# ototoi/pbrt-r3

Measured on AMD Instinct MI355X. Metric: Mrays/s, higher is better.
Workload: dtype f32

## Files before the change

pbrt-r3_amd/csrc/pt_context.cpp:

```cpp
#include <hip/hip_runtime.h>

#include <dlfcn.h>

#include <chrono>
#include <cmath>
#include <cstdio>
#include <cstdlib>
#include <cstring>
#include <functional>
#include <string>
#include <array>
#include <memory>
#include <vector>
#include <algorithm>
#include <thread>

#include "../../include/pbrtgpu.h"
#include "pt_bvh.h"
#include "pt_device.h"
#include "pt_host_math.h"
#include "pt_kernels.h"
#include "pt_lobes.h"

namespace {
// ... 154 lines not shown
        ctx->sobol_n_inv = hdr[3];
        ctx->sobol_m32.resize((size_t)hdr[0] * hdr[1]);
        ctx->sobol_vdc.resize((size_t)hdr[2] * hdr[1]);
        ctx->sobol_inv.resize((size_t)hdr[3] * hdr[1]);
        ok = std::fread(ctx->sobol_m32.data(), 4, ctx->sobol_m32.size(), f) == ctx->sobol_m32.size() &&
             std::fread(ctx->sobol_vdc.data(), 8, ctx->sobol_vdc.size(), f) == ctx->sobol_vdc.size() &&
             std::fread(ctx->sobol_inv.data(), 8, ctx->sobol_inv.size(), f) == ctx->sobol_inv.size();
    }
    std::fclose(f);
    return ok;
}

template <class T>
pt_status upload(pt_context* ctx, DevBuf& b, const T* src, size_t n) {
    PT_HIP(b.alloc(n * sizeof(T)));
    if (n) PT_HIP(hipMemcpy(b.p, src, n * sizeof(T), hipMemcpyHostToDevice));
    return PT_OK;
}

pt_status ensure_pool(pt_context* ctx, size_t n_paths) {
    if (ctx->sc.n_instances && ctx->d_hit_inst.bytes < std::max(n_paths, ctx->pool_paths) * 4) {
        PT_HIP(ctx->d_hit_inst.alloc(std::max(n_paths, ctx->pool_paths) * 4));
        ctx->paths.hit_inst = ctx->d_hit_inst.as<uint32_t>();
    }
    const bool tex_split = ctx->sc.textured && !ctx->sc.n_instances;
    if (tex_split && ctx->d_tex_res.bytes < std::max(n_paths, ctx->pool_paths) * (size_t)(PT_TEX_RES_F4 * 16)) {
        PT_HIP(ctx->d_tex_res.alloc(std::max(n_paths, ctx->pool_paths) * (size_t)(PT_TEX_RES_F4 * 16)));
        ctx->paths.tex_res = ctx->d_tex_res.as<float4>();
    } else if (!tex_split && ctx->d_tex_res.p) {
        ctx->d_tex_res.release();
        ctx->paths.tex_res = nullptr;
    }
    if (ctx->pool_paths >= n_paths && ctx->d_pool.p) return PT_OK;
    const size_t per_path = 11 * 16 + 8 + 8 + 6 * 4 + 4;
    PT_HIP(ctx->d_pool.alloc(n_paths * per_path + 16384));
    char* base = ctx->d_pool.as<char>();
    size_t off = 0;
    auto carve = [&](size_t elem) { void* p = base + off; off += (n_paths * elem + 255) & ~(size_t)255; return p; };
    PtPaths& P = ctx->paths;
    P.ray_o = (float4*)carve(16); P.ray_d = (float4*)carve(16);
    P.sh_o = (float4*)carve(16); P.sh_d = (float4*)carve(16);
    P.pr_o = (float4*)carve(16); P.pr_d = (float4*)carve(16);
    P.beta = (float4*)carve(16); P.L = (float4*)carve(16);
    P.pendA = (float4*)carve(16); P.pendB = (float4*)carve(16); P.pbeta = (float4*)carve(16);
    P.p_film = (float2*)carve(8);
    P.sobol_index = (uint64_t*)carve(8);
    P.pixel = (uint32_t*)carve(4); P.state = (uint32_t*)carve(4);
    P.hit_t = (float*)carve(4); P.hit_rec = (int32_t*)carve(4);
    P.nee = (uint32_t*)carve(4);
    P.probe_rec = (int32_t*)carve(4);
    P.occluded = (uint8_t*)carve(1);
    if (off > ctx->d_pool.bytes) return ctx->fail(PT_ERR_DEVICE, "internal: path pool carve overflow");
    PT_HIP(ctx->d_qa.alloc(n_paths * 4));
    PT_HIP(ctx->d_qb.alloc(n_paths * 4));
    PT_HIP(ctx->d_qnee.alloc(n_paths * 4));
    PT_HIP(ctx->d_qsorted.alloc(n_paths * 4));
    PT_HIP(ctx->d_qshadow.alloc(n_paths * 4));
    PT_HIP(ctx->d_qprobe.alloc(n_paths * 4));
    ctx->pool_paths = n_paths;
    return PT_OK;
}

pt_status ensure_traversal_scratch(pt_context* ctx) {
    uint32_t need = ctx->max_stack + 1 > PT_FS_SLOTS - 1 ? ctx->max_stack + 1 - (PT_FS_SLOTS - 1) : 0;
    size_t threads = (size_t)std::max(ctx->grid_trace, 2048) * PT_BLOCK;
    if (!ctx->d_spill.p || ctx->spill_depth < need) {
        PT_HIP(ctx->d_spill.alloc((size_t)std::max(need, 1u) * threads * 4 + PT_DIAG_WORDS * 4));
        PT_HIP(hipMemsetAsync(ctx->d_spill.p, 0, PT_DIAG_WORDS * 4, ctx->stream));
        ctx->spill_depth = need;
    }
    return PT_OK;
}

hipEvent_t get_event(pt_context* ctx, size_t i) {
    while (ctx->ev.size() <= i) {
        hipEvent_t e;
        if (hipEventCreate(&e) != hipSuccess) return nullptr;
        ctx->ev.push_back(e);
    }
    return ctx->ev[i];
}

}

extern "C" {
// ... 1687 lines not shown
            for (int32_t x = sbnd[0]; x < sbnd[2]; x += 16) {
                pt_tile t = {x, y, std::min(x + 16, sbnd[2]), std::min(y + 16, sbnd[3])};
                all.push_back(t);
            }
        tiles = all.data();
        n_tiles = (uint32_t)all.size();
    }
    std::vector<uint32_t> tile_off(n_tiles);
    size_t n_pixels_total = 0;
    for (uint32_t i = 0; i < n_tiles; i++) {
        const pt_tile& t = tiles[i];
        if (t.x0 < sbnd[0] || t.y0 < sbnd[1] || t.x1 > sbnd[2] || t.y1 > sbnd[3] || t.x1 < t.x0 || t.y1 < t.y0)
            return ctx->fail(PT_ERR_INVALID_ARGUMENT, "tile outside the sample bounds");
        tile_off[i] = (uint32_t)n_pixels_total;
        n_pixels_total += (size_t)(t.x1 - t.x0) * (size_t)(t.y1 - t.y0);
        if (n_pixels_total > (size_t)(sbnd[2] - sbnd[0]) * (size_t)(sbnd[3] - sbnd[1])) return ctx->fail(PT_ERR_INVALID_ARGUMENT, "tiles overlap (more pixels than the sample bounds hold)");
    }
    if (n_pixels_total == 0) return PT_OK;
    const uint32_t spp = sc.sobol.spp;

    size_t pool_target = (size_t)288 << 20;
    if (const char* e = std::getenv("PBRTGPU_POOL_PATHS")) pool_target = std::max<size_t>(65536, std::strtoull(e, nullptr, 10));
    pool_target = std::min<size_t>(pool_target, (size_t)1 << 30);
    const bool ao = sc.integrator == PT_INTEGRATOR_AO;
    const bool aov = sc.integrator == PT_INTEGRATOR_AOV;
    const bool rec = sc.integrator == PT_INTEGRATOR_DIRECTLIGHTING || sc.integrator == PT_INTEGRATOR_WHITTED;
    const uint32_t rec_epp = !rec ? 0u : (sc.integrator == PT_INTEGRATOR_DIRECTLIGHTING && sc.direct_strategy == PT_DIRECT_ONE) ? 1u
                             : sc.integrator == PT_INTEGRATOR_WHITTED ? std::max(1u, sc.n_lights) : std::max(1u, ctx->light_samples_total);
    const uint32_t rec_depth = (uint32_t)std::max(1, sc.max_depth);
    const size_t rec_per_path = 64 + (size_t)rec_depth * PT_REC_FRAME_F4 * 16 + (size_t)rec_epp * (6 * 16 + 1 + 4 + 4 + 8);
    {
        size_t free_b = 0, total_b = 0;
        if (hipMemGetInfo(&free_b, &total_b) == hipSuccess) {
            size_t per_path = 11 * 16 + 8 + 8 + 6 * 4 + 4 + 6 * 4 + 4 * 4;
            if (sc.textured && !sc.n_instances) per_path += PT_TEX_RES_F4 * 16;
            if (ctx->sort_cont != 0) per_path += 4 * 4;
            if (rec) {
                const size_t have = ctx->pool_paths * per_path + ctx->rec_paths * rec_per_path;
                const size_t budget = (free_b + have) / 2;
                pool_target = std::min(pool_target, std::max<size_t>(65536, budget / (per_path + rec_per_path)));
            } else if (ctx->pool_paths < pool_target) {
                pool_target = std::min(pool_target, std::max<size_t>(ctx->pool_paths, std::max<size_t>(1u << 20, (free_b / 2) / per_path)));
            }
        }
    }
    if (rec) pool_target = std::min<size_t>(pool_target, ((size_t)1 << 31) / std::max(1u, rec_epp));
    if (rec) if (const char* e = std::getenv("PBRTGPU_REC_POOL_BYTES")) pool_target = std::max<size_t>(65536, std::min<size_t>(pool_target, std::strtoull(e, nullptr, 10) / rec_per_path));
    if (ao) pool_target = std::max<size_t>(65536, std::min<size_t>(pool_target, ((size_t)128 << 20) / (size_t)sc.ao_samples));
    size_t chunk_pix = std::min(n_pixels_total, pool_target);
    uint32_t S = (uint32_t)std::max<size_t>(1, std::min<size_t>(spp, pool_target / chunk_pix));
    {
        const uint32_t passes = (spp + S - 1) / S;
        S = (spp + passes - 1) / passes;
    }
    pt_status st;
    if ((st = ensure_pool(ctx, chunk_pix * S)) != PT_OK) return st;
    if (ctx->pixels_cap < n_pixels_total) {
        PT_HIP(ctx->d_pixels.alloc(n_pixels_total * 4));
        ctx->pixels_cap = n_pixels_total;
    }
    {
        const size_t sb_w = (size_t)(sbnd[2] - sbnd[0]), sb_h = (size_t)(sbnd[3] - sbnd[1]);
        const size_t bm_bytes = ((sb_w * sb_h + 31) / 32) * 4;
        if (ctx->d_tilebits.bytes < bm_bytes) PT_HIP(ctx->d_tilebits.alloc(bm_bytes));
        if (ctx->d_tiles.bytes < (size_t)n_tiles * 20) PT_HIP(ctx->d_tiles.alloc((size_t)n_tiles * 20));
        uint32_t* d_off = reinterpret_cast<uint32_t*>(ctx->d_tiles.as<char>() + (size_t)n_tiles * 16);
        PT_HIP(hipMemsetAsync(ctx->d_tilebits.p, 0, bm_bytes, ctx->stream));
// ... 50 lines not shown
            PT_HIP(ctx->d_csort_keys[1].alloc(ctx->pool_paths * 4));
            PT_HIP(ctx->d_csort_temp.alloc(tb));
            ctx->csort_cap = ctx->pool_paths;
        }
    }
    PtCounters* cnt = ctx->d_counters.as<PtCounters>();
    uint32_t* err = ctx->d_err.as<uint32_t>();
    size_t ev_i = 0;
    std::vector<std::pair<size_t, int>> spans;
    const bool bounce_log = std::getenv("PBRTGPU_BOUNCE_LOG") != nullptr;
    std::vector<std::array<uint32_t, 3>> bounce_counts;
    const bool no_events = std::getenv("PBRTGPU_NO_EVENTS") != nullptr;

    hipEvent_t ev_begin = get_event(ctx, ev_i++), ev_end = get_event(ctx, ev_i++);
    PT_HIP(hipEventRecord(ev_begin, ctx->stream));

    for (size_t c0 = 0; c0 < n_pixels_total; c0 += chunk_pix) {
        uint32_t n_pix = (uint32_t)std::min(chunk_pix, n_pixels_total - c0);
        const uint32_t* d_pix = ctx->d_pixels.as<uint32_t>() + c0;
        for (uint32_t s0 = 0; s0 < spp; s0 += S) {
            uint32_t ns = std::min(S, spp - s0);
            uint32_t* qa = ctx->d_qa.as<uint32_t>();
            uint32_t* qb = ctx->d_qb.as<uint32_t>();
            Q.cur = qa; Q.next = qb;
            PT_HIP(ptk_gen(ctx->stream, ctx->grid_wide, sc, ctx->paths, Q, d_pix, n_pix, s0, ns, cnt));
            if (ao) {
                const uint32_t n_paths = n_pix * ns;
                const size_t cap = (size_t)n_paths * (size_t)sc.ao_samples;
                if (ctx->ao_rays_cap < cap) {
                    PT_HIP(ctx->d_ao.alloc(cap * 41 + 256));
                    ctx->ao_rays_cap = cap;
                    PT_HIP(ptk_iota(ctx->stream, ctx->grid_wide, reinterpret_cast<uint32_t*>(ctx->d_ao.as<char>() + ctx->ao_rays_cap * 36), (uint32_t)cap));
                }
                float4* ao_o = ctx->d_ao.as<float4>();
                float4* ao_d = ao_o + ctx->ao_rays_cap;
                float* ao_w = reinterpret_cast<float*>(ao_d + ctx->ao_rays_cap);
                uint32_t* ao_ids = reinterpret_cast<uint32_t*>(ao_w + ctx->ao_rays_cap);
                uint8_t* ao_occ = reinterpret_cast<uint8_t*>(ao_ids + ctx->ao_rays_cap);
                uint32_t* ao_count = ctx->d_ticket.as<uint32_t>() + 2;
                hipEvent_t a = get_event(ctx, ev_i), b = get_event(ctx, ev_i + 1), c = get_event(ctx, ev_i + 2);
                if (!a || !b || !c) return ctx->fail(PT_ERR_DEVICE, "hipEventCreate failed");
                spans.push_back({ev_i, 0});
                ev_i += 3;
                PT_HIP(hipMemsetAsync(ctx->d_ticket.p, 0, 16, ctx->stream));
                PT_HIP(ptk_ao_tag(ctx->stream, ctx->grid_wide, ctx->paths, n_pix, n_paths, s0));
                PT_HIP(hipEventRecord(a, ctx->stream));
                PT_HIP(ptk_trace_any(ctx, ctx->stream, ctx->grid_trace, ctx->grid_trace_dist, sc, ctx->paths, Q, cnt, ctx->d_spill.as<uint32_t>(), ctx->spill_depth, err, 0, ctx->scene_alpha ? 1 : 0));
                ctx->trace_launches++;
                PT_HIP(ptk_ao_rays_any(ctx, ctx->stream, ctx->grid_wide, sc, ctx->paths, n_paths, ao_o, ao_d, ao_w, ao_count, cnt));
                {
                    PtPaths AP = ctx->paths;
                    AP.sh_o = ao_o; AP.sh_d = ao_d; AP.occluded = ao_occ;
                    PtQueues AQ = Q;
                    AQ.shadow = ao_ids;
                    PT_HIP(ptk_ao_queue(ctx->stream, AQ, ao_count, (uint32_t)sc.ao_samples));
                    PT_HIP(ptk_trace_any(ctx, ctx->stream, ctx->grid_trace, ctx->grid_trace_dist, sc, AP, AQ, cnt, ctx->d_spill.as<uint32_t>(), ctx->spill_depth, err, 0, ctx->scene_alpha ? 1 : 0));
                    ctx->trace_launches++;
                }
                PT_HIP(hipEventRecord(b, ctx->stream));
                PT_HIP(ptk_ao_resolve_any(ctx, ctx->stream, ctx->grid_wide, sc, ctx->paths, n_paths, ao_w, ao_occ));
                PT_HIP(hipEventRecord(c, ctx->stream));
            } else if (aov) {
                const uint32_t n_paths = n_pix * ns;
                hipEvent_t a = get_event(ctx, ev_i), b = get_event(ctx, ev_i + 1), c = get_event(ctx, ev_i + 2);
                if (!a || !b || !c) return ctx->fail(PT_ERR_DEVICE, "hipEventCreate failed");
                spans.push_back({ev_i, 0});
                ev_i += 3;
                PT_HIP(hipEventRecord(a, ctx->stream));
                PT_HIP(ptk_trace_any(ctx, ctx->stream, ctx->grid_trace, ctx->grid_trace_dist, sc, ctx->paths, Q, cnt, ctx->d_spill.as<uint32_t>(), ctx->spill_depth, err, 0, ctx->scene_alpha ? 1 : 0));
                ctx->trace_launches++;
                PT_HIP(hipEventRecord(b, ctx->stream));
                PT_HIP(ptk_aov_any(ctx, ctx->stream, ctx->grid_wide, sc, ctx->paths, n_paths, ctx->aov_target, ctx->aov_scale, cnt));
                PT_HIP(hipEventRecord(c, ctx->stream));
            } else if (rec) {
                const uint32_t n_paths = n_pix * ns;
                const size_t np = chunk_pix * (size_t)S, ne = np * rec_epp;
                if (ctx->rec_paths < np || ctx->rec_epp != rec_epp || ctx->rec_depth != rec_depth || !ctx->d_rec.p) {
                    PT_HIP(ctx->d_rec.alloc(np * rec_per_path + 65536));
                    ctx->rec_paths = np; ctx->rec_epp = rec_epp; ctx->rec_depth = rec_depth;
                    if (!ctx->d_counts2.p) PT_HIP(ctx->d_counts2.alloc(PT_COUNTS_WORDS * 4));
                }
                PT_HIP(hipMemsetAsync(ctx->d_counts2.p, 0, PT_COUNTS_WORDS * 4, ctx->stream));
                PtRec R;
                char* rb = ctx->d_rec.as<char>();
                auto take = [&](size_t bytes) { char* q = rb; rb += (bytes + 255) & ~(size_t)255; return q; };
                R.diff = (float4*)take(np * 64);
                R.frames = (float4*)take(np * (size_t)rec_depth * PT_REC_FRAME_F4 * 16);
                R.sh_o = (float4*)take(ne * 16); R.sh_d = (float4*)take(ne * 16); R.pr_o = (float4*)take(ne * 16); R.pr_d = (float4*)take(ne * 16);
                R.A = (float4*)take(ne * 16); R.B = (float4*)take(ne * 16);
                R.panic = err;
                R.prec = (int32_t*)take(ne * 4); R.flags = (uint32_t*)take(ne * 4);
                uint32_t* nl_shadow = (uint32_t*)take(ne * 4);
                uint32_t* nl_probe = (uint32_t*)take(ne * 4);
                R.occ = (uint8_t*)take(ne);
                R.n_paths = (uint32_t)np; R.max_depth = rec_depth; R.epp = rec_epp;
                R.n_arrays = (sc.integrator == PT_INTEGRATOR_DIRECTLIGHTING && sc.direct_strategy == PT_DIRECT_ALL) ? 2u * sc.n_lights * (uint32_t)std::max(sc.max_depth, 0) : 0u;
                R.s0 = s0; R.n_pix = n_pix;
                if (5u + 2u * R.n_arrays > 60000u) return ctx->fail(PT_ERR_UNSUPPORTED, "directlighting \"all\": too many lights x maxdepth for the sampler's array dimensions");
                PtPaths NP = ctx->paths;
                NP.sh_o = R.sh_o; NP.sh_d = R.sh_d; NP.pr_o = R.pr_o; NP.pr_d = R.pr_d; NP.occluded = R.occ; NP.probe_rec = R.prec;
                PtQueues Qn = Q;
                Qn.counts = ctx->d_counts2.as<uint32_t>(); Qn.shadow = nl_shadow; Qn.probe = nl_probe;
                PT_HIP(ptk_rec_init_any(ctx, ctx->stream, ctx->grid_wide, sc, ctx->paths, R, n_paths));
                if (!ctx->h_live) PT_HIP(hipHostMalloc((void**)&ctx->h_live, 64));
                hipEvent_t rb_ev[2] = {get_event(ctx, ev_i), get_event(ctx, ev_i + 1)};
                if (!rb_ev[0] || !rb_ev[1]) return ctx->fail(PT_ERR_DEVICE, "hipEventCreate failed");
                ev_i += 2;
                for (uint32_t iter = 0; iter < 100000u; iter++) {
                    hipEvent_t a = get_event(ctx, ev_i), b = get_event(ctx, ev_i + 1), c = get_event(ctx, ev_i + 2);
                    if (!a || !b || !c) return ctx->fail(PT_ERR_DEVICE, "hipEventCreate failed");
                    if (ev_i < 3000) { spans.push_back({ev_i, 0}); ev_i += 3; }
                    Qn.cur = Q.cur;
                    PT_HIP(hipEventRecord(a, ctx->stream));
                    PT_HIP(ptk_trace_any(ctx, ctx->stream, ctx->grid_trace, ctx->grid_trace_dist, sc, ctx->paths, Q, cnt, ctx->d_spill.as<uint32_t>(), ctx->spill_depth, err, 0, ctx->scene_alpha ? 1 : 0));
                    PT_HIP(ptk_prep(ctx->stream, Qn, 0));
                    PT_HIP(ptk_rec_enter_any(ctx, ctx->stream, ctx->grid_shade, sc, ctx->paths, Q, Qn, R, cnt, rec_epp));
                    PtQueues Qt = Qn;
                    if (Qn.shadow_key) {
                        uint32_t n_sh = 0;
                        PT_HIP(hipMemcpyAsync(&n_sh, Qn.counts + PT_Q_SHADOW, 4, hipMemcpyDeviceToHost, ctx->stream));
                        PT_HIP(hipStreamSynchronize(ctx->stream));
                        if (n_sh >= (uint32_t)ctx->sort_shadow_min) {
                            uint32_t* sorted = nullptr;
                            PT_HIP(ptk_sort_shadow_rays(ctx->stream, Qn.shadow, ctx->d_sort_ids.as<uint32_t>(), ctx->d_sort_keys[0].as<uint32_t>(),
                                                        ctx->d_sort_keys[1].as<uint32_t>(), ctx->d_sort_temp.p, ctx->d_sort_temp.bytes, n_sh, &sorted));
                            Qt.shadow = sorted;
                        }
                    }
                    PT_HIP(ptk_trace_any(ctx, ctx->stream, ctx->grid_trace, ctx->grid_trace_dist, sc, NP, Qt, cnt, ctx->d_spill.as<uint32_t>(), ctx->spill_depth, err, 0, ctx->scene_alpha ? 1 : 0));
                    ctx->trace_launches += 2;
                    PT_HIP(hipEventRecord(b, ctx->stream));
                    PT_HIP(ptk_rec_next_any(ctx, ctx->stream, ctx->grid_shade, sc, ctx->paths, Q, R));
                    PT_HIP(ptk_prep(ctx->stream, Q, 1));
// ... 323 lines not shown
    PT_HIP(hipMemsetAsync(ctx->d_ticket.p, 0, 16, ctx->stream));
    hipEvent_t a = get_event(ctx, 0), b = get_event(ctx, 1);
    PT_HIP(hipEventRecord(a, ctx->stream));
    PT_HIP(ptk_trace_batch_any(ctx, ctx->stream, ctx->grid_trace, ctx->sc, n, d_o.as<float>(), d_d.as<float>(), d_t.as<float>(), any_hit ? nullptr : d_out.as<pt_hit>(),
                           any_hit ? d_out.as<uint8_t>() : nullptr, any_hit, ctx->d_ticket.as<uint32_t>(), ctx->d_counters.as<PtCounters>(),
                           ctx->d_spill.as<uint32_t>(), ctx->spill_depth, ctx->d_err.as<uint32_t>(), ctx->scene_alpha ? 1 : 0));
    PT_HIP(hipEventRecord(b, ctx->stream));
    PT_HIP(hipStreamSynchronize(ctx->stream));
    float ms = 0;
    PT_HIP(hipEventElapsedTime(&ms, a, b));
    ctx->trace_ms += ms;
    ctx->trace_launches++;
    uint32_t herr = 0;
    PT_HIP(hipMemcpy(&herr, ctx->d_err.p, 4, hipMemcpyDeviceToHost));
    if (herr) { PT_HIP(hipMemsetAsync(ctx->d_err.p, 0, 4, ctx->stream)); PT_HIP(hipStreamSynchronize(ctx->stream)); return ctx->fail(PT_ERR_DEVICE, "traversal stack overflow"); }
    if (any_hit) PT_HIP(hipMemcpy(occ, d_out.p, n, hipMemcpyDeviceToHost));
    else PT_HIP(hipMemcpy(out, d_out.p, (size_t)n * sizeof(pt_hit), hipMemcpyDeviceToHost));
    return PT_OK;
}

pt_status pt_trace_closest(pt_context* ctx, uint32_t n, const float* o, const float* d, const float* tmax, pt_hit* out) {
    return trace_batch(ctx, n, o, d, tmax, out, nullptr, 0);
}
pt_status pt_trace_any(pt_context* ctx, uint32_t n, const float* o, const float* d, const float* tmax, uint8_t* occluded_out) {
    return trace_batch(ctx, n, o, d, tmax, nullptr, occluded_out, 1);
}

pt_status pt_trace_wavefront(pt_context* ctx, uint32_t n, const float* o, const float* d, const float* tmax, const uint8_t* kind, pt_hit* out,
                             uint8_t* occluded_out) {
    if (!ctx || !o || !d || !tmax || !kind || !out || !occluded_out) return PT_ERR_INVALID_ARGUMENT;
    if (!ctx->have_scene) return ctx->fail(PT_ERR_NO_SCENE, "no scene uploaded");
    if (n == 0) return PT_OK;
    (void)hipSetDevice(ctx->device);
    std::vector<float> o4((size_t)n * 4), d4((size_t)n * 4);
    std::vector<uint32_t> ids[3];
    for (uint32_t i = 0; i < n; i++) {
        if (kind[i] < 1 || kind[i] > 3) return ctx->fail(PT_ERR_INVALID_ARGUMENT, "ray kind must be 1 (continuation), 2 (shadow) or 3 (probe)");
        ids[kind[i] - 1].push_back(i);
        for (int k = 0; k < 3; k++) { o4[4 * (size_t)i + k] = o[3 * (size_t)i + k]; d4[4 * (size_t)i + k] = d[3 * (size_t)i + k]; }
        o4[4 * (size_t)i + 3] = tmax[i];
        d4[4 * (size_t)i + 3] = 0.0f;
    }
    pt_status st;
    if ((st = ensure_pool(ctx, std::max<size_t>(n, 65536))) != PT_OK) return st;
    const PtPaths& P = ctx->paths;
    float4* const dst_o[3] = {P.ray_o, P.sh_o, P.pr_o};
    float4* const dst_d[3] = {P.ray_d, P.sh_d, P.pr_d};
    for (int k = 0; k < 3; k++) {
        PT_HIP(hipMemcpyAsync(dst_o[k], o4.data(), (size_t)n * 16, hipMemcpyHostToDevice, ctx->stream));
        PT_HIP(hipMemcpyAsync(dst_d[k], d4.data(), (size_t)n * 16, hipMemcpyHostToDevice, ctx->stream));
    }
    PtQueues Q;
    Q.cur = ctx->d_qa.as<uint32_t>(); Q.next = ctx->d_qb.as<uint32_t>();
    Q.nee = ctx->d_qnee.as<uint32_t>(); Q.counts = ctx->d_counts.as<uint32_t>(); Q.sorted = ctx->d_qsorted.as<uint32_t>();
    Q.shadow = ctx->d_qshadow.as<uint32_t>(); Q.probe = ctx->d_qprobe.as<uint32_t>(); Q.shadow_key = nullptr; Q.bin = nullptr;
    uint32_t* const dst_q[3] = {Q.cur, Q.shadow, Q.probe};
    for (int k = 0; k < 3; k++)
        if (!ids[k].empty()) PT_HIP(hipMemcpyAsync(dst_q[k], ids[k].data(), ids[k].size() * 4, hipMemcpyHostToDevice, ctx->stream));
    std::vector<uint32_t> counts(PT_COUNTS_WORDS, 0u);
    counts[PT_Q_CUR] = (uint32_t)ids[0].size(); counts[PT_Q_SHADOW] = (uint32_t)ids[1].size(); counts[PT_Q_PROBE] = (uint32_t)ids[2].size();
    PT_HIP(hipMemcpyAsync(Q.counts, counts.data(), counts.size() * 4, hipMemcpyHostToDevice, ctx->stream));
    DevBuf d_kind, d_out, d_occ;
    PT_HIP(d_kind.alloc(n)); PT_HIP(d_out.alloc((size_t)n * sizeof(pt_hit))); PT_HIP(d_occ.alloc(n));
    PT_HIP(hipMemcpyAsync(d_kind.p, kind, n, hipMemcpyHostToDevice, ctx->stream));
    hipEvent_t a = get_event(ctx, 0), b = get_event(ctx, 1);
    PT_HIP(hipEventRecord(a, ctx->stream));
    PT_HIP(ptk_trace_any(ctx, ctx->stream, ctx->grid_trace, ctx->grid_trace_dist, ctx->sc, P, Q, ctx->d_counters.as<PtCounters>(), ctx->d_spill.as<uint32_t>(), ctx->spill_depth,
                     ctx->d_err.as<uint32_t>(), ctx->trace_far > 0 ? 1 : 0, ctx->scene_alpha ? 1 : 0));
    PT_HIP(hipEventRecord(b, ctx->stream));
    PT_HIP(ptk_wavefront_results_any(ctx, ctx->stream, ctx->grid_wide, ctx->sc, P, n, d_kind.as<uint8_t>(), d_out.as<pt_hit>(), d_occ.as<uint8_t>()));
    PT_HIP(hipMemsetAsync(Q.counts, 0, PT_COUNTS_WORDS * 4, ctx->stream));
    PT_HIP(hipStreamSynchronize(ctx->stream));
    float ms = 0;
    PT_HIP(hipEventElapsedTime(&ms, a, b));
    ctx->trace_ms += ms;
    ctx->trace_launches++;
    uint32_t herr = 0;
    PT_HIP(hipMemcpy(&herr, ctx->d_err.p, 4, hipMemcpyDeviceToHost));
    if (herr) { PT_HIP(hipMemsetAsync(ctx->d_err.p, 0, 4, ctx->stream)); PT_HIP(hipStreamSynchronize(ctx->stream)); return ctx->fail(PT_ERR_DEVICE, "traversal stack overflow"); }
    PT_HIP(hipMemcpy(out, d_out.p, (size_t)n * sizeof(pt_hit), hipMemcpyDeviceToHost));
    PT_HIP(hipMemcpy(occluded_out, d_occ.p, n, hipMemcpyDeviceToHost));
    return PT_OK;
}

// ... 235 lines not shown
```

pbrt-r3_amd/csrc/pt_device.h:

```cpp
#pragma once
#include <stdint.h>
#include "../../include/pbrtgpu.h"

#define PT_WAVE 64
#define PT_BLOCK 256
#ifndef PT_LDS_STACK
#define PT_LDS_STACK 32
#endif
#ifndef PT_TRACE_WIDE
#define PT_TRACE_WIDE 1
#endif
#define PT_TBLOCK (PT_TRACE_WIDE ? 1024 : PT_BLOCK)
#define PT_SLOT (PT_TBLOCK * 4u)
#ifndef PT_TOP_NODES
#define PT_TOP_NODES (PT_TRACE_WIDE ? 341 : 85)
#endif
#ifndef PT_SORT_CELL_BITS
#define PT_SORT_CELL_BITS 4
#endif
#define PT_TOP_BFS_NODES 1365u
#if PT_TOP_NODES > 0
#define PT_FS_SLOTS (PT_LDS_STACK < 24 ? PT_LDS_STACK : 24)
#else
#define PT_FS_SLOTS PT_LDS_STACK
#endif
#define PT_DIAG_WORDS 2048u
#define PT_EMPTY_REF 0xffffffffu
#define PT_LEAF_BIT 0x80000000u
#define PT_LEAF_COUNT_SHIFT 28
#define PT_LEAF_FIRST_MASK 0x03ffffffu
#define PT_REF_INDEX_MASK 0x03ffffffu
#define PT_REF_AXIS_SHIFT 26

// ... 254 lines not shown
    uint32_t n_envs;
    const pt_texture* textures;
    const uint32_t* tex_prog;
    const PtImage* images;
    const PtMatParams* mat_params;
    uint32_t textured;
    uint32_t n_spheres;
    uint32_t n_lights;
    uint32_t root_ref;
    uint32_t n_top;
    float cell_scale[3];
    float wb_min[3], wb_max[3];
    int32_t max_depth;
    float rr_threshold;
    int32_t integrator;
    int32_t direct_strategy;
    int32_t ao_samples, ao_cos_sample;
    PtCamera cam;
    PtFilm film;
    PtSobol sobol;
    PtLightGrid grid;
};
PT_HOSTDEV_ENVS inline const PtEnvLight* scene_envs(const PtScene& sc) { return reinterpret_cast<const PtEnvLight*>(sc.lights + sc.n_lights); }
PT_HOSTDEV_ENVS inline const PtDeltaLight* scene_deltas(const PtScene& sc) { return reinterpret_cast<const PtDeltaLight*>(scene_envs(sc) + sc.n_envs); }
PT_HOSTDEV_ENVS inline uint32_t scene_n_mix(const PtScene& sc) { return sc.general_materials >> 1; }
PT_HOSTDEV_ENVS inline const PtMix& material_mix(const PtScene& sc, const PtMaterial& m) {
    return reinterpret_cast<const PtMix*>(sc.materials + m.mix_base)[m.mix1 - 1u];
}
PT_HOSTDEV_ENVS inline const PtDisneyParams& material_disney(const PtMaterial& m) { return *reinterpret_cast<const PtDisneyParams*>(m.lobes); }
static_assert(sizeof(PtMaterial) % 16 == 0 && sizeof(PtMix) % 4 == 0, "the PtMix table behind the materials");
static_assert(sizeof(PtDeltaLight) == 80 && sizeof(PtEnvLight) % 8 == 0 && sizeof(PtLight) % 16 == 0, "side records of the light buffer");
static_assert(__builtin_offsetof(PtScene, nodes) == 16, "n_deltas fills the hole in front of PtScene::nodes");

struct PtPaths {
    float4* ray_o;
    float4* ray_d;
    float4* sh_o;
    float4* sh_d;
    float4* pr_o;
    float4* pr_d;
    float4* beta;
    float4* L;
    float4* pendA;
    float4* pendB;
    float4* pbeta;
    float2* p_film;
    uint64_t* sobol_index;
    uint32_t* pixel;
    uint32_t* state;
    float* hit_t;
    int32_t* hit_rec;
    uint32_t* nee;
    uint8_t* occluded;
    int32_t* probe_rec;
    uint32_t* hit_inst;
    float4* tex_res;
};
#define PT_TEX_RES_F4 9u

#define PT_REC_FRAME_F4 8u
struct PtRec {
    float4* diff;
    float4* frames;
    float4 *sh_o, *sh_d, *pr_o, *pr_d, *A, *B;
    uint8_t* occ;
    int32_t* prec;
    uint32_t* flags;
    uint32_t n_paths, max_depth, epp, n_arrays;
    uint32_t s0, n_pix;
    uint32_t* panic;
};
#define PT_REC_OUT_FRAME 0u
#define PT_REC_OUT_RETURN0 1u
#define PT_REC_OUT_RETRACE 2u
#define PT_ST_DIFF 1u

#define PT_ST_SPECULAR 1u
#define PT_ST_CAMERA 2u
#define PT_NEE_SHADOW 1u
#define PT_NEE_PROBE 2u

struct PtQueues {
    uint32_t* cur;
    uint32_t* next;
    uint32_t* nee;
    uint32_t* shadow;
    uint32_t* probe;
    uint32_t* counts;
    uint32_t* sorted;
    uint16_t* bin;
    uint32_t* shadow_key;
};
#define PT_Q_CUR 0u
#define PT_Q_MATTE_END 1u
#define PT_Q_GENERAL_END 2u
#define PT_Q_TEX_BEGIN 3u
#define PT_Q_NEXT 32u
// ... 14 lines not shown
```

pbrt-r3_amd/csrc/pt_kernels.hip:

```cpp
#include <hip/hip_runtime.h>
#include <cstdlib>
#include "pt_device.h"
#include "pt_device_math.h"
#include "pt_bxdf.h"
#include "pt_sphere.h"
#include "pt_quadric.h"
#include "pt_texture.h"
#include <type_traits>
#include "pt_lobes.h"
#include "pt_kernels.h"
#include "../../include/pbrtgpu.h"

#if PT_QUADRIC
#define PT_KERNEL __global__
#ifndef PT_KERNEL_NS
#define PT_KERNEL_NS ptq
#endif
namespace PT_KERNEL_NS {
#else
#define PT_KERNEL extern "C" __global__
#endif

#ifndef PT_LIGHTS_IN_LDS
#define PT_LIGHTS_IN_LDS 8
// ... 977 lines not shown
        slot[HANDOUT] += dt;
        if (handout) { slot[HANDOUTS] += 1; slot[HANDOUTS_CLK] += dt; }
    }
    PT_DEV void serviced() { t_mark = now(); slot[SERVICE] += (unsigned long long)(t_mark - t_iter); }
    PT_DEV void round(int clk, int rounds, int items, unsigned long long n) { lap(clk); slot[rounds] += 1; slot[items] += n; }
    PT_DEV void node_round(unsigned long long lanes) { round(NODE, NODE_ROUNDS, NODE_LANES, (unsigned long long)__popcll(lanes)); }
    PT_DEV void general_round(unsigned long long lanes) { round(GENERAL, GENERAL_ROUNDS, NODE_LANES, (unsigned long long)__popcll(lanes)); }
    PT_DEV void leaf_round(unsigned long long items) { round(LEAF_FINISH, LEAF_ROUNDS, LEAF_ITEMS, items); }
    PT_DEV void leaf_issued() { lap(LEAF_ISSUE); asm volatile("s_waitcnt vmcnt(0)" ::: "memory"); lap(LEAF_WAIT); }
    PT_DEV void finish(uint32_t* diag, uint32_t lane) {
        slot[TOTAL] = (unsigned long long)(now() - t_start);
        if (lane == 0) for (int i = 0; i < SLOTS; i++) atomicAdd(reinterpret_cast<unsigned long long*>(diag) + i, slot[i]);
    }
};
#else
#define PT_PROF_BEGIN() ((void)0)
#define PT_PROF(call) ((void)0)
#endif
#ifndef PT_REFILL_MIN
#define PT_REFILL_MIN 8
#endif
#ifndef PT_LEAF_MIN
#define PT_LEAF_MIN 24
#endif
#ifndef PT_LEAF_MIN_INST
#define PT_LEAF_MIN_INST 40
#endif
#ifndef PT_TRACE_WAVES
#define PT_TRACE_WAVES 4
#endif
#ifndef PT_TRACE_DIST_WAVES
#define PT_TRACE_DIST_WAVES 4
#endif

#ifndef PT_LEAF_LANES_MIN
#define PT_LEAF_LANES_MIN 18
#endif
static_assert(PT_LEAF_LANES_MIN > 0, "the leaf round is triggered by the number of parked lanes");
#ifndef PT_SPH_LANES_MIN
#define PT_SPH_LANES_MIN 8
#endif
PT_DEV uint32_t wave_max_scan(uint32_t x) {
    x = max(x, (uint32_t)__builtin_amdgcn_update_dpp(0, (int)x, 0x111, 0xf, 0xf, false));
    x = max(x, (uint32_t)__builtin_amdgcn_update_dpp(0, (int)x, 0x112, 0xf, 0xf, false));
    x = max(x, (uint32_t)__builtin_amdgcn_update_dpp(0, (int)x, 0x114, 0xf, 0xf, false));
    x = max(x, (uint32_t)__builtin_amdgcn_update_dpp(0, (int)x, 0x118, 0xf, 0xf, false));
    x = max(x, (uint32_t)__builtin_amdgcn_update_dpp(0, (int)x, 0x142, 0xa, 0xf, false));
    x = max(x, (uint32_t)__builtin_amdgcn_update_dpp(0, (int)x, 0x143, 0xc, 0xf, false));
    return x;
}
template <bool DIST, bool SPH, bool INST = false, bool FAR = false, bool ALPHA = false>
PT_DEV void trace_body(const PtScene& sc, const PtPaths& P, const PtQueues& Q, PtCounters* cnt, uint32_t* spill, uint32_t spill_depth, uint32_t* err) {
    constexpr uint32_t TB = DIST ? PT_TBLOCK : PT_BLOCK;
    __shared__ uint32_t s_stack[(DIST ? PT_FS_SLOTS : PT_LDS_STACK) * TB];
    __shared__ unsigned long long s_cnt[4];
    __shared__ float4 s_res[DIST ? TB : 1];
#if PT_TOP_NODES > 0
    __shared__ float4 s_top[DIST ? PT_TOP_NODES * 7 : 1];
#endif
    TravCtx c;
    c.lds = &s_stack[threadIdx.x];
    c.top_lds = 0; c.top_bytes = 0; c.n_nodes_lds = 0;
    c.spill_stride = gridDim.x * TB;
    c.spill = spill + PT_DIAG_WORDS + (size_t)blockIdx.x * TB + threadIdx.x;
    c.spill_depth = spill_depth;
    c.n_nodes = 0; c.n_tris = 0; c.overflow = 0;
// ... 34 lines not shown
    PT_PROF_BEGIN();
    for (;;) {
        PT_PROF(iteration());
        constexpr bool PF_BYPASS = DIST && !FAR;
        int pf_gate = pf_stage;
        if constexpr (PF_BYPASS) asm volatile("" : "+s"(pf_gate));
        if (PF_BYPASS && pf_gate == 3) {
        } else if (pf_stage == 0) {
            if (more) {
                if (lane == 0) pf_raw = atomicAdd(&Q.counts[PT_Q_SEG_TICKET0 + 32u * seg], 64u);
                pf_stage = 1;
            }
        } else if (pf_stage == 1) {
            const uint32_t seg_lo = seg * seg_len, seg_hi = min(total, seg_lo + seg_len);
            const uint32_t base = seg_lo + (uint32_t)__builtin_amdgcn_readfirstlane((int)pf_raw);
            if (seg_lo >= total || base >= seg_hi) {
                seg = (seg + 1u) & 7u;
                if (++seg_dry == 8u) more = false;
                pf_stage = 0;
            } else {
                seg_dry = 0;
                pf_count = min(64u, seg_hi - base);
                pf_used = 0;
                const uint32_t item = base + lane;
                if (lane < pf_count) {
                    if (item < n_cur) { pf_p = Q.cur[item]; pf_kind = 1; }
                    else if (item < n_cur + n_sh) { pf_p = Q.shadow[item - n_cur]; pf_kind = 2; }
                    else { pf_p = Q.probe[item - n_cur - n_sh]; pf_kind = 3; }
                }
                pf_stage = 2;
            }
        } else if (pf_stage == 2) {
            if (lane < pf_count) {
                const float4* so = pf_kind == 1 ? P.ray_o : (pf_kind == 2 ? P.sh_o : P.pr_o);
                const float4* sd = pf_kind == 1 ? P.ray_d : (pf_kind == 2 ? P.sh_d : P.pr_d);
                pf_o = so[pf_p]; pf_d = sd[pf_p];
            }
            pf_stage = 3;
        }
        PT_PROF(lap(PhaseProf::PREFETCH));
        constexpr bool LATE_RETIRE = DIST;
#define PT_RETIRE()                                                                                                                                      \
        if (kind != 0 && ray_done(r)) {                                                                                                                  \
            if (kind == 1) { P.hit_t[p] = r.ray_tmax; P.hit_rec[p] = r.best; if (INST && (!ALPHA || sc.n_instances)) P.hit_inst[p] = r.best_inst; }      \
            else if (kind == 2) P.occluded[p] = r.best >= 0 ? 1 : 0;                                                                                     \
            else P.probe_rec[p] = r.best;                                                                                                                \
            kind = 0;                                                                                                                                    \
        }
        if constexpr (LATE_RETIRE) {
            if (!more) { PT_RETIRE() }
        } else {
            PT_RETIRE()
        }
        {
            const unsigned long long idle = LATE_RETIRE ? __ballot(kind == 0 || ray_done(r)) : __ballot(kind == 0);
            const uint32_t n_idle = (uint32_t)__popcll(idle);
            if (pf_stage == 3 && (n_idle >= PT_REFILL_MIN || idle == ~0ull || (!more && n_idle != 0))) {
                PT_PROF(hand_out());
                if constexpr (LATE_RETIRE) { PT_RETIRE() }
                const uint32_t take = min(n_idle, pf_count - pf_used);
                const uint32_t rank = (uint32_t)__popcll(idle & below);
                const int src = (int)((pf_used + rank) & 63u);
                const uint32_t np = (uint32_t)__shfl((int)pf_p, src, 64);
                const int nk = __shfl(pf_kind, src, 64);
                float4 ro, rd;
                ro.x = __shfl(pf_o.x, src, 64); ro.y = __shfl(pf_o.y, src, 64); ro.z = __shfl(pf_o.z, src, 64); ro.w = __shfl(pf_o.w, src, 64);
                rd.x = __shfl(pf_d.x, src, 64); rd.y = __shfl(pf_d.y, src, 64); rd.z = __shfl(pf_d.z, src, 64);
                if (kind == 0 && rank < take) {
                    p = np; kind = nk;
                    if (nk == 2) shadow++; else regular++;
                    if constexpr (DIST) ray_begin_fs(sc, r, c, f4_3(ro), mk3(rd.x, rd.y, rd.z), ro.w);
                    else ray_begin(sc, r, f4_3(ro), mk3(rd.x, rd.y, rd.z), ro.w);
                }
                pf_used += take;
                if (pf_used == pf_count) pf_stage = 0;
            }
        }
// ... 142 lines not shown
            };
            const bool lean = __ballot(w_node && r.sa >= r.sa_limit) == 0ull;
            if (lean && m_node != 0 && leaf_level < LEAF_DUE) {
                PT_PROF(mark());
                if constexpr (FAR) node_step_coop(sc, r, c, w_node, m_node);
                else if (w_node) node_step_lean(sc, r, c);
                PT_PROF(node_round(m_node));
            } else if (m_node != 0 && leaf_level < LEAF_DUE) {
                PT_PROF(mark());
                if (w_node) node_step_general(sc, r, c);
                PT_PROF(general_round(m_node));
            } else if ((m_tri | m_tri_s) != 0) {
                if constexpr (SPH) {
                    sround = sph_go || m_tri == 0;
                    w_serve = w_tri && (sph_wait == sround);
                    tcnt_r = w_serve ? tcnt : 0u;
                }
                PT_PROF(mark());
                if (SPH && sround) leaf_issue(std::true_type{}); else leaf_issue(std::false_type{});
                PT_PROF(leaf_issued());
                if (SPH && sround) leaf_finish(std::true_type{}); else leaf_finish(std::false_type{});
                PT_PROF(leaf_round(lf_items));
            }
        } else {
        if (m_node != 0 && __popcll(m_tri) < (INST ? PT_LEAF_MIN_INST : PT_LEAF_MIN)) {
            if (w_node) ray_step_node(sc, r, c);
            PT_PROF(general_round(m_node));
        } else {
            if constexpr (INST) {
                if (w_tri) {
                    if (r.top == PT_INST_EXIT_REF) {
                        (void)stk_pop(c, r.top, r.sp);
                        const float w_tmax = __uint_as_float(stk_pop(c, r.top, r.sp)), w_tmin = __uint_as_float(stk_pop(c, r.top, r.sp));
                        const float4 ro = (kind == 1 ? P.ray_o : (kind == 2 ? P.sh_o : P.pr_o))[p], rd = (kind == 1 ? P.ray_d : (kind == 2 ? P.sh_d : P.pr_d))[p];
                        const bool hit_inside = r.best >= 0 && r.best_inst == r.cur_inst;
                        ray_set_direction_state(r, f4_3(ro), mk3(rd.x, rd.y, rd.z));
                        r.tmin = w_tmin; r.tmax = hit_inside ? r.ray_tmax : w_tmax;
                        r.cur_inst = 0;
                    } else ray_step_tri_enter<SPH, ALPHA>(sc, r, kind == 2, c);
                }
            } else {
                if (w_tri) ray_step_tri<SPH, INST>(sc, r, kind == 2, c);
            }
            PT_PROF(leaf_round((unsigned long long)__popcll(m_tri)));
        }
        }
    }
    PT_PROF(finish(spill, lane));
    if (c.overflow) atomicOr(err, 1u);
    flush_counters(cnt, s_cnt, regular, shadow, c.n_nodes, c.n_tris);
    {
        unsigned long long v = c.n_nodes_lds;
        for (int o = 32; o > 0; o >>= 1) v += (unsigned long long)__shfl_xor((int)(v >> 32), o, 64) << 32 | (unsigned int)__shfl_xor((int)(unsigned int)v, o, 64);
        if ((threadIdx.x & 63) == 0 && v) atomicAdd(&cnt->nodes_lds, v);
    }
}
PT_KERNEL void __launch_bounds__(PT_TBLOCK, PT_TRACE_DIST_WAVES) k_trace(PtScene sc, PtPaths P, PtQueues Q, PtCounters* cnt, uint32_t* spill,
                                                              uint32_t spill_depth, uint32_t* err) {
    trace_body<true, false>(sc, P, Q, cnt, spill, spill_depth, err);
}
PT_KERNEL void __launch_bounds__(PT_TBLOCK, PT_TRACE_DIST_WAVES) k_trace_far(PtScene sc, PtPaths P, PtQueues Q, PtCounters* cnt, uint32_t* spill,
                                                                   uint32_t spill_depth, uint32_t* err) {
    trace_body<true, false, false, true>(sc, P, Q, cnt, spill, spill_depth, err);
}
PT_KERNEL void __launch_bounds__(PT_BLOCK, PT_TRACE_WAVES) k_trace_seq(PtScene sc, PtPaths P, PtQueues Q, PtCounters* cnt, uint32_t* spill,
                                                                  uint32_t spill_depth, uint32_t* err) {
    trace_body<false, false>(sc, P, Q, cnt, spill, spill_depth, err);
// ... 65 lines not shown
    }
    if (c.overflow) atomicOr(err, 1u);
    flush_counters(cnt, s_cnt, regular, shadow, c.n_nodes, c.n_tris);
}
PT_KERNEL void __launch_bounds__(PT_BLOCK) k_trace_batch(PtScene sc, uint32_t n, const float* o, const float* d, const float* tmax,
                                                                    pt_hit* out, uint8_t* occ_out, int any_hit, uint32_t* ticket, PtCounters* cnt,
                                                                    uint32_t* spill, uint32_t spill_depth, uint32_t* err) {
    trace_batch_body<false>(sc, n, o, d, tmax, out, occ_out, any_hit, ticket, cnt, spill, spill_depth, err);
}
PT_KERNEL void __launch_bounds__(PT_BLOCK) k_trace_batch_sph(PtScene sc, uint32_t n, const float* o, const float* d, const float* tmax,
                                                                        pt_hit* out, uint8_t* occ_out, int any_hit, uint32_t* ticket, PtCounters* cnt,
                                                                        uint32_t* spill, uint32_t spill_depth, uint32_t* err) {
    trace_batch_body<true>(sc, n, o, d, tmax, out, occ_out, any_hit, ticket, cnt, spill, spill_depth, err);
}
PT_KERNEL void __launch_bounds__(PT_BLOCK) k_trace_batch_inst(PtScene sc, uint32_t n, const float* o, const float* d, const float* tmax,
                                                                         pt_hit* out, uint8_t* occ_out, int any_hit, uint32_t* ticket, PtCounters* cnt,
                                                                         uint32_t* spill, uint32_t spill_depth, uint32_t* err) {
    trace_batch_body<true, true>(sc, n, o, d, tmax, out, occ_out, any_hit, ticket, cnt, spill, spill_depth, err);
}
PT_KERNEL void __launch_bounds__(PT_BLOCK) k_trace_batch_alpha(PtScene sc, uint32_t n, const float* o, const float* d, const float* tmax,
                                                                          pt_hit* out, uint8_t* occ_out, int any_hit, uint32_t* ticket, PtCounters* cnt,
                                                                          uint32_t* spill, uint32_t spill_depth, uint32_t* err) {
    trace_batch_body<true, true, true>(sc, n, o, d, tmax, out, occ_out, any_hit, ticket, cnt, spill, spill_depth, err);
}

PT_KERNEL void __launch_bounds__(PT_BLOCK) k_wavefront_results(PtScene sc, PtPaths P, uint32_t n, const uint8_t* kind, pt_hit* out, uint8_t* occ) {
    for (uint32_t i = blockIdx.x * blockDim.x + threadIdx.x; i < n; i += gridDim.x * blockDim.x) {
        const uint32_t k = kind[i];
        pt_hit h;
        h.t = 0.0f; h.prim = -1; h.b0 = 0.0f; h.b1 = 0.0f;
        uint8_t oc = 0;
        if (k == 2u) oc = P.occluded[i];
        else {
            const int32_t rec = k == 1u ? P.hit_rec[i] : P.probe_rec[i];
            if (rec >= 0) {
                const uint32_t inst = (k == 1u && sc.n_instances) ? P.hit_inst[i] : 0u;
                TriVerts tv = load_tri(sc.tris, (uint32_t)rec);
                h.prim = inst ? (int32_t)sc.instances[inst - 1u].world_prim : (int32_t)tv.prim;
                if (k == 1u) {
                    h.t = P.hit_t[i];
                    if (!inst && !(tv.flags & (PT_TRI_SPHERE | PT_TRI_INSTANCE))) {
                        RayPre rp;
                        ray_precompute(rp, f4_3(P.ray_o[i]), f4_3(P.ray_d[i]));
                        TriHit th;
                        tri_test(rp, tv.p0, tv.p1, tv.p2, tv.flags, PT_INF, th);
                        h.b0 = th.b0; h.b1 = th.b1;
                    }
                }
            }
        }
        out[i] = h;
        occ[i] = oc;
    }
}
hipError_t ptk_wavefront_results(hipStream_t st, int grid, const PtScene& sc, const PtPaths& P, uint32_t n, const uint8_t* kind, pt_hit* out, uint8_t* occ) {
    hipLaunchKernelGGL(k_wavefront_results, dim3(grid), dim3(PT_BLOCK), 0, st, sc, P, n, kind, out, occ);
    return hipGetLastError();
}

PT_KERNEL void __launch_bounds__(PT_BLOCK) k_expand_tiles(const int4* tiles, const uint32_t* tile_off, uint32_t n_tiles, int32_t sb_x0, int32_t sb_y0,
                                                                     uint32_t sb_w, uint32_t* pixels, uint32_t* bitmap, uint32_t* err) {
    for (uint32_t t = blockIdx.x; t < n_tiles; t += gridDim.x) {
        const int4 tl = tiles[t];
        const uint32_t w = (uint32_t)(tl.z - tl.x), n = w * (uint32_t)(tl.w - tl.y), off = tile_off[t];
        for (uint32_t i = threadIdx.x; i < n; i += blockDim.x) {
            const uint32_t x = (uint32_t)(tl.x - sb_x0) + i % w, y = (uint32_t)(tl.y - sb_y0) + i / w;
            pixels[off + i] = x | (y << 16);
            const uint32_t bit = y * sb_w + x;
            if (atomicOr(&bitmap[bit >> 5], 1u << (bit & 31u)) & (1u << (bit & 31u))) atomicOr(err, 2u);
        }
    }
}
hipError_t ptk_expand_tiles(hipStream_t st, const int4* tiles, const uint32_t* tile_off, uint32_t n_tiles, int32_t sb_x0, int32_t sb_y0, uint32_t sb_w,
                            uint32_t* pixels, uint32_t* bitmap, uint32_t* err) {
    hipLaunchKernelGGL(k_expand_tiles, dim3(n_tiles < 4096u ? n_tiles : 4096u), dim3(PT_BLOCK), 0, st, tiles, tile_off, n_tiles, sb_x0, sb_y0, sb_w, pixels, bitmap, err);
    return hipGetLastError();
}

PT_KERNEL void __launch_bounds__(PT_BLOCK) k_gen(PtScene sc, PtPaths P, PtQueues Q, const uint32_t* pixels, uint32_t n_pix,
                                                            uint32_t s0, uint32_t n_samples, PtCounters* cnt) {
    uint32_t n = n_pix * n_samples;
    for (uint32_t i = blockIdx.x * blockDim.x + threadIdx.x; i < n; i += gridDim.x * blockDim.x) {
        uint32_t pk = pixels[i % n_pix];
        uint32_t s = s0 + i / n_pix;
        int32_t rx = (int32_t)(pk & 0xffffu), ry = (int32_t)(pk >> 16);
        int32_t px = rx + sc.film.sample_bounds[0], py = ry + sc.film.sample_bounds[1];
        Sampler sm;
        sm.index = sampler_index(sc, s, px, py);
        sm.dim = 0; sm.px = px; sm.py = py;
        V2 uf = sm.get_2d(sc);
        V2 p_film = mk2((float)px + uf.x, (float)py + uf.y);
        V2 u_lens = sm.get_2d(sc);
        (void)sm.get_1d(sc);
        V3 o, d;
        generate_camera_ray(sc, p_film, u_lens, &o, &d);
        P.ray_o[i] = make_float4(o.x, o.y, o.z, PT_INF);
        P.ray_d[i] = make_float4(d.x, d.y, d.z, 0.0f);
        P.beta[i] = make_float4(1.0f, 1.0f, 1.0f, 1.0f);
        P.L[i] = make_float4(0.0f, 0.0f, 0.0f, 0.0f);
        P.p_film[i] = make_float2(p_film.x, p_film.y);
        P.sobol_index[i] = sm.index;
        P.pixel[i] = pk;
        P.state[i] = sm.dim | (PT_ST_CAMERA << 24);
        P.nee[i] = 0;
        Q.cur[i] = i;
    }
    if (blockIdx.x == 0 && threadIdx.x == 0) {
        Q.counts[PT_Q_CUR] = n; Q.counts[PT_Q_NEXT] = 0; Q.counts[PT_Q_NEE] = 0; Q.counts[PT_Q_TICKET] = 0; Q.counts[PT_Q_SHADOW] = 0; Q.counts[PT_Q_PROBE] = 0;
        for (uint32_t k = 0; k < 8u; k++) Q.counts[PT_Q_SEG_TICKET0 + 32u * k] = 0;
        atomicAdd(&cnt->camera_rays, (unsigned long long)n);
    }
}

PT_KERNEL void k_prep(PtQueues Q, int mode) {
    if (threadIdx.x == 0 && blockIdx.x == 0) {
        if (mode == 0) {
            Q.counts[PT_Q_NEXT] = 0; Q.counts[PT_Q_NEE] = 0; Q.counts[PT_Q_TICKET] = 0; Q.counts[PT_Q_TICKET2] = 0; Q.counts[PT_Q_TICKET3] = 0; Q.counts[PT_Q_SHADOW] = 0; Q.counts[PT_Q_PROBE] = 0;
            for (uint32_t k = 0; k < 8u; k++) Q.counts[PT_Q_SEG_TICKET0 + 32u * k] = 0;
        } else {
            Q.counts[PT_Q_CUR] = Q.counts[PT_Q_NEXT]; Q.counts[PT_Q_NEXT] = 0; Q.counts[PT_Q_TICKET] = 0;
            for (uint32_t k = 0; k < 8u; k++) Q.counts[PT_Q_SEG_TICKET0 + 32u * k] = 0;
        }
    }
}

struct Surf {
    V3 p, p_error, n, wo;
    V3 sh_n, sh_dpdu;
    uint32_t prim;
    int32_t material, light;
    V2 uv;
    V3 dpdu, dpdv;
    V3 sh_dpdv, sh_dndu, sh_dndv;
};

PT_DEV void tri_dpdu(const PtScene& sc, bool has_attr, const PtTriInfo& ti, V3 p0, V3 p1, V3 p2, V3* dpdu, V3* dpdv, V2* uvs) {
// ... 400 lines not shown
            return i < 4 ? lo : hi;
        };
        uint32_t first = 0, len = n + 1;
        while (len > 0) {
            uint32_t half = len >> 1, middle = first + half;
            if (get(n + middle) <= u) { first = middle + 1; len -= half + 1; }
            else len = half;
        }
        idx = first == 0 ? 0 : first - 1;
        if (idx > n - 1) idx = n - 1;
        f_idx = get(idx);
        func_int = get(2 * n + 1);
    } else {
        const float* cdf = tab + n;
        uint32_t first = 0, len = n + 1;
        while (len > 0) {
            uint32_t half = len >> 1, middle = first + half;
            if (cdf[middle] <= u) { first = middle + 1; len -= half + 1; }
            else len = half;
        }
        idx = first == 0 ? 0 : first - 1;
        if (idx > n - 1) idx = n - 1;
        f_idx = tab[idx];
        func_int = tab[2 * n + 1];
    }
    *pdf = func_int > 0.0f ? f_idx * (1.0f / (float)n) / func_int : 0.0f;
    return idx;
}

PT_KERNEL void __launch_bounds__(PT_BLOCK) k_nee_resolve(PtScene sc, PtPaths P, PtQueues Q) {
    const uint32_t n = Q.counts[PT_Q_NEE];
    for (uint32_t i = blockIdx.x * blockDim.x + threadIdx.x; i < n; i += gridDim.x * blockDim.x) {
        const uint32_t p = Q.nee[i];
        const float4 A = P.pendA[p];
        if (__float_as_uint(A.w) == 0u) {
            if (P.occluded[p] == 0) {
                float4 L = P.L[p];
                L.x += A.x; L.y += A.y; L.z += A.z;
                P.L[p] = L;
            }
            continue;
        }
        const uint32_t nee = P.nee[p];
        V3 ld = mk3(0.0f, 0.0f, 0.0f);
        if ((nee & PT_NEE_SHADOW) && P.occluded[p] == 0) ld = ld + mk3(A.x, A.y, A.z);
        if (nee & PT_NEE_PROBE) {
            const int32_t best = P.probe_rec[p];
            if (best >= 0 && (uint32_t)best == sc.lights[nee >> 8].tri_rec) { float4 B = P.pendB[p]; ld = ld + mk3(B.x, B.y, B.z); }
        }
        V3 ldn = ld / A.w;
        float4 pb = P.pbeta[p];
        float4 L = P.L[p];
        V3 add = mk3(pb.x, pb.y, pb.z) * ldn;
        L.x += add.x; L.y += add.y; L.z += add.z;
        P.L[p] = L;
    }
}
PT_KERNEL void __launch_bounds__(PT_BLOCK) k_nee_resolve_env(PtScene sc, PtPaths P, PtQueues Q) {
    const uint32_t n = Q.counts[PT_Q_NEE];
    for (uint32_t i = blockIdx.x * blockDim.x + threadIdx.x; i < n; i += gridDim.x * blockDim.x) {
        const uint32_t p = Q.nee[i];
        const float4 A = P.pendA[p];
        if (__float_as_uint(A.w) == 0u) {
            if (P.occluded[p] == 0) {
                float4 L = P.L[p];
                L.x += A.x; L.y += A.y; L.z += A.z;
                P.L[p] = L;
            }
            continue;
        }
        const uint32_t nee = P.nee[p];
        V3 ld = mk3(0.0f, 0.0f, 0.0f);
        if ((nee & PT_NEE_SHADOW) && P.occluded[p] == 0) ld = ld + mk3(A.x, A.y, A.z);
        if (nee & PT_NEE_PROBE) {
            const int32_t best = P.probe_rec[p];
            const PtLight& lt = sc.lights[nee >> 8];
            const bool take = (lt.mesh_flags & PT_LIGHT_INFINITE) ? best < 0 : (best >= 0 && (uint32_t)best == lt.tri_rec);
            if (take) { float4 B = P.pendB[p]; ld = ld + mk3(B.x, B.y, B.z); }
        }
        V3 ldn = ld / A.w;
        float4 pb = P.pbeta[p];
        float4 L = P.L[p];
        V3 add = mk3(pb.x, pb.y, pb.z) * ldn;
        L.x += add.x; L.y += add.y; L.z += add.z;
        P.L[p] = L;
    }
}

PT_DEV uint32_t path_sort_bin(const PtScene& sc, const PtPaths& P, uint32_t p) {
    int32_t rec = P.hit_rec[p];
    if (rec < 0) return 0xffffffffu;
    uint32_t m1 = sc.tris[rec].flags >> PT_TRI_MATERIAL_SHIFT;
    return m1 == 0 ? (sc.n_instances ? PT_SORT_GENERAL0 : 0u) : sc.materials[m1 - 1].sort_bin;
}
PT_DEV uint32_t wave_bin_reserve(uint32_t* counters, uint32_t bin, bool valid) {
    uint32_t slot = 0;
    unsigned long long todo = __ballot(valid);
    const uint32_t lane = threadIdx.x & 63;
    while (todo) {
        int leader = __ffsll((long long)todo) - 1;
        uint32_t b0 = (uint32_t)__shfl((int)bin, leader, 64);
        unsigned long long same = __ballot(valid && bin == b0) & todo;
        uint32_t base = 0;
        if ((int)lane == leader) base = atomicAdd(&counters[b0], (uint32_t)__popcll(same));
        base = (uint32_t)__shfl((int)base, leader, 64);
        if (valid && bin == b0) slot = base + (uint32_t)__popcll(same & ((lane == 0) ? 0ull : (~0ull >> (64 - lane))));
        todo &= ~same;
    }
    return slot;
}
PT_DEV void sort_chunk(uint32_t n, uint32_t* lo, uint32_t* hi) {
    uint32_t chunk = (n + gridDim.x - 1) / gridDim.x;
    chunk = (chunk + 63u) & ~63u;
    *lo = min(n, blockIdx.x * chunk);
    *hi = min(n, *lo + chunk);
}
PT_KERNEL void __launch_bounds__(PT_BLOCK) k_sort_count(PtScene sc, PtPaths P, PtQueues Q) {
    __shared__ uint32_t s_cnt[PT_SORT_BINS];
    s_cnt[threadIdx.x] = 0;
    __syncthreads();
    uint32_t lo, hi;
    sort_chunk(Q.counts[PT_Q_CUR], &lo, &hi);
    for (uint32_t i = lo + threadIdx.x; i < ((hi + 63u) & ~63u); i += blockDim.x) {
// ... 378 lines not shown
                if (e & 1u) Q.next[bc + (uint32_t)__popcll(mc & below)] = ep;
                if (e & 2u) Q.nee[bn + (uint32_t)__popcll(mn & below)] = ep;
                if (e & 4u) {
                    Q.shadow[bs + (uint32_t)__popcll(ms & below)] = ep;
                    if (Q.shadow_key) Q.shadow_key[bs + (uint32_t)__popcll(ms & below)] = s_pkey[j][threadIdx.x];
                }
                if (e & 8u) Q.probe[bp + (uint32_t)__popcll(mp & below)] = ep;
                bc += (uint32_t)__popcll(mc); bn += (uint32_t)__popcll(mn); bs += (uint32_t)__popcll(ms); bp += (uint32_t)__popcll(mp);
            }
        }
        n_batch = 0; pend_want = 0;
    };
    for (;;) {
        PT_SHP(11);
        if (chunk_left == 0) {
            uint32_t t0 = 0;
            if (lane == 0) t0 = atomicAdd(ticket, 64u * PT_SHADE_TICKET);
            next_base = begin + (uint32_t)__builtin_amdgcn_readfirstlane((int)t0);
            chunk_left = PT_SHADE_TICKET;
        }
        uint32_t base = next_base;
        next_base += 64u; chunk_left--;
        if (base >= end) break;
#ifdef PT_PROFILE_SHADE
        shp_acc[12]++;
#endif
        uint32_t item = base + lane;
        bool active = item < end;
        bool cont = false, want_nee = false, want_sh = false, want_pr = false;
        uint32_t p = 0;
        uint32_t wr = 0, o_nee = 0, o_state = 0;
        float4 o_ray_o = make_float4(0.0f, 0.0f, 0.0f, 0.0f), o_ray_d = o_ray_o, o_beta = o_ray_o;
        auto commit = [&]() {
            if (wr & 64u) P.pendA[p] = s_stage[4][threadIdx.x];
            if (wr & 4u) { P.sh_o[p] = s_stage[0][threadIdx.x]; P.sh_d[p] = s_stage[1][threadIdx.x]; }
            if (wr & 8u) { P.pr_o[p] = s_stage[2][threadIdx.x]; P.pr_d[p] = s_stage[3][threadIdx.x]; }
            if (wr & 16u) { P.pendA[p] = s_stage[4][threadIdx.x]; P.pendB[p] = s_stage[5][threadIdx.x]; P.pbeta[p] = s_stage[6][threadIdx.x]; P.nee[p] = o_nee; }
            if (wr & 1u) P.ray_o[p] = o_ray_o;
            if (wr & 2u) { P.ray_d[p] = o_ray_d; P.beta[p] = o_beta; }
            if (wr & 32u) P.state[p] = o_state;
            wr = 0;
        };
#ifndef PT_DEFER_WIDE
#define PT_DEFER_WIDE 0
#endif
#ifndef PT_DEFER_SITES
#define PT_DEFER_SITES (PT_DEFER_WIDE ? 63 : 0)
#endif
#define PT_COMMIT_NOW(site) do { if constexpr ((TEX || INST) && !((PT_DEFER_SITES >> (site)) & 1)) commit(); } while (0)
        const bool had_pf = pf_valid;
        const uint32_t pf_p_now = pf_p;
        const int32_t pf_rec_now = pf_rec;
        const uint32_t pf_st_now = pf_st, pf_pk_now = pf_pk;
        const uint64_t pf_idx_now = pf_idx;
        pf_valid = chunk_left > 0;
        const bool pf_lane = pf_valid && next_base + lane < end;
        if (pf_lane) pf_p = list[next_base + lane];
        if (active) {
            p = had_pf ? pf_p_now : list[item];
            PT_SHP_SYNC(13);
            const float4 ro4 = P.ray_o[p], rd4 = P.ray_d[p], beta4 = P.beta[p];
            V3 ro = f4_3(ro4), rd = f4_3(rd4);
            int32_t rec = had_pf ? pf_rec_now : P.hit_rec[p];
            uint32_t st = had_pf ? pf_st_now : P.state[p];
            uint32_t dim = st & 0xffffu, bounces = (st >> 16) & 0xffu, flags = st >> 24;
            V3 beta = f4_3(beta4);
            float eta_scale = beta4.w;
            PT_SHP_SYNC(14);
            float4 rec_a = make_float4(0.0f, 0.0f, 0.0f, 0.0f), rec_b = rec_a, rec_c = rec_a;
            if (rec >= 0) {
                const float4* q = reinterpret_cast<const float4*>(sc.tris) + (size_t)(uint32_t)rec * 3;
                rec_a = q[0]; rec_b = q[1]; rec_c = q[2];
            }
            SamplerPre sm;
            sm.s.index = 0; sm.s.dim = dim; sm.s.px = 0; sm.s.py = 0; sm.dim0 = dim; sm.have = false;
            if (rec >= 0 && (int32_t)bounces < sc.max_depth) {
                sm.s.index = had_pf ? pf_idx_now : P.sobol_index[p];
                const uint32_t pk = had_pf ? pf_pk_now : P.pixel[p];
                sm.s.px = (int32_t)(pk & 0xffffu) + sc.film.sample_bounds[0];
                sm.s.py = (int32_t)(pk >> 16) + sc.film.sample_bounds[1];
                PT_SHP_SYNC(15);
                sm.begin(sc);
                PT_SHP_SYNC(10);
            }
            Surf s;
            float thit;
            bool found;
            if constexpr (INST) found = rec >= 0 && make_surf_inst<SPH>(sc, ro, rd, (uint32_t)rec, P.hit_inst[p], s, &thit);
            else found = rec >= 0 && make_surf_any_rec<SPH>(sc, ro, rd, (uint32_t)rec, rec_a, rec_b, rec_c, s, &thit);
            PT_SHP(0);
            if (pf_lane) {
                pf_rec = P.hit_rec[pf_p];
                pf_st = P.state[pf_p]; pf_idx = P.sobol_index[pf_p]; pf_pk = P.pixel[pf_p];
            }
            if constexpr (ENV) {
                if (rec < 0 && (bounces == 0 || (flags & PT_ST_SPECULAR))) {
                    float4 L = P.L[p];
                    for (uint32_t k = 0; k < sc.n_envs; k++) {
                        const V3 add = beta * env_le(sc, scene_envs(sc)[k], rd);
                        L.x += add.x; L.y += add.y; L.z += add.z;
                    }
                    P.L[p] = L;
                }
            }
            if (found && (bounces == 0 || (flags & PT_ST_SPECULAR))) {
                int32_t li = s.light;
                if (li >= 0) {
                    V3 le = light_L(sc.lights[li], s.n, -rd);
                    float4 L = P.L[p];
                    V3 add = beta * le;
                    L.x += add.x; L.y += add.y; L.z += add.z;
                    P.L[p] = L;
                }
            }
            if (found && (int32_t)bounces < sc.max_depth) {
                bool no_bsdf = s.material < 0;
                PtMaterial tm;
                std::conditional_t<MIX, PtMixHit, PtNoMix> mh;
                bool use_tm = false;
                if constexpr (TEX) {
                    if (!no_bsdf && sc.materials[s.material].textured) {
                        TexHit th;
                        th.p = s.p; th.uv = s.uv;
                        RayDiffs rdf;
                        const bool has_diff = (flags & PT_ST_CAMERA) != 0;
                        if (has_diff) {
                            Sampler sl;
                            sl.index = P.sobol_index[p];
                            sl.dim = 2;
                            uint32_t pk2 = P.pixel[p];
                            sl.px = (int32_t)(pk2 & 0xffffu) + sc.film.sample_bounds[0];
                            sl.py = (int32_t)(pk2 >> 16) + sc.film.sample_bounds[1];
                            V2 u_lens = mk2(0.0f, 0.0f);
                            if (sc.cam.lens_radius > 0.0f) u_lens = sl.get_2d(sc);
                            float2 pf = P.p_film[p];
                            camera_differentials(sc, mk2(pf.x, pf.y), u_lens, ro, rd, rdf);
                        }
                        compute_differentials(th, s.p, s.n, s.dpdu, s.dpdv, has_diff, rdf);
                        if constexpr (MIX) {
                            if (sc.materials[s.material].mix1) mix_hit(sc, s.material, th, &tm, &mh, s);
                            else textured_lobes(sc, s.material, th, &tm, s.n, s.uv, &s.sh_n, &s.sh_dpdu, s.sh_dpdv, s.sh_dndu, s.sh_dndv);
                        } else
                        textured_lobes(sc, s.material, th, &tm, s.n, s.uv, &s.sh_n, &s.sh_dpdu, s.sh_dpdv, s.sh_dndu, s.sh_dndv);
                        use_tm = true;
                        no_bsdf = tm.has_bsdf == 0;
                    }
                }
                if constexpr (RES) {
                    if (!no_bsdf && sc.materials[s.material].textured) {
                        const float4* r = P.tex_res + (size_t)p * PT_TEX_RES_F4;
                        const float4 r0 = r[0], r1 = r[1], r2 = r[2], r3 = r[3], r4 = r[4], r5 = r[5], r6 = r[6], r7 = r[7], r8 = r[8];
                        PtMatParams mp = sc.mat_params[s.material];
                        mp.m.kd[0] = r0.x; mp.m.kd[1] = r0.y; mp.m.kd[2] = r0.z; mp.m.ks[0] = r0.w; mp.m.ks[1] = r1.x; mp.m.ks[2] = r1.y;
                        mp.m.kr[0] = r1.z; mp.m.kr[1] = r1.w; mp.m.kr[2] = r2.x; mp.m.kt[0] = r2.y; mp.m.kt[1] = r2.z; mp.m.kt[2] = r2.w;
                        mp.m.opacity[0] = r3.x; mp.m.opacity[1] = r3.y; mp.m.opacity[2] = r3.z; mp.m.sigma = r3.w;
                        mp.m.metal_eta[0] = r4.x; mp.m.metal_eta[1] = r4.y; mp.m.metal_eta[2] = r4.z; mp.m.metal_k[0] = r4.w; mp.m.metal_k[1] = r5.x; mp.m.metal_k[2] = r5.y;
                        mp.m.uroughness = r5.z; mp.m.vroughness = r5.w; mp.m.eta = r6.x;
                        build_lobes_call(mp.m, r6.y, r6.z, r6.w, tm);
                        s.sh_n = mk3(r7.x, r7.y, r7.z); s.sh_dpdu = mk3(r7.w, r8.x, r8.y);
                        use_tm = true;
                        no_bsdf = tm.has_bsdf == 0;
                    }
                }
// ... 235 lines not shown
    if (n_vert) atomicAdd(&s_vert, (unsigned long long)n_vert);
    __syncthreads();
    if (threadIdx.x == 0 && s_vert) atomicAdd(&cnt->vertices, s_vert);
}
PT_KERNEL void __launch_bounds__(PT_BLOCK, PT_SHADE_WAVES) k_shade(PtScene sc, PtPaths P, PtQueues Q, PtCounters* cnt) {
    shade_body<false, false>(sc, P, Q, cnt, Q.cur, 0u, Q.counts[PT_Q_CUR], &Q.counts[PT_Q_TICKET]);
}
PT_KERNEL void __launch_bounds__(PT_BLOCK, PT_SHADE_WAVES) k_shade_matte_sorted(PtScene sc, PtPaths P, PtQueues Q, PtCounters* cnt) {
    shade_body<false, false>(sc, P, Q, cnt, Q.sorted, 0u, Q.counts[PT_Q_MATTE_END], &Q.counts[PT_Q_TICKET]);
}
PT_KERNEL void __launch_bounds__(PT_BLOCK, PT_SHADE_GEN_WAVES) k_shade_general(PtScene sc, PtPaths P, PtQueues Q, PtCounters* cnt) {
    shade_body<true, false>(sc, P, Q, cnt, Q.sorted, Q.counts[PT_Q_MATTE_END], Q.counts[PT_Q_TEX_BEGIN], &Q.counts[PT_Q_TICKET2]);
}
PT_KERNEL void __launch_bounds__(PT_BLOCK, PT_WIDE_KERNEL_WAVES) k_shade_matte_sorted_sph(PtScene sc, PtPaths P, PtQueues Q, PtCounters* cnt) {
    shade_body<false, true>(sc, P, Q, cnt, Q.sorted, 0u, Q.counts[PT_Q_MATTE_END], &Q.counts[PT_Q_TICKET]);
}
PT_KERNEL void __launch_bounds__(PT_BLOCK, PT_WIDE_KERNEL_WAVES) k_shade_general_sph(PtScene sc, PtPaths P, PtQueues Q, PtCounters* cnt) {
    shade_body<true, true>(sc, P, Q, cnt, Q.sorted, Q.counts[PT_Q_MATTE_END], Q.counts[PT_Q_TEX_BEGIN], &Q.counts[PT_Q_TICKET2]);
}
PT_KERNEL void __launch_bounds__(PT_BLOCK, PT_WIDE_KERNEL_WAVES) k_shade_general_inst(PtScene sc, PtPaths P, PtQueues Q, PtCounters* cnt) {
    shade_body<true, true, true, true>(sc, P, Q, cnt, Q.sorted, Q.counts[PT_Q_MATTE_END], Q.counts[PT_Q_GENERAL_END], &Q.counts[PT_Q_TICKET2]);
}
PT_KERNEL void __launch_bounds__(PT_BLOCK, PT_WIDE_KERNEL_WAVES) k_shade_general_inst_plain(PtScene sc, PtPaths P, PtQueues Q, PtCounters* cnt) {
    shade_body<true, false, false, true>(sc, P, Q, cnt, Q.sorted, Q.counts[PT_Q_MATTE_END], Q.counts[PT_Q_GENERAL_END], &Q.counts[PT_Q_TICKET2]);
}

template <bool SPH>
PT_DEV void tex_resolve_body(const PtScene& sc, const PtPaths& P, const PtQueues& Q) {
    const uint32_t begin = Q.counts[PT_Q_TEX_BEGIN], end = Q.counts[PT_Q_GENERAL_END];
    const uint32_t* list = Q.sorted;
    __shared__ float s_texval[3 * PT_TEX_PROG_MAX][PT_BLOCK];
    for (uint32_t i = begin + blockIdx.x * blockDim.x + threadIdx.x; i < end; i += gridDim.x * blockDim.x) {
        const uint32_t p = list[i];
        const int32_t rec = P.hit_rec[p];
        const uint32_t st = P.state[p];
        const uint32_t bounces = (st >> 16) & 0xffu, flags = st >> 24;
        if (rec < 0 || (int32_t)bounces >= sc.max_depth) continue;
        const float4 ro4 = P.ray_o[p], rd4 = P.ray_d[p];
        const V3 ro = f4_3(ro4), rd = f4_3(rd4);
        const float4* q = reinterpret_cast<const float4*>(sc.tris) + (size_t)(uint32_t)rec * 3;
        const float4 rec_a = q[0], rec_b = q[1], rec_c = q[2];
        Surf s;
        float thit;
        if (!make_surf_any_rec<SPH>(sc, ro, rd, (uint32_t)rec, rec_a, rec_b, rec_c, s, &thit)) continue;
        if (s.material < 0 || !sc.materials[s.material].textured) continue;
        TexHit th;
        th.p = s.p; th.uv = s.uv;
        RayDiffs rdf;
        const bool has_diff = (flags & PT_ST_CAMERA) != 0;
        if (has_diff) {
            Sampler sl;
            sl.index = P.sobol_index[p];
            sl.dim = 2;
            const uint32_t pk2 = P.pixel[p];
            sl.px = (int32_t)(pk2 & 0xffffu) + sc.film.sample_bounds[0];
            sl.py = (int32_t)(pk2 >> 16) + sc.film.sample_bounds[1];
            V2 u_lens = mk2(0.0f, 0.0f);
            if (sc.cam.lens_radius > 0.0f) u_lens = sl.get_2d(sc);
            const float2 pf = P.p_film[p];
            camera_differentials(sc, mk2(pf.x, pf.y), u_lens, ro, rd, rdf);
        }
        compute_differentials(th, s.p, s.n, s.dpdu, s.dpdv, has_diff, rdf);
        PtMatParams mp;
        float a3[3];
        textured_params_t<true>(sc, s.material, th, mp, a3, s.n, s.uv, &s.sh_n, &s.sh_dpdu, s.sh_dpdv, s.sh_dndu, s.sh_dndv, &s_texval[0][threadIdx.x]);
        float4* o = P.tex_res + (size_t)p * PT_TEX_RES_F4;
        o[0] = make_float4(mp.m.kd[0], mp.m.kd[1], mp.m.kd[2], mp.m.ks[0]);
        o[1] = make_float4(mp.m.ks[1], mp.m.ks[2], mp.m.kr[0], mp.m.kr[1]);
        o[2] = make_float4(mp.m.kr[2], mp.m.kt[0], mp.m.kt[1], mp.m.kt[2]);
        o[3] = make_float4(mp.m.opacity[0], mp.m.opacity[1], mp.m.opacity[2], mp.m.sigma);
        o[4] = make_float4(mp.m.metal_eta[0], mp.m.metal_eta[1], mp.m.metal_eta[2], mp.m.metal_k[0]);
        o[5] = make_float4(mp.m.metal_k[1], mp.m.metal_k[2], mp.m.uroughness, mp.m.vroughness);
        o[6] = make_float4(mp.m.eta, a3[0], a3[1], a3[2]);
        o[7] = make_float4(s.sh_n.x, s.sh_n.y, s.sh_n.z, s.sh_dpdu.x);
        o[8] = make_float4(s.sh_dpdu.y, s.sh_dpdu.z, 0.0f, 0.0f);
    }
}
#ifndef PT_TEX_RESOLVE_WAVES
#define PT_TEX_RESOLVE_WAVES 2
#endif
PT_KERNEL void __launch_bounds__(PT_BLOCK, PT_TEX_RESOLVE_WAVES) k_tex_resolve(PtScene sc, PtPaths P, PtQueues Q) { tex_resolve_body<false>(sc, P, Q); }
PT_KERNEL void __launch_bounds__(PT_BLOCK, PT_TEX_RESOLVE_WAVES) k_tex_resolve_sph(PtScene sc, PtPaths P, PtQueues Q) { tex_resolve_body<true>(sc, P, Q); }
PT_KERNEL void __launch_bounds__(PT_BLOCK, PT_SHADE_GEN_WAVES) k_shade_general_res(PtScene sc, PtPaths P, PtQueues Q, PtCounters* cnt) {
    shade_body<true, false, false, false, true>(sc, P, Q, cnt, Q.sorted, Q.counts[PT_Q_TEX_BEGIN], Q.counts[PT_Q_GENERAL_END], &Q.counts[PT_Q_TICKET3]);
}
PT_KERNEL void __launch_bounds__(PT_BLOCK, PT_WIDE_KERNEL_WAVES) k_shade_general_res_sph(PtScene sc, PtPaths P, PtQueues Q, PtCounters* cnt) {
    shade_body<true, true, false, false, true>(sc, P, Q, cnt, Q.sorted, Q.counts[PT_Q_TEX_BEGIN], Q.counts[PT_Q_GENERAL_END], &Q.counts[PT_Q_TICKET3]);
}

PT_KERNEL void __launch_bounds__(PT_BLOCK) k_cont_keys(PtScene sc, PtPaths P, const uint32_t* list, uint32_t n, uint32_t* keys) {
    for (uint32_t i = blockIdx.x * blockDim.x + threadIdx.x; i < n; i += gridDim.x * blockDim.x) {
        const uint32_t p = list[i];
        const float4 o = P.ray_o[p], d = P.ray_d[p];
        keys[i] = ray_sort_key(sc, mk3(o.x, o.y, o.z), mk3(d.x, d.y, d.z));
    }
}

PT_KERNEL void __launch_bounds__(PT_BLOCK, PT_SHADE_GEN_WAVES) k_shade_all(PtScene sc, PtPaths P, PtQueues Q, PtCounters* cnt) {
    shade_body<true, false>(sc, P, Q, cnt, Q.cur, 0u, Q.counts[PT_Q_CUR], &Q.counts[PT_Q_TICKET]);
}
PT_KERNEL void __launch_bounds__(PT_BLOCK, PT_WIDE_KERNEL_WAVES) k_shade_all_sph(PtScene sc, PtPaths P, PtQueues Q, PtCounters* cnt) {
    shade_body<true, true>(sc, P, Q, cnt, Q.cur, 0u, Q.counts[PT_Q_CUR], &Q.counts[PT_Q_TICKET]);
}
PT_KERNEL void __launch_bounds__(PT_BLOCK, PT_SHADE_TEX_WAVES) k_shade_env(PtScene sc, PtPaths P, PtQueues Q, PtCounters* cnt) {
    shade_body<true, true, true, false, false, true>(sc, P, Q, cnt, Q.cur, 0u, Q.counts[PT_Q_CUR], &Q.counts[PT_Q_TICKET]);
}
PT_KERNEL void __launch_bounds__(PT_BLOCK, PT_WIDE_KERNEL_WAVES) k_shade_env_inst(PtScene sc, PtPaths P, PtQueues Q, PtCounters* cnt) {
    shade_body<true, true, true, true, false, true>(sc, P, Q, cnt, Q.cur, 0u, Q.counts[PT_Q_CUR], &Q.counts[PT_Q_TICKET]);
}
PT_KERNEL void __launch_bounds__(PT_BLOCK, PT_SHADE_TEX_WAVES) k_shade_delta(PtScene sc, PtPaths P, PtQueues Q, PtCounters* cnt) {
    shade_body<true, true, true, false, false, true, true>(sc, P, Q, cnt, Q.cur, 0u, Q.counts[PT_Q_CUR], &Q.counts[PT_Q_TICKET]);
}
PT_KERNEL void __launch_bounds__(PT_BLOCK, PT_WIDE_KERNEL_WAVES) k_shade_delta_inst(PtScene sc, PtPaths P, PtQueues Q, PtCounters* cnt) {
    shade_body<true, true, true, true, false, true, true>(sc, P, Q, cnt, Q.cur, 0u, Q.counts[PT_Q_CUR], &Q.counts[PT_Q_TICKET]);
}
PT_KERNEL void __launch_bounds__(PT_BLOCK, PT_SHADE_TEX_WAVES) k_shade_mix(PtScene sc, PtPaths P, PtQueues Q, PtCounters* cnt) {
    shade_body<true, true, true, false, false, true, true, true>(sc, P, Q, cnt, Q.cur, 0u, Q.counts[PT_Q_CUR], &Q.counts[PT_Q_TICKET]);
}
PT_KERNEL void __launch_bounds__(PT_BLOCK, PT_WIDE_KERNEL_WAVES) k_shade_mix_inst(PtScene sc, PtPaths P, PtQueues Q, PtCounters* cnt) {
    shade_body<true, true, true, true, false, true, true, true>(sc, P, Q, cnt, Q.cur, 0u, Q.counts[PT_Q_CUR], &Q.counts[PT_Q_TICKET]);
}

PT_DEV V3 validate_radiance(V3 l) {
    if (!finite3(l)) return mk3(0.0f, 0.0f, 0.0f);
    float y = lum_y(l);
    if (y < -1e-5f) return mk3(0.0f, 0.0f, 0.0f);
// ... 21 lines not shown
    for (int32_t y = p0y; y < p1y; y++)
        for (int32_t x = p0x; x < p1x; x++) {
            float w = film_weight(fm, x, y, pf);
            sum += w;
            if (w != 0.0f) nz++;
        }
    if (sum <= 0.0f) return;
    float isum = 1.0f / sum;
    int32_t width = fm.crop[2] - fm.crop[0];
    for (int32_t y = p0y; y < p1y; y++)
        for (int32_t x = p0x; x < p1x; x++) {
            float w = film_weight(fm, x, y, pf);
            if (w == 0.0f) continue;
            w *= isum;
            V3 cadd = (l * 1.0f) * w;
            if (nz == 1 && x == px && y == py) {
                own_acc.x += cadd.x; own_acc.y += cadd.y; own_acc.z += cadd.z; own_acc.w += w;
            } else {
                float* dst = reinterpret_cast<float*>(spill + (size_t)(y - fm.crop[1]) * width + (x - fm.crop[0]));
                atomicAdd(dst + 0, cadd.x); atomicAdd(dst + 1, cadd.y); atomicAdd(dst + 2, cadd.z); atomicAdd(dst + 3, w);
            }
        }
}
PT_KERNEL void __launch_bounds__(PT_BLOCK) k_film(PtScene sc, PtPaths P, const uint32_t* pixels, uint32_t n_pix, uint32_t n_samples,
                                                             float4* own, float4* spill, float* radiance_out, uint32_t s0, uint32_t spp_total) {
    for (uint32_t j = blockIdx.x * blockDim.x + threadIdx.x; j < n_pix; j += gridDim.x * blockDim.x) {
        uint32_t pk = pixels[j];
        int32_t px = (int32_t)(pk & 0xffffu) + sc.film.sample_bounds[0], py = (int32_t)(pk >> 16) + sc.film.sample_bounds[1];
        bool inside = px >= sc.film.crop[0] && px < sc.film.crop[2] && py >= sc.film.crop[1] && py < sc.film.crop[3];
        size_t fidx = inside ? (size_t)(py - sc.film.crop[1]) * (sc.film.crop[2] - sc.film.crop[0]) + (px - sc.film.crop[0]) : 0;
        float4 acc = inside ? own[fidx] : make_float4(0.0f, 0.0f, 0.0f, 0.0f);
        for (uint32_t k = 0; k < n_samples; k++) {
            size_t path = (size_t)k * n_pix + j;
            float4 L4 = P.L[path];
            V3 l = validate_radiance(mk3(L4.x, L4.y, L4.z));
            if (radiance_out) {
                float* ro = radiance_out + ((size_t)j * spp_total + (s0 + k)) * 3;
                ro[0] = l.x; ro[1] = l.y; ro[2] = l.z;
            }
            float2 pf = P.p_film[path];
            film_add(sc.film, spill, inside ? px : -0x7fffffff, py, mk2(pf.x, pf.y), l, acc);
        }
        if (inside) own[fidx] = acc;
    }
}
PT_KERNEL void k_film_xyzw(const float4* own, const float4* spill, float4* xyzw, uint32_t n) {
    for (uint32_t i = blockIdx.x * blockDim.x + threadIdx.x; i < n; i += gridDim.x * blockDim.x) {
        float4 a = own[i], b = spill[i];
        V3 xa = rgb_to_xyz(mk3(a.x, a.y, a.z)), xb = rgb_to_xyz(mk3(b.x, b.y, b.z));
        xyzw[i] = make_float4(xa.x + xb.x, xa.y + xb.y, xa.z + xb.z, a.w + b.w);
    }
}
PT_KERNEL void k_film_add(float4* xyzw, const float4* other, uint32_t n) {
    for (uint32_t i = blockIdx.x * blockDim.x + threadIdx.x; i < n; i += gridDim.x * blockDim.x) {
        float4 a = xyzw[i], b = other[i];
        xyzw[i] = make_float4(a.x + b.x, a.y + b.y, a.z + b.z, a.w + b.w);
    }
}
PT_KERNEL void k_film_rgb(const float4* xyzw, float* rgb, uint32_t n, float scale) {
    for (uint32_t i = blockIdx.x * blockDim.x + threadIdx.x; i < n; i += gridDim.x * blockDim.x) {
        float4 v = xyzw[i];
        V3 c = xyz_to_rgb(mk3(v.x, v.y, v.z));
        if (v.w > 0.0f) {
            float inv = 1.0f / v.w;
            c = mk3(fmaxf(0.0f, c.x * inv), fmaxf(0.0f, c.y * inv), fmaxf(0.0f, c.z * inv));
        }
        rgb[3 * (size_t)i + 0] = (c.x + 0.0f) * scale;
// ... 86 lines not shown
        float avg = sum / (float)(128u * nl);
        float min_contrib = avg > 0.0f ? 0.001f * avg : 1.0f;
        for (uint32_t j = 0; j < nl; j++) func[j] = fmaxf(min_contrib, func[j]);
        cdf[0] = 0.0f;
        for (uint32_t j = 1; j < nl + 1; j++) cdf[j] = cdf[j - 1] + func[j - 1] / (float)nl;
        float func_int = cdf[nl];
        if (func_int == 0.0f) for (uint32_t j = 1; j < nl + 1; j++) cdf[j] = (float)j / (float)nl;
        else for (uint32_t j = 1; j < nl + 1; j++) cdf[j] /= func_int;
        cdf[nl + 1] = func_int;
    }
}
PT_KERNEL __launch_bounds__(128) void k_light_grid(PtScene sc, float* data, uint32_t n_vox, const uint32_t* vox_list) { light_grid_sums<false>(sc, data, n_vox, vox_list); }
PT_KERNEL __launch_bounds__(128) void k_light_grid_sph(PtScene sc, float* data, uint32_t n_vox, const uint32_t* vox_list) { light_grid_sums<true>(sc, data, n_vox, vox_list); }
PT_KERNEL __launch_bounds__(128) void k_light_grid_env(PtScene sc, float* data, uint32_t n_vox, const uint32_t* vox_list) { light_grid_sums<true, true>(sc, data, n_vox, vox_list); }
PT_DEV uint32_t grid_voxel_of(const PtLightGrid& g, V3 p) {
    uint32_t pi[3];
    float pc[3] = {p.x, p.y, p.z};
    for (int i = 0; i < 3; i++) {
        float o = pc[i] - g.wb_min[i];
        if (g.wb_max[i] > g.wb_min[i]) o = o / (g.wb_max[i] - g.wb_min[i]);
        o = clampf(o, 0.0f, 1.0f);
        float f = o * (float)g.voxels[i];
        uint32_t v = f > 0.0f ? (uint32_t)f : 0u;
        if (v > g.voxels[i] - 1) v = g.voxels[i] - 1;
        pi[i] = v;
    }
    return (pi[2] * g.voxels[1] + pi[1]) * g.voxels[0] + pi[0];
}
template <bool SPH, bool INST>
PT_DEV void grid_mark_body(const PtScene& sc, const PtPaths& P, const PtQueues& Q, int32_t* row_of, uint32_t* todo, uint32_t* todo_count) {
    const uint32_t n = Q.counts[PT_Q_CUR];
    for (uint32_t i = blockIdx.x * blockDim.x + threadIdx.x; i < n; i += gridDim.x * blockDim.x) {
        const uint32_t p = Q.cur[i];
        const int32_t rec = P.hit_rec[p];
        if (rec < 0) continue;
        const V3 ro = f4_3(P.ray_o[p]), rd = f4_3(P.ray_d[p]);
        Surf s;
        float thit;
        bool found;
        if constexpr (INST) found = make_surf_inst<SPH>(sc, ro, rd, (uint32_t)rec, P.hit_inst[p], s, &thit);
        else found = make_surf_any<SPH>(sc, ro, rd, (uint32_t)rec, s, &thit);
        if (!found) continue;
        const uint32_t vox = grid_voxel_of(sc.grid, s.p);
        if (row_of[vox] == -1 && atomicCAS(&row_of[vox], -1, -2) == -1) todo[atomicAdd(todo_count, 1u)] = vox;
    }
}
PT_KERNEL void __launch_bounds__(PT_BLOCK) k_grid_mark(PtScene sc, PtPaths P, PtQueues Q, int32_t* row_of, uint32_t* todo, uint32_t* todo_count) {
    grid_mark_body<false, false>(sc, P, Q, row_of, todo, todo_count);
}
PT_KERNEL void __launch_bounds__(PT_BLOCK) k_grid_mark_sph(PtScene sc, PtPaths P, PtQueues Q, int32_t* row_of, uint32_t* todo, uint32_t* todo_count) {
    grid_mark_body<true, false>(sc, P, Q, row_of, todo, todo_count);
}
PT_KERNEL void __launch_bounds__(PT_BLOCK) k_grid_mark_inst(PtScene sc, PtPaths P, PtQueues Q, int32_t* row_of, uint32_t* todo, uint32_t* todo_count) {
    grid_mark_body<true, true>(sc, P, Q, row_of, todo, todo_count);
}
PT_KERNEL void k_grid_assign(int32_t* row_of, const uint32_t* todo, uint32_t n, uint32_t row0, uint32_t* todo_count) {
    const uint32_t i = blockIdx.x * blockDim.x + threadIdx.x;
    if (i < n) row_of[todo[i]] = (int32_t)(row0 + i);
    if (i == 0) *todo_count = 0;
}
PT_KERNEL void k_light_grid_cdf(PtScene sc, float* data, uint32_t n_vox) { light_grid_cdf(sc, data, n_vox); }

PT_KERNEL void k_camera_rays(PtScene sc, uint32_t n, const int32_t* pixel_xy, const uint32_t* sample_index, float* out_o, float* out_d,
                                         float* out_pf) {
    for (uint32_t i = blockIdx.x * blockDim.x + threadIdx.x; i < n; i += gridDim.x * blockDim.x) {
        int32_t px = pixel_xy[2 * i], py = pixel_xy[2 * i + 1];
        Sampler sm;
        sm.index = sampler_index(sc, sample_index[i], px, py);
        sm.dim = 0; sm.px = px; sm.py = py;
// ... 165 lines not shown
    nd.gb.lobes = m->lobes; nd.gb.n_lobes = m->n_lobes;
    if constexpr (MIX) {
        nd.gb.scales = nullptr;
        const PtMaterial& m0 = sc.materials[nd.s.material];
        if (m0.mix1) {
            if (m0.textured) { nd.gb.lobes = nd.mh.lobes; nd.gb.scales = &nd.mh.scales; }
            else { const PtMix& mx = material_mix(sc, m0); nd.gb.lobes = mx.lobes; nd.gb.n_lobes = mx.n_lobes; nd.gb.scales = &mx.scales; }
        }
    }
    nd.bsdf_eta = m->bsdf_eta;
    nd.spec_mask = m->spec_mask;
}
PT_DEV float4* rec_frame(const PtRec& R, uint32_t depth, uint32_t k, uint32_t p) { return R.frames + ((size_t)depth * PT_REC_FRAME_F4 + k) * R.n_paths + p; }
template <bool FULL, bool ENV = false, bool MIX = false>
PT_DEV uint32_t rec_estimate_direct(const PtScene& sc, const PtRec& R, const RecNodeT<MIX>& nd, uint32_t light_num, V2 u_light, V2 u_scat, uint32_t e, float divisor = 1.0f) {
    const Surf& s = nd.s;
    const PtLight& lt = sc.lights[light_num];
    const uint32_t kNoSpec = PT_BSDF_ALL & ~PT_BSDF_SPECULAR;
    uint32_t nee = light_num << 8;
    V3 A = mk3(0.0f, 0.0f, 0.0f), B = A;
    V3 li, wi, lp, lperr, ln;
    float lpdf;
    bool sampled;
    if constexpr (ENV) sampled = light_sample_kind<FULL, true>(sc, lt, s.p, s.p_error, s.n, u_light, &li, &wi, &lpdf, &lp, &lperr, &ln);
    else sampled = light_sample_any<FULL>(sc, lt, s.p, s.p_error, s.n, u_light, &li, &wi, &lpdf, &lp, &lperr, &ln);
    if (sampled) {
        if (lpdf > 0.0f && !is_black(li)) {
            V3 f = xbsdf_f(nd.gb, s.wo, wi, kNoSpec) * abs_dot(wi, s.sh_n);
            float spdf = xbsdf_pdf(nd.gb, s.wo, wi, kNoSpec);
            if (!is_black(f)) {
                V3 origin = offset_ray_origin(s.p, s.p_error, s.n, lp - s.p);
                V3 target = offset_ray_origin(lp, lperr, ln, origin - lp);
                V3 sd = target - origin;
                R.sh_o[e] = make_float4(origin.x, origin.y, origin.z, 1.0f - PT_SHADOW_EPS);
                R.sh_d[e] = make_float4(sd.x, sd.y, sd.z, 0.0f);
                if (light_is_delta<ENV>(lt)) A = f * li / lpdf;
                else {
                    float weight = power_heuristic(lpdf, spdf);
                    A = f * li * (weight / lpdf);
                }
                nee |= PT_NEE_SHADOW;
            }
        }
    }
    V3 f2, wi2;
    float spdf2;
    uint32_t type2;
    if (!light_is_delta<ENV>(lt) && xbsdf_sample_f(nd.gb, s.wo, u_scat, kNoSpec, &f2, &wi2, &spdf2, &type2)) {
        V3 f = f2 * abs_dot(wi2, s.sh_n);
        if (!is_black(f) && spdf2 > 0.0f) {
            V3 po = offset_ray_origin(s.p, s.p_error, s.n, wi2);
            Surf ls;
            float lt_t;
            bool env_done = false;
            if constexpr (ENV) {
                if (lt.mesh_flags & PT_LIGHT_INFINITE) {
                    env_done = true;
                    const PtEnvLight& en = scene_envs(sc)[__float_as_uint(lt.p0[0])];
                    const float lp2 = env_pdf_li(en, wi2);
                    if (lp2 != 0.0f) {
                        const float weight = power_heuristic(spdf2, lp2);
                        const V3 le = env_le(sc, en, wi2);
                        B = f * le * 1.0f * (weight / spdf2);
                        R.pr_o[e] = make_float4(po.x, po.y, po.z, PT_INF);
                        R.pr_d[e] = make_float4(wi2.x, wi2.y, wi2.z, 0.0f);
                        nee |= PT_NEE_PROBE;
                    }
                }
            }
            if (!env_done && make_surf_any<FULL>(sc, po, wi2, lt.tri_rec, ls, &lt_t)) {
                float lp2 = distance_squared(s.p, ls.p) / (abs_dot(ls.n, -wi2) * lt.area);
                if (isinf(lp2)) lp2 = 0.0f;
                if (lp2 != 0.0f) {
                    float weight = power_heuristic(spdf2, lp2);
                    V3 le = light_L(lt, ls.n, -wi2);
                    B = f * le * 1.0f * (weight / spdf2);
                    R.pr_o[e] = make_float4(po.x, po.y, po.z, PT_INF);
                    R.pr_d[e] = make_float4(wi2.x, wi2.y, wi2.z, 0.0f);
                    nee |= PT_NEE_PROBE;
                }
            }
        }
    }
    R.A[e] = make_float4(A.x, A.y, A.z, divisor);
    R.B[e] = make_float4(B.x, B.y, B.z, 0.0f);
    R.flags[e] = nee;
    return nee;
}
PT_KERNEL void __launch_bounds__(PT_BLOCK) k_rec_init(PtScene sc, PtPaths P, PtRec R, uint32_t n) {
    for (uint32_t p = blockIdx.x * blockDim.x + threadIdx.x; p < n; p += gridDim.x * blockDim.x) {
        Sampler sl;
        sl.index = P.sobol_index[p];
        sl.dim = 2;
        const uint32_t pk = P.pixel[p];
        sl.px = (int32_t)(pk & 0xffffu) + sc.film.sample_bounds[0];
        sl.py = (int32_t)(pk >> 16) + sc.film.sample_bounds[1];
        V2 u_lens = mk2(0.0f, 0.0f);
        if (sc.cam.lens_radius > 0.0f) u_lens = sl.get_2d(sc);
        const float2 pf = P.p_film[p];
        RayDiffs rdf;
        camera_differentials(sc, mk2(pf.x, pf.y), u_lens, f4_3(P.ray_o[p]), f4_3(P.ray_d[p]), rdf);
        R.diff[p] = make_float4(rdf.rx_o.x, rdf.rx_o.y, rdf.rx_o.z, 0.0f);
        R.diff[(size_t)R.n_paths + p] = make_float4(rdf.ry_o.x, rdf.ry_o.y, rdf.ry_o.z, 0.0f);
        R.diff[2 * (size_t)R.n_paths + p] = make_float4(rdf.rx_d.x, rdf.rx_d.y, rdf.rx_d.z, 0.0f);
        R.diff[3 * (size_t)R.n_paths + p] = make_float4(rdf.ry_d.x, rdf.ry_d.y, rdf.ry_d.z, 0.0f);
        P.state[p] = (5u + 2u * R.n_arrays) | (0u << 16) | (PT_ST_DIFF << 24);
        P.nee[p] = 0;
    }
}
PT_DEV RayDiffs rec_load_diff(const PtRec& R, uint32_t p) {
    RayDiffs d;
    d.rx_o = f4_3(R.diff[p]); d.ry_o = f4_3(R.diff[(size_t)R.n_paths + p]);
    d.rx_d = f4_3(R.diff[2 * (size_t)R.n_paths + p]); d.ry_d = f4_3(R.diff[3 * (size_t)R.n_paths + p]);
    return d;
}
template <bool FULL, bool ENV = false, bool MIX = false>
PT_DEV void rec_enter_body(const PtScene& sc, const PtPaths& P, const PtQueues& Q, const PtQueues& Qn, const PtRec& R, PtCounters* cnt) {
    const uint32_t n = Q.counts[PT_Q_CUR];
    const uint32_t lane = threadIdx.x & 63, wave = threadIdx.x >> 6;
    const bool whitted = sc.integrator == PT_INTEGRATOR_WHITTED;
    uint32_t n_vert = 0;
    __shared__ uint32_t s_ws[PT_BLOCK / 64], s_wp[PT_BLOCK / 64], s_qbase[2];
    for (uint32_t bbase = blockIdx.x * blockDim.x; bbase < n; bbase += gridDim.x * blockDim.x) {
        const uint32_t i = bbase + threadIdx.x;
        uint32_t ns = 0, np = 0, e_first = 0;
        if (i < n) {
        const uint32_t p = Q.cur[i];
        const V3 ro = f4_3(P.ray_o[p]), rd = f4_3(P.ray_d[p]);
        const int32_t rec = P.hit_rec[p];
        const uint32_t inst = sc.n_instances ? P.hit_inst[p] : 0u;
        uint32_t st = P.state[p];
        uint32_t dim = st & 0xffffu, depth = (st >> 16) & 0xffu, flags = (st >> 24) & 3u;
        const bool has_diff = (flags & PT_ST_DIFF) != 0;
        RayDiffs rdf;
        rdf.rx_o = rdf.ry_o = rdf.rx_d = rdf.ry_d = mk3(0.0f, 0.0f, 0.0f);
        if (has_diff) rdf = rec_load_diff(R, p);
        RecNodeT<MIX> nd;
        rec_build<FULL, MIX>(sc, ro, rd, rec, inst, has_diff, rdf, nd);
        uint32_t outcome = PT_REC_OUT_FRAME;
        if (!nd.found) outcome = PT_REC_OUT_RETURN0;
        else if (!nd.has_bsdf) {
            if (whitted) outcome = PT_REC_OUT_RETURN0;
            else {
                const V3 no = offset_ray_origin(nd.s.p, nd.s.p_error, nd.s.n, rd);
                P.ray_o[p] = make_float4(no.x, no.y, no.z, PT_INF);
                flags &= ~PT_ST_DIFF;
                outcome = PT_REC_OUT_RETRACE;
            }
        }
        if (outcome == PT_REC_OUT_FRAME) {
            n_vert++;
            Sampler sm;
            sm.index = P.sobol_index[p];
            sm.dim = dim;
            const uint32_t pk = P.pixel[p];
            sm.px = (int32_t)(pk & 0xffffu) + sc.film.sample_bounds[0];
            sm.py = (int32_t)(pk >> 16) + sc.film.sample_bounds[1];
            V3 l = mk3(0.0f, 0.0f, 0.0f);
            const uint32_t e0 = p * R.epp;
            if (whitted) {
                for (uint32_t j = 0; j < sc.n_lights; j++) {
                    const V2 u = sm.get_2d(sc);
                    const PtLight& lt = sc.lights[j];
                    uint32_t nee = j << 8;
                    V3 A = mk3(0.0f, 0.0f, 0.0f);
                    V3 li, wi, lp, lperr, ln;
                    float lpdf;
                    bool sampled;
                    if constexpr (ENV) sampled = light_sample_kind<FULL, true>(sc, lt, nd.s.p, nd.s.p_error, nd.s.n, u, &li, &wi, &lpdf, &lp, &lperr, &ln);
                    else sampled = light_sample_any<FULL>(sc, lt, nd.s.p, nd.s.p_error, nd.s.n, u, &li, &wi, &lpdf, &lp, &lperr, &ln);
                    if (sampled && !(lpdf <= 0.0f || is_black(li))) {
                        V3 f = xbsdf_f(nd.gb, nd.s.wo, wi, PT_BSDF_ALL);
                        if (!is_black(f)) {
                            V3 origin = offset_ray_origin(nd.s.p, nd.s.p_error, nd.s.n, lp - nd.s.p);
                            V3 target = offset_ray_origin(lp, lperr, ln, origin - lp);
                            V3 sd = target - origin;
                            R.sh_o[e0 + j] = make_float4(origin.x, origin.y, origin.z, 1.0f - PT_SHADOW_EPS);
                            R.sh_d[e0 + j] = make_float4(sd.x, sd.y, sd.z, 0.0f);
                            A = f * li * (abs_dot(wi, nd.n_before) / lpdf);
                            nee |= PT_NEE_SHADOW;
                        }
                    }
                    R.A[e0 + j] = make_float4(A.x, A.y, A.z, 1.0f);
                    R.flags[e0 + j] = nee;
                }
            } else {
                if (nd.s.light >= 0) l = light_L(sc.lights[nd.s.light], nd.s.n, nd.s.wo);
                if (sc.n_lights > 0) {
                    if (sc.direct_strategy == PT_DIRECT_ALL) {
                        uint32_t arr = P.nee[p], off = 0;
                        const uint64_t sample_num = (uint64_t)R.s0 + p / R.n_pix;
                        for (uint32_t j = 0; j < sc.n_lights; j++) {
                            const uint32_t n = sc.lights[j].n_samples;
                            if (arr + 2u <= R.n_arrays) {
                                arr += 2u;
                                for (uint32_t k = 0; k < n; k++) {
                                    const uint64_t idx = n == 1u ? sm.index : sampler_index(sc, sample_num * n + k, sm.px, sm.py);
                                    const V2 u = mk2(sample_dimension(sc, idx, 5u, sm.px, sm.py), sample_dimension(sc, idx, 6u, sm.px, sm.py));
                                    rec_estimate_direct<FULL, ENV, MIX>(sc, R, nd, j, u, u, e0 + off + k, (float)n);
                                }
                            } else {
                                arr = R.n_arrays;
                                const V2 u_light = sm.get_2d(sc);
                                const V2 u_scat = sm.get_2d(sc);
                                rec_estimate_direct<FULL, ENV, MIX>(sc, R, nd, j, u_light, u_scat, e0 + off, 1.0f);
                                for (uint32_t k = 1; k < n; k++) R.flags[e0 + off + k] = 0u;
                            }
                            off += n;
                        }
                        P.nee[p] = arr;
                    } else {
                        const float fl = sm.get_1d(sc) * (float)sc.n_lights;
                        uint32_t light_num = fl > 0.0f ? (fl >= 4294967296.0f ? 0xffffffffu : (uint32_t)fl) : 0u;
                        if (light_num > sc.n_lights - 1u) light_num = sc.n_lights - 1u;
                        const float light_pdf = 1.0f / (float)sc.n_lights;
                        const V2 u_light = sm.get_2d(sc);
                        const V2 u_scat = sm.get_2d(sc);
                        rec_estimate_direct<FULL, ENV, MIX>(sc, R, nd, light_num, u_light, u_scat, e0);
                        float4 a = R.A[e0];
                        a.w = light_pdf;
                        R.A[e0] = a;
                    }
                }
            }
            dim = sm.dim;
            if (sc.sobol.kind == PT_SAMPLER_HALTON && dim > sc.sobol.h_n_dims) atomicOr(R.panic, 4u);
            *rec_frame(R, depth, 0, p) = make_float4(ro.x, ro.y, ro.z, __uint_as_float((uint32_t)rec));
            *rec_frame(R, depth, 1, p) = make_float4(rd.x, rd.y, rd.z, __uint_as_float(inst | (has_diff ? 0x80000000u : 0u)));
            *rec_frame(R, depth, 2, p) = make_float4(rdf.rx_o.x, rdf.rx_o.y, rdf.rx_o.z, 0.0f);
            *rec_frame(R, depth, 3, p) = make_float4(rdf.ry_o.x, rdf.ry_o.y, rdf.ry_o.z, __uint_as_float(nd.spec_mask));
            *rec_frame(R, depth, 4, p) = make_float4(rdf.rx_d.x, rdf.rx_d.y, rdf.rx_d.z, 0.0f);
            *rec_frame(R, depth, 5, p) = make_float4(rdf.ry_d.x, rdf.ry_d.y, rdf.ry_d.z, 0.0f);
            *rec_frame(R, depth, 6, p) = make_float4(l.x, l.y, l.z, 0.0f);
        }
        if constexpr (ENV) {
            if (outcome == PT_REC_OUT_RETURN0) {
                const V3 le = nd.found ? mk3(0.0f, 0.0f, 0.0f) : (rec < 0 ? env_le_all(sc, rd) : mk3(0.0f, 0.0f, 0.0f));
                *rec_frame(R, depth, 6, p) = make_float4(le.x, le.y, le.z, 0.0f);
            }
        }
        P.state[p] = (dim & 0xffffu) | (depth << 16) | ((flags | (outcome << 2)) << 24);
        if (outcome == PT_REC_OUT_FRAME) {
            e_first = p * R.epp;
            for (uint32_t j = 0; j < R.epp; j++) { const uint32_t fl = R.flags[e_first + j]; ns += (fl & PT_NEE_SHADOW) ? 1u : 0u; np += (fl & PT_NEE_PROBE) ? 1u : 0u; }
        }
        }
        uint32_t is = ns, ip = np;
        for (int o = 1; o < 64; o <<= 1) {
            const uint32_t a = (uint32_t)__shfl_up((int)is, o, 64), b = (uint32_t)__shfl_up((int)ip, o, 64);
            if ((int)lane >= o) { is += a; ip += b; }
        }
        if (lane == 63u) { s_ws[wave] = is; s_wp[wave] = ip; }
        __syncthreads();
        if (threadIdx.x == 0) {
            uint32_t ts = 0, tp = 0;
            for (uint32_t w = 0; w < PT_BLOCK / 64; w++) { ts += s_ws[w]; tp += s_wp[w]; }
            s_qbase[0] = ts ? atomicAdd(&Qn.counts[PT_Q_SHADOW], ts) : 0u;
            s_qbase[1] = tp ? atomicAdd(&Qn.counts[PT_Q_PROBE], tp) : 0u;
        }
        __syncthreads();
        if (ns | np) {
            uint32_t os = s_qbase[0] + (is - ns), op = s_qbase[1] + (ip - np);
            for (uint32_t w = 0; w < wave; w++) { os += s_ws[w]; op += s_wp[w]; }
            for (uint32_t j = 0; j < R.epp; j++) {
                const uint32_t e = e_first + j, fl = R.flags[e];
                if (fl & PT_NEE_SHADOW) {
                    Qn.shadow[os] = e;
                    if (Qn.shadow_key) { const float4 o4 = R.sh_o[e], d4 = R.sh_d[e]; Qn.shadow_key[os] = ray_sort_key(sc, mk3(o4.x, o4.y, o4.z), mk3(d4.x, d4.y, d4.z)); }
                    os++;
                }
                if (fl & PT_NEE_PROBE) Qn.probe[op++] = e;
            }
        }
        __syncthreads();
    }
    __shared__ unsigned long long s_vert;
    if (threadIdx.x == 0) s_vert = 0;
    __syncthreads();
    if (n_vert) atomicAdd(&s_vert, (unsigned long long)n_vert);
    __syncthreads();
    if (threadIdx.x == 0 && s_vert) atomicAdd(&cnt->vertices, s_vert);
}
PT_KERNEL void __launch_bounds__(PT_BLOCK, PT_WIDE_KERNEL_WAVES) k_rec_enter(PtScene sc, PtPaths P, PtQueues Q, PtQueues Qn, PtRec R, PtCounters* cnt) {
    rec_enter_body<true>(sc, P, Q, Qn, R, cnt);
}
PT_KERNEL void __launch_bounds__(PT_BLOCK, PT_WIDE_KERNEL_WAVES) k_rec_enter_plain(PtScene sc, PtPaths P, PtQueues Q, PtQueues Qn, PtRec R, PtCounters* cnt) {
    rec_enter_body<false>(sc, P, Q, Qn, R, cnt);
}
PT_KERNEL void __launch_bounds__(PT_BLOCK, PT_WIDE_KERNEL_WAVES) k_rec_enter_env(PtScene sc, PtPaths P, PtQueues Q, PtQueues Qn, PtRec R, PtCounters* cnt) {
    rec_enter_body<true, true>(sc, P, Q, Qn, R, cnt);
}
template <bool FULL, bool MIX = false>
PT_DEV bool rec_sample_child(const PtScene& sc, const PtPaths& P, const PtRec& R, uint32_t p, uint32_t depth, bool transmit, Sampler& sm, V3* pend_f, float* pend_scale, uint32_t* child_flags) {
    if (!(__float_as_uint(rec_frame(R, depth, 3, p)->w) & (transmit ? 2u : 1u))) { sm.dim += 2; return false; }
    const float4 f0 = *rec_frame(R, depth, 0, p), f1 = *rec_frame(R, depth, 1, p);
    const V3 ro = f4_3(f0), rd = f4_3(f1);
    const int32_t rec = (int32_t)__float_as_uint(f0.w);
    const uint32_t iw = __float_as_uint(f1.w);
    const bool has_diff = (iw & 0x80000000u) != 0;
    RayDiffs rdf;
    rdf.rx_o = f4_3(*rec_frame(R, depth, 2, p)); rdf.ry_o = f4_3(*rec_frame(R, depth, 3, p));
    rdf.rx_d = f4_3(*rec_frame(R, depth, 4, p)); rdf.ry_d = f4_3(*rec_frame(R, depth, 5, p));
    RecNodeT<MIX> nd;
    rec_build<FULL, MIX>(sc, ro, rd, rec, iw & 0x7fffffffu, has_diff, rdf, nd);
    const V2 u = sm.get_2d(sc);
    V3 f, wi;
    float pdf;
    uint32_t ty;
    if (!xbsdf_sample_f(nd.gb, nd.s.wo, u, (transmit ? PT_BSDF_TRANSMISSION : PT_BSDF_REFLECTION) | PT_BSDF_SPECULAR, &f, &wi, &pdf, &ty)) return false;
    const Surf& s = nd.s;
    const V3 wo = s.wo;
    V3 ns = s.sh_n;
    float wi_ns = abs_dot(wi, ns);
    float wo_ns = dot(wo, ns);
    if (!(pdf > 0.0f && !is_black(f) && wi_ns != 0.0f)) return false;
    const V3 no = offset_ray_origin(s.p, s.p_error, s.n, wi);
    P.ray_o[p] = make_float4(no.x, no.y, no.z, PT_INF);
    P.ray_d[p] = make_float4(wi.x, wi.y, wi.z, 0.0f);
    *child_flags = 0;
    if (has_diff) {
        const V3 rx_o = s.p + nd.th.dpdx, ry_o = s.p + nd.th.dpdy;
        V3 dndx = s.sh_dndu * nd.th.dudx + s.sh_dndv * nd.th.dvdx;
        V3 dndy = s.sh_dndu * nd.th.dudy + s.sh_dndv * nd.th.dvdy;
        V3 rx_d, ry_d;
        if (!transmit) {
            const V3 dwodx = -rdf.rx_d - wo, dwody = -rdf.ry_d - wo;
            const float d_dndx = dot(dwodx, ns) + dot(wo, dndx);
            const float d_dndy = dot(dwody, ns) + dot(wo, dndy);
            rx_d = wi - dwodx + 2.0f * (wo_ns * dndx + d_dndx * ns);
            ry_d = wi - dwody + 2.0f * (wo_ns * dndy + d_dndy * ns);
        } else {
            float eta = 1.0f / nd.bsdf_eta;
            if (dot(wo, ns) < 0.0f) {
                eta = 1.0f / eta;
                ns = -ns; dndx = -dndx; dndy = -dndy;
                wi_ns = abs_dot(wi, ns);
                wo_ns = dot(wo, ns);
            }
            const V3 dwodx = -rdf.rx_d - wo, dwody = -rdf.ry_d - wo;
            const float d_dndx = dot(dwodx, ns) + dot(wo, dndx);
            const float d_dndy = dot(dwody, ns) + dot(wo, dndy);
            const float mu = eta * wo_ns - wi_ns;
            const float dmudx = (eta - (eta * eta * wo_ns) / wi_ns) * d_dndx;
            const float dmudy = (eta - (eta * eta * wo_ns) / wi_ns) * d_dndy;
            rx_d = wi - eta * dwodx + (mu * dndx + dmudx * ns);
            ry_d = wi - eta * dwody + (mu * dndy + dmudy * ns);
        }
        R.diff[p] = make_float4(rx_o.x, rx_o.y, rx_o.z, 0.0f);
        R.diff[(size_t)R.n_paths + p] = make_float4(ry_o.x, ry_o.y, ry_o.z, 0.0f);
        R.diff[2 * (size_t)R.n_paths + p] = make_float4(rx_d.x, rx_d.y, rx_d.z, 0.0f);
        R.diff[3 * (size_t)R.n_paths + p] = make_float4(ry_d.x, ry_d.y, ry_d.z, 0.0f);
// ... 6 lines not shown
template <bool FULL, bool ENV = false, bool MIX = false>
PT_DEV void rec_next_body(const PtScene& sc, const PtPaths& P, const PtQueues& Q, const PtRec& R) {
    const uint32_t n = Q.counts[PT_Q_CUR];
    const uint32_t lane = threadIdx.x & 63;
    const unsigned long long below = (lane == 0) ? 0ull : (~0ull >> (64 - lane));
    const bool whitted = sc.integrator == PT_INTEGRATOR_WHITTED;
    __shared__ uint32_t s_e[PT_SHADE_FLUSH][PT_BLOCK];
    uint32_t n_batch = 0, want = 0;
    auto flush = [&]() {
        if (n_batch == 0) return;
        uint32_t tc = 0;
#pragma unroll
        for (uint32_t j = 0; j < PT_SHADE_FLUSH; j++)
            if (j < n_batch) tc += (uint32_t)__popcll(__ballot(((want >> j) & 1u) != 0));
        uint32_t bc = 0;
        if (lane == 0 && tc) bc = atomicAdd(&Q.counts[PT_Q_NEXT], tc);
        bc = (uint32_t)__builtin_amdgcn_readfirstlane((int)bc);
#pragma unroll
        for (uint32_t j = 0; j < PT_SHADE_FLUSH; j++)
            if (j < n_batch) {
                const bool w = ((want >> j) & 1u) != 0;
                const unsigned long long mc = __ballot(w);
                if (w) Q.next[bc + (uint32_t)__popcll(mc & below)] = s_e[j][threadIdx.x];
                bc += (uint32_t)__popcll(mc);
            }
        n_batch = 0; want = 0;
    };
    for (uint32_t base = (blockIdx.x * blockDim.x + threadIdx.x) - lane; base < n; base += gridDim.x * blockDim.x) {
        const uint32_t i = base + lane;
        bool cont = false;
        uint32_t p = 0;
        if (i < n) {
            p = Q.cur[i];
            uint32_t st = P.state[p];
            uint32_t dim = st & 0xffffu, depth = (st >> 16) & 0xffu, flags = (st >> 24) & 3u;
            const uint32_t outcome = (st >> 26) & 3u;
            if (outcome == PT_REC_OUT_RETRACE) cont = true;
            else {
                Sampler sm;
                sm.index = P.sobol_index[p];
                sm.dim = dim;
                const uint32_t pk = P.pixel[p];
                sm.px = (int32_t)(pk & 0xffffu) + sc.film.sample_bounds[0];
                sm.py = (int32_t)(pk >> 16) + sc.film.sample_bounds[1];
                V3 v = mk3(0.0f, 0.0f, 0.0f);
                bool returning = outcome == PT_REC_OUT_RETURN0;
                if constexpr (ENV) { if (returning) v = f4_3(*rec_frame(R, depth, 6, p)); }
                int32_t d = returning ? (int32_t)depth - 1 : (int32_t)depth;
                uint32_t phase = 0;
                V3 l = mk3(0.0f, 0.0f, 0.0f);
                if (!returning) {
                    l = f4_3(*rec_frame(R, depth, 6, p));
                    const uint32_t e0 = p * R.epp;
                    if (whitted) {
                        for (uint32_t j = 0; j < sc.n_lights; j++) {
                            const uint32_t fl = R.flags[e0 + j];
                            V3 term = mk3(0.0f, 0.0f, 0.0f);
                            if ((fl & PT_NEE_SHADOW) && R.occ[e0 + j] == 0) term = f4_3(R.A[e0 + j]);
                            l = l + term;
                        }
                    } else if (sc.n_lights > 0) {
                        V3 ld_all = mk3(0.0f, 0.0f, 0.0f);
                        const bool all = sc.direct_strategy == PT_DIRECT_ALL;
                        const uint32_t n_groups = all ? sc.n_lights : 1u;
                        uint32_t off = 0;
                        for (uint32_t j = 0; j < n_groups; j++) {
                            const uint32_t n = all ? sc.lights[j].n_samples : 1u;
                            const float divisor = R.A[e0 + off].w;
                            V3 ld = mk3(0.0f, 0.0f, 0.0f);
                            for (uint32_t k = 0; k < n; k++) {
                                const uint32_t e = e0 + off + k;
                                const uint32_t fl = R.flags[e];
                                V3 est = mk3(0.0f, 0.0f, 0.0f);
                                if ((fl & PT_NEE_SHADOW) && R.occ[e] == 0) est = est + f4_3(R.A[e]);
                                if (fl & PT_NEE_PROBE) {
                                    const int32_t best = R.prec[e];
                                    if constexpr (ENV) {
                                        const PtLight& lt = sc.lights[fl >> 8];
                                        if ((lt.mesh_flags & PT_LIGHT_INFINITE) ? best < 0 : (best >= 0 && (uint32_t)best == lt.tri_rec)) est = est + f4_3(R.B[e]);
                                    } else {
                                        if (best >= 0 && (uint32_t)best == sc.lights[fl >> 8].tri_rec) est = est + f4_3(R.B[e]);
                                    }
                                }
                                ld = ld + est;
                            }
                            if (all) ld_all = ld_all + ld / divisor;
                            else ld_all = ld / divisor;
                            off += n;
                        }
                        l = l + ld_all;
                    }
                }
                for (;;) {
                    if (returning) {
                        if (d < 0) { P.L[p] = make_float4(v.x, v.y, v.z, 0.0f); break; }
                        const float4 fr2 = *rec_frame(R, (uint32_t)d, 2, p);
                        const uint32_t ph = __float_as_uint(fr2.w);
                        const float4 pf = *rec_frame(R, (uint32_t)d, 7, p);
                        const float scale = rec_frame(R, (uint32_t)d, 4, p)->w;
                        l = f4_3(*rec_frame(R, (uint32_t)d, 6, p));
                        l = l + (f4_3(pf) * v) * scale;
                        returning = false;
                        if (ph == 2u) { v = l; returning = true; d--; continue; }
                        phase = 1;
                    }
                    if ((uint32_t)d + 1u < (uint32_t)sc.max_depth) {
                        V3 pend_f;
                        float pend_scale;
                        uint32_t cflags;
                        bool child = false;
                        if (phase == 0) {
                            child = rec_sample_child<FULL, MIX>(sc, P, R, p, (uint32_t)d, false, sm, &pend_f, &pend_scale, &cflags);
                            if (!child) { l = l + mk3(0.0f, 0.0f, 0.0f); phase = 1; }
                        }
                        if (!child && phase == 1) {
                            child = rec_sample_child<FULL, MIX>(sc, P, R, p, (uint32_t)d, true, sm, &pend_f, &pend_scale, &cflags);
                            if (child) phase = 2;
                            else l = l + mk3(0.0f, 0.0f, 0.0f);
                        } else if (child) phase = 1;
                        if (child) {
                            *rec_frame(R, (uint32_t)d, 6, p) = make_float4(l.x, l.y, l.z, 0.0f);
                            *rec_frame(R, (uint32_t)d, 7, p) = make_float4(pend_f.x, pend_f.y, pend_f.z, 0.0f);
                            float4 fr2 = *rec_frame(R, (uint32_t)d, 2, p);
                            fr2.w = __uint_as_float(phase);
                            *rec_frame(R, (uint32_t)d, 2, p) = fr2;
                            float4 fr4 = *rec_frame(R, (uint32_t)d, 4, p);
                            fr4.w = pend_scale;
                            *rec_frame(R, (uint32_t)d, 4, p) = fr4;
                            depth = (uint32_t)d + 1u;
                            flags = cflags;
                            cont = true;
                            break;
                        }
                    }
                    v = l; returning = true; d--;
                }
                dim = sm.dim;
                if (sc.sobol.kind == PT_SAMPLER_HALTON && dim > sc.sobol.h_n_dims) atomicOr(R.panic, 4u);
                P.state[p] = (dim & 0xffffu) | (depth << 16) | (flags << 24);
            }
            if (outcome == PT_REC_OUT_RETRACE) P.state[p] = st & ~(3u << 26);
        }
        s_e[n_batch][threadIdx.x] = p;
        want |= (cont ? 1u : 0u) << n_batch;
        if (++n_batch == PT_SHADE_FLUSH) flush();
    }
    flush();
}
PT_KERNEL void __launch_bounds__(PT_BLOCK, PT_WIDE_KERNEL_WAVES) k_rec_next(PtScene sc, PtPaths P, PtQueues Q, PtRec R) { rec_next_body<true>(sc, P, Q, R); }
PT_KERNEL void __launch_bounds__(PT_BLOCK, PT_WIDE_KERNEL_WAVES) k_rec_next_plain(PtScene sc, PtPaths P, PtQueues Q, PtRec R) { rec_next_body<false>(sc, P, Q, R); }
PT_KERNEL void __launch_bounds__(PT_BLOCK, PT_WIDE_KERNEL_WAVES) k_rec_next_env(PtScene sc, PtPaths P, PtQueues Q, PtRec R) { rec_next_body<true, true>(sc, P, Q, R); }
PT_KERNEL void __launch_bounds__(PT_BLOCK, PT_WIDE_KERNEL_WAVES) k_rec_enter_mix(PtScene sc, PtPaths P, PtQueues Q, PtQueues Qn, PtRec R, PtCounters* cnt) {
    rec_enter_body<true, true, true>(sc, P, Q, Qn, R, cnt);
}
PT_KERNEL void __launch_bounds__(PT_BLOCK, PT_WIDE_KERNEL_WAVES) k_rec_next_mix(PtScene sc, PtPaths P, PtQueues Q, PtRec R) { rec_next_body<true, true, true>(sc, P, Q, R); }
hipError_t ptk_rec_init(hipStream_t st, int grid, const PtScene& sc, const PtPaths& P, const PtRec& R, uint32_t n) {
    hipLaunchKernelGGL(k_rec_init, dim3(grid), dim3(PT_BLOCK), 0, st, sc, P, R, n);
    return hipGetLastError();
}
hipError_t ptk_rec_enter(hipStream_t st, int grid, const PtScene& sc, const PtPaths& P, const PtQueues& Q, const PtQueues& Qn, const PtRec& R, PtCounters* cnt,
                         uint32_t lights_per_node) {
    (void)lights_per_node;
    if (scene_n_mix(sc)) hipLaunchKernelGGL(k_rec_enter_mix, dim3(grid), dim3(PT_BLOCK), 0, st, sc, P, Q, Qn, R, cnt);
    else if (sc.n_envs || sc.n_deltas) hipLaunchKernelGGL(k_rec_enter_env, dim3(grid), dim3(PT_BLOCK), 0, st, sc, P, Q, Qn, R, cnt);
    else if (sc.n_spheres || sc.n_instances || sc.textured) hipLaunchKernelGGL(k_rec_enter, dim3(grid), dim3(PT_BLOCK), 0, st, sc, P, Q, Qn, R, cnt);
    else hipLaunchKernelGGL(k_rec_enter_plain, dim3(grid), dim3(PT_BLOCK), 0, st, sc, P, Q, Qn, R, cnt);
    return hipGetLastError();
}
hipError_t ptk_rec_next(hipStream_t st, int grid, const PtScene& sc, const PtPaths& P, const PtQueues& Q, const PtRec& R) {
    if (scene_n_mix(sc)) hipLaunchKernelGGL(k_rec_next_mix, dim3(grid), dim3(PT_BLOCK), 0, st, sc, P, Q, R);
    else if (sc.n_envs || sc.n_deltas) hipLaunchKernelGGL(k_rec_next_env, dim3(grid), dim3(PT_BLOCK), 0, st, sc, P, Q, R);
    else if (sc.n_spheres || sc.n_instances || sc.textured) hipLaunchKernelGGL(k_rec_next, dim3(grid), dim3(PT_BLOCK), 0, st, sc, P, Q, R);
    else hipLaunchKernelGGL(k_rec_next_plain, dim3(grid), dim3(PT_BLOCK), 0, st, sc, P, Q, R);
    return hipGetLastError();
}

PT_DEV V3 aov_clamp(V3 v, float scale) { return mk3(clampf(v.x, 0.0f, 1.0f), clampf(v.y, 0.0f, 1.0f), clampf(v.z, 0.0f, 1.0f)) * scale; }
PT_DEV V3 aov_v2c(V3 v, float scale) { return aov_clamp(0.5f * v + mk3(0.5f, 0.5f, 0.5f), scale); }
PT_DEV void aov_bump(const PtScene& sc, uint32_t prog, const TexHit& th, Surf& s) {
    float du = 0.5f * (fabsf(th.dudx) + fabsf(th.dudy));
    if (du == 0.0f) du = 0.0005f;
    float dv = 0.5f * (fabsf(th.dvdx) + fabsf(th.dvdy));
    if (dv == 0.0f) dv = 0.0005f;
    TexHit ev = th;
    ev.p = th.p + du * s.sh_dpdu; ev.uv = mk2(s.uv.x + du, s.uv.y + 0.0f);
    const float u_displace = tex_eval(sc.textures, sc.tex_prog + prog, ev, sc.images).x;
    ev.p = th.p + dv * s.sh_dpdv; ev.uv = mk2(s.uv.x + 0.0f, s.uv.y + dv);
    const float v_displace = tex_eval(sc.textures, sc.tex_prog + prog, ev, sc.images).x;
    const float displace = tex_eval(sc.textures, sc.tex_prog + prog, th, sc.images).x;
    const V3 dpdu = s.sh_dpdu + (u_displace - displace) / du * s.sh_n + displace * s.sh_dndu;
    const V3 dpdv = s.sh_dpdv + (v_displace - displace) / dv * s.sh_n + displace * s.sh_dndv;
    s.sh_n = face_forward(normalize(cross(dpdu, dpdv)), s.n);
    s.sh_dpdu = dpdu; s.sh_dpdv = dpdv;
}
template <bool FULL, bool MIX = false>
PT_DEV void aov_body(const PtScene& sc, const PtPaths& P, uint32_t n_paths, int32_t target, float scale, PtCounters* cnt) {
    const uint32_t lane = threadIdx.x & 63;
    for (uint32_t base = (blockIdx.x * blockDim.x + threadIdx.x) - lane; base < n_paths; base += gridDim.x * blockDim.x) {
        const uint32_t p = base + lane;
        bool found = false;
        if (p < n_paths) {
            const int32_t rec = P.hit_rec[p];
            if (rec >= 0) {
                const V3 ro = f4_3(P.ray_o[p]), rd = f4_3(P.ray_d[p]);
                Sampler sl;
                sl.index = P.sobol_index[p];
                sl.dim = 2;
                const uint32_t pk = P.pixel[p];
                sl.px = (int32_t)(pk & 0xffffu) + sc.film.sample_bounds[0];
                sl.py = (int32_t)(pk >> 16) + sc.film.sample_bounds[1];
                V2 u_lens = mk2(0.0f, 0.0f);
                if (sc.cam.lens_radius > 0.0f) u_lens = sl.get_2d(sc);
                const float2 pf = P.p_film[p];
                RayDiffs rdf;
                camera_differentials(sc, mk2(pf.x, pf.y), u_lens, ro, rd, rdf);
                uint32_t inst = 0;
                if constexpr (FULL) inst = sc.n_instances ? P.hit_inst[p] : 0u;
                Surf sf;
                float thit;
                if constexpr (FULL) found = make_surf_inst<true>(sc, ro, rd, (uint32_t)rec, inst, sf, &thit);
                else found = make_surf_any<false>(sc, ro, rd, (uint32_t)rec, sf, &thit);
                if (found) {
                    TexHit th;
                    th.p = sf.p; th.uv = sf.uv;
                    compute_differentials(th, sf.p, sf.n, sf.dpdu, sf.dpdv, true, rdf);
                    if constexpr (FULL) {
                        if constexpr (MIX) {
                            int32_t bm = sf.material;
                            if (bm >= 0 && sc.materials[bm].mix1) bm = material_mix(sc, sc.materials[bm]).leaf_material[0];
                            if (bm >= 0 && sc.materials[bm].textured) {
                                const uint32_t prog = sc.mat_params[bm].prog[8];
                                if (prog) aov_bump(sc, prog, th, sf);
                            }
                        } else
                        if (sf.material >= 0 && sc.materials[sf.material].textured) {
                            const uint32_t prog = sc.mat_params[sf.material].prog[8];
                            if (prog) aov_bump(sc, prog, th, sf);
                        }
                    }
                    V3 l = mk3(0.0f, 0.0f, 0.0f);
                    switch (target) {
                        case PT_AOV_DISTANCE: { const float dist = P.hit_t[p] / length(rd); l = aov_clamp(mk3(dist, dist, dist), scale); break; }
                        case PT_AOV_DEPTH: { const float dist = length(sf.p - ro); l = aov_clamp(mk3(dist, dist, dist), scale); break; }
                        case PT_AOV_N: l = aov_v2c(sf.n, scale); break;
                        case PT_AOV_NS: l = aov_v2c(sf.sh_n, scale); break;
                        case PT_AOV_UV: l = aov_clamp(mk3(sf.uv.x, sf.uv.y, 0.0f), scale); break;
                        case PT_AOV_RDXC: case PT_AOV_DRODX: l = aov_v2c(rdf.rx_o, scale); break;
                        case PT_AOV_DRDDX: l = aov_v2c(rdf.rx_d, scale); break;
                        case PT_AOV_DPDX: l = aov_v2c(th.dpdx, scale); break;
                        case PT_AOV_DPDY: l = aov_v2c(th.dpdy, scale); break;
                        case PT_AOV_DPDU: l = aov_v2c(sf.dpdu, scale); break;
                        case PT_AOV_DPDV: l = aov_v2c(sf.dpdv, scale); break;
                        case PT_AOV_DUVDX: l = aov_v2c(mk3(fabsf(th.dudx), fabsf(th.dvdx), 0.0f), scale); break;
                        case PT_AOV_DUVDY: l = aov_v2c(mk3(fabsf(th.dudy), fabsf(th.dvdy), 0.0f), scale); break;
                        case PT_AOV_DPDUS: l = aov_v2c(sf.sh_dpdu, scale); break;
                        case PT_AOV_DPDVS: l = aov_v2c(sf.sh_dpdv, scale); break;
                        default: break;
                    }
                    P.L[p] = make_float4(l.x, l.y, l.z, 0.0f);
                }
            }
        }
        const uint64_t hits = __ballot(found);
        if (lane == 0 && hits) atomicAdd(&cnt->vertices, (unsigned long long)__popcll(hits));
    }
}
PT_KERNEL void __launch_bounds__(PT_BLOCK, PT_WIDE_KERNEL_WAVES) k_aov(PtScene sc, PtPaths P, uint32_t n_paths, int32_t target, float scale, PtCounters* cnt) {
    aov_body<true>(sc, P, n_paths, target, scale, cnt);
}
PT_KERNEL void __launch_bounds__(PT_BLOCK) k_aov_plain(PtScene sc, PtPaths P, uint32_t n_paths, int32_t target, float scale, PtCounters* cnt) {
    aov_body<false>(sc, P, n_paths, target, scale, cnt);
}
PT_KERNEL void __launch_bounds__(PT_BLOCK, PT_WIDE_KERNEL_WAVES) k_aov_mix(PtScene sc, PtPaths P, uint32_t n_paths, int32_t target, float scale, PtCounters* cnt) {
    aov_body<true, true>(sc, P, n_paths, target, scale, cnt);
}
hipError_t ptk_aov(hipStream_t st, int grid, const PtScene& sc, const PtPaths& P, uint32_t n_paths, int32_t target, float scale, PtCounters* cnt) {
    if (scene_n_mix(sc)) { hipLaunchKernelGGL(k_aov_mix, dim3(grid), dim3(PT_BLOCK), 0, st, sc, P, n_paths, target, scale, cnt); return hipGetLastError(); }
    if (sc.n_spheres || sc.n_instances || sc.textured) hipLaunchKernelGGL(k_aov, dim3(grid), dim3(PT_BLOCK), 0, st, sc, P, n_paths, target, scale, cnt);
    else hipLaunchKernelGGL(k_aov_plain, dim3(grid), dim3(PT_BLOCK), 0, st, sc, P, n_paths, target, scale, cnt);
    return hipGetLastError();
}

#define PT_LAUNCH_CHECK() hipGetLastError()

int ptk_trace_dist_blocks_per_cu() { return PT_TRACE_WIDE ? 1 : PT_TRACE_DIST_WAVES; }
int ptk_trace_wide() { return PT_TRACE_WIDE; }
int ptk_shade_prof_read(unsigned long long* out16) {
#ifdef PT_PROFILE_SHADE
    unsigned long long z[16] = {0, 0, 0, 0, 0, 0, 0, 0, 0, 0, 0, 0, 0, 0, 0, 0};
    if (hipMemcpyFromSymbol(out16, HIP_SYMBOL(g_shade_prof), sizeof(z)) != hipSuccess) return 0;
    (void)hipMemcpyToSymbol(HIP_SYMBOL(g_shade_prof), z, sizeof(z));
    return 1;
// ... 23 lines not shown
    else hipLaunchKernelGGL(k_nee_resolve, dim3(grid), dim3(PT_BLOCK), 0, st, sc, P, Q);
    return PT_LAUNCH_CHECK();
}
PT_KERNEL void __launch_bounds__(PT_BLOCK) k_light_renumber(PtTri* tris, PtTriInfo* tinfo, const PtLight* lights, uint32_t n) {
    const uint32_t i = blockIdx.x * blockDim.x + threadIdx.x;
    if (i >= n || (lights[i].mesh_flags & (PT_LIGHT_INFINITE | PT_LIGHT_DELTA))) return;
    const uint32_t r = lights[i].tri_rec;
    tris[r].light1 = i + 1u;
    if (tinfo) tinfo[r].light = (int32_t)i;
}
hipError_t ptk_light_renumber(hipStream_t st, PtTri* tris, PtTriInfo* tinfo, const PtLight* lights, uint32_t n) {
    if (n == 0) return hipSuccess;
    hipLaunchKernelGGL(k_light_renumber, dim3((n + PT_BLOCK - 1) / PT_BLOCK), dim3(PT_BLOCK), 0, st, tris, tinfo, lights, n);
    return PT_LAUNCH_CHECK();
}
hipError_t ptk_light_hooks(hipStream_t st, const PtScene& sc, uint32_t light, uint32_t mode, uint32_t n, const float* a, const float* b, float* o3a, float* o3b,
                           float* o1) {
    hipLaunchKernelGGL(k_light_hooks, dim3((n + PT_BLOCK - 1) / PT_BLOCK), dim3(PT_BLOCK), 0, st, sc, light, mode, n, a, b, o3a, o3b, o1);
    return PT_LAUNCH_CHECK();
}
hipError_t ptk_light_pdf_from(hipStream_t st, const PtScene& sc, uint32_t light, uint32_t n, const float* ref, const float* wi, float* pdf) {
    hipLaunchKernelGGL(k_light_pdf_from, dim3((n + PT_BLOCK - 1) / PT_BLOCK), dim3(PT_BLOCK), 0, st, sc, light, n, ref, wi, pdf);
    return PT_LAUNCH_CHECK();
}
hipError_t ptk_trace_batch(hipStream_t st, int grid, const PtScene& sc, uint32_t n, const float* o, const float* d, const float* tmax, pt_hit* out,
                           uint8_t* occ, int any_hit, uint32_t* ticket, PtCounters* cnt, uint32_t* spill, uint32_t spill_depth, uint32_t* err, int alpha) {
    if (alpha) hipLaunchKernelGGL(k_trace_batch_alpha, dim3(grid), dim3(PT_BLOCK), 0, st, sc, n, o, d, tmax, out, occ, any_hit, ticket, cnt, spill, spill_depth, err);
    else if (sc.n_instances) hipLaunchKernelGGL(k_trace_batch_inst, dim3(grid), dim3(PT_BLOCK), 0, st, sc, n, o, d, tmax, out, occ, any_hit, ticket, cnt, spill, spill_depth, err);
    else if (sc.n_spheres) hipLaunchKernelGGL(k_trace_batch_sph, dim3(grid), dim3(PT_BLOCK), 0, st, sc, n, o, d, tmax, out, occ, any_hit, ticket, cnt, spill, spill_depth, err);
    else hipLaunchKernelGGL(k_trace_batch, dim3(grid), dim3(PT_BLOCK), 0, st, sc, n, o, d, tmax, out, occ, any_hit, ticket, cnt, spill, spill_depth, err);
    return PT_LAUNCH_CHECK();
}
template <bool SPH, bool INST>
PT_DEV void ao_rays_body(const PtScene& sc, const PtPaths& P, uint32_t n_paths, float4* ao_o, float4* ao_d, float* ao_w, uint32_t* counter,
                         PtCounters* cnt) {
    const uint32_t lane = threadIdx.x & 63;
    const uint32_t n_s = (uint32_t)sc.ao_samples;
    for (uint32_t base = (blockIdx.x * blockDim.x + threadIdx.x) - lane; base < n_paths; base += gridDim.x * blockDim.x) {
        const uint32_t p = base + lane;
        bool found = false;
        Surf s;
        V3 rd = mk3(0.0f, 0.0f, 1.0f);
        if (p < n_paths) {
            const V3 ro = f4_3(P.ray_o[p]);
            rd = f4_3(P.ray_d[p]);
            const int32_t rec = P.hit_rec[p];
            float thit;
            if constexpr (INST) found = rec >= 0 && make_surf_inst<SPH>(sc, ro, rd, (uint32_t)rec, P.hit_inst[p], s, &thit);
            else found = rec >= 0 && make_surf_any<SPH>(sc, ro, rd, (uint32_t)rec, s, &thit);
        }
        const uint64_t hits = __ballot(found);
        uint32_t slot0 = 0;
        if (lane == 0 && hits) {
            slot0 = atomicAdd(counter, (uint32_t)__popcll(hits));
            atomicAdd(&cnt->vertices, (unsigned long long)__popcll(hits));
        }
        slot0 = (uint32_t)__shfl((int)slot0, 0, 64);
        if (p < n_paths) P.nee[p] = found ? slot0 + (uint32_t)__popcll(hits & ((1ull << lane) - 1ull)) + 1u : 0u;
        if (!found) continue;
        const size_t r0 = (size_t)(slot0 + (uint32_t)__popcll(hits & ((1ull << lane) - 1ull))) * n_s;
        const V3 n = face_forward(s.n, -rd);
        const V3 ss = normalize(s.dpdu);
        const V3 tt = cross(s.n, ss);
        const uint32_t pk = P.pixel[p];
        const int32_t px = (int32_t)(pk & 0xffffu) + sc.film.sample_bounds[0], py = (int32_t)(pk >> 16) + sc.film.sample_bounds[1];
        const uint32_t cam_sample = (uint32_t)P.probe_rec[p];
        for (uint32_t k = 0; k < n_s; k++) {
            const uint64_t index = sampler_index(sc, (uint64_t)cam_sample * n_s + k, px, py);
            const V2 u = mk2(sample_dimension(sc, index, 5u, px, py), sample_dimension(sc, index, 6u, px, py));
            V3 wi;
            float pdf;
            if (sc.ao_cos_sample) { wi = cosine_sample_hemisphere(u); pdf = fabsf(wi.z) * PT_INV_PI; }
            else {
                const float z = u.x, r = sqrtf(fmaxf(0.0f, 1.0f - z * z)), phi = 2.0f * PT_PI * u.y;
                float sn, cs;
                pt_sincosf(phi, &sn, &cs);
                wi = mk3(r * cs, r * sn, z);
                pdf = PT_INV_PI * 0.5f;
            }
            wi = mk3(wi.x * ss.x + wi.y * tt.x + wi.z * n.x, wi.x * ss.y + wi.y * tt.y + wi.z * n.y, wi.x * ss.z + wi.y * tt.z + wi.z * n.z);
            const V3 o = offset_ray_origin(s.p, s.p_error, s.n, wi);
            const size_t r = r0 + k;
            ao_o[r] = make_float4(o.x, o.y, o.z, PT_INF);
            ao_d[r] = make_float4(wi.x, wi.y, wi.z, 0.0f);
            ao_w[r] = dot(wi, n) / (pdf * (float)n_s);
        }
    }
}
PT_KERNEL void __launch_bounds__(PT_BLOCK) k_ao_rays(PtScene sc, PtPaths P, uint32_t n_paths, float4* ao_o, float4* ao_d, float* ao_w,
                                                                uint32_t* counter, PtCounters* cnt) {
    ao_rays_body<false, false>(sc, P, n_paths, ao_o, ao_d, ao_w, counter, cnt);
}
PT_KERNEL void __launch_bounds__(PT_BLOCK) k_ao_rays_sph(PtScene sc, PtPaths P, uint32_t n_paths, float4* ao_o, float4* ao_d, float* ao_w,
                                                                    uint32_t* counter, PtCounters* cnt) {
    ao_rays_body<true, false>(sc, P, n_paths, ao_o, ao_d, ao_w, counter, cnt);
}
PT_KERNEL void __launch_bounds__(PT_BLOCK) k_ao_rays_inst(PtScene sc, PtPaths P, uint32_t n_paths, float4* ao_o, float4* ao_d, float* ao_w,
                                                                     uint32_t* counter, PtCounters* cnt) {
    ao_rays_body<true, true>(sc, P, n_paths, ao_o, ao_d, ao_w, counter, cnt);
}
PT_KERNEL void __launch_bounds__(PT_BLOCK) k_ao_tag(PtPaths P, uint32_t n_pix, uint32_t n_paths, uint32_t s0) {
    for (uint32_t i = blockIdx.x * blockDim.x + threadIdx.x; i < n_paths; i += gridDim.x * blockDim.x) P.probe_rec[i] = (int32_t)(s0 + i / n_pix);
}
PT_KERNEL void __launch_bounds__(PT_BLOCK) k_ao_resolve(PtScene sc, PtPaths P, uint32_t n_paths, const float* ao_w, const uint8_t* occ) {
    const uint32_t n_s = (uint32_t)sc.ao_samples;
    for (uint32_t p = blockIdx.x * blockDim.x + threadIdx.x; p < n_paths; p += gridDim.x * blockDim.x) {
        float l = 0.0f;
        const uint32_t slot1 = P.nee[p];
        if (slot1) {
            const size_t r0 = (size_t)(slot1 - 1u) * n_s;
            for (uint32_t k = 0; k < n_s; k++)
                if (!occ[r0 + k]) l += ao_w[r0 + k];
        }
        P.L[p] = make_float4(l, l, l, 0.0f);
        P.nee[p] = 0;
    }
}
hipError_t ptk_ao_tag(hipStream_t st, int grid, const PtPaths& P, uint32_t n_pix, uint32_t n_paths, uint32_t s0) {
    hipLaunchKernelGGL(k_ao_tag, dim3(grid), dim3(PT_BLOCK), 0, st, P, n_pix, n_paths, s0);
    return PT_LAUNCH_CHECK();
}
hipError_t ptk_ao_rays(hipStream_t st, int grid, const PtScene& sc, const PtPaths& P, uint32_t n_paths, float4* ao_o, float4* ao_d, float* ao_w,
                       uint32_t* counter, PtCounters* cnt) {
    if (sc.n_instances) hipLaunchKernelGGL(k_ao_rays_inst, dim3(grid), dim3(PT_BLOCK), 0, st, sc, P, n_paths, ao_o, ao_d, ao_w, counter, cnt);
    else if (sc.n_spheres) hipLaunchKernelGGL(k_ao_rays_sph, dim3(grid), dim3(PT_BLOCK), 0, st, sc, P, n_paths, ao_o, ao_d, ao_w, counter, cnt);
    else hipLaunchKernelGGL(k_ao_rays, dim3(grid), dim3(PT_BLOCK), 0, st, sc, P, n_paths, ao_o, ao_d, ao_w, counter, cnt);
    return PT_LAUNCH_CHECK();
}
PT_KERNEL void k_ao_queue(PtQueues Q, const uint32_t* counter, uint32_t n_s) {
    if (threadIdx.x == 0 && blockIdx.x == 0) {
        Q.counts[PT_Q_CUR] = 0; Q.counts[PT_Q_SHADOW] = counter[0] * n_s; Q.counts[PT_Q_PROBE] = 0; Q.counts[PT_Q_NEE] = 0;
        for (uint32_t k = 0; k < 8u; k++) Q.counts[PT_Q_SEG_TICKET0 + 32u * k] = 0;
    }
}
PT_KERNEL void __launch_bounds__(PT_BLOCK) k_iota(uint32_t* out, uint32_t n) {
    for (uint32_t i = blockIdx.x * blockDim.x + threadIdx.x; i < n; i += gridDim.x * blockDim.x) out[i] = i;
}
hipError_t ptk_ao_queue(hipStream_t st, const PtQueues& Q, const uint32_t* counter, uint32_t n_s) {
    hipLaunchKernelGGL(k_ao_queue, dim3(1), dim3(64), 0, st, Q, counter, n_s);
    return PT_LAUNCH_CHECK();
}
hipError_t ptk_iota(hipStream_t st, int grid, uint32_t* out, uint32_t n) {
    hipLaunchKernelGGL(k_iota, dim3(grid), dim3(PT_BLOCK), 0, st, out, n);
    return PT_LAUNCH_CHECK();
}
hipError_t ptk_ao_resolve(hipStream_t st, int grid, const PtScene& sc, const PtPaths& P, uint32_t n_paths, const float* ao_w, const uint8_t* occ) {
    hipLaunchKernelGGL(k_ao_resolve, dim3(grid), dim3(PT_BLOCK), 0, st, sc, P, n_paths, ao_w, occ);
    return PT_LAUNCH_CHECK();
}
hipError_t ptk_gen(hipStream_t st, int grid, const PtScene& sc, const PtPaths& P, const PtQueues& Q, const uint32_t* pixels, uint32_t n_pix,
                   uint32_t s0, uint32_t n_samples, PtCounters* cnt) {
    hipLaunchKernelGGL(k_gen, dim3(grid), dim3(PT_BLOCK), 0, st, sc, P, Q, pixels, n_pix, s0, n_samples, cnt);
    return PT_LAUNCH_CHECK();
}
hipError_t ptk_prep(hipStream_t st, const PtQueues& Q, int mode) {
    hipLaunchKernelGGL(k_prep, dim3(1), dim3(64), 0, st, Q, mode);
    return PT_LAUNCH_CHECK();
}
hipError_t ptk_shade(hipStream_t st, int grid, const PtScene& sc, const PtPaths& P, const PtQueues& Q, PtCounters* cnt, int local_sort) {
// ... 114 lines not shown
```

pbrt-r3_amd/csrc/pt_kernels_decl.inc:

```
hipError_t ptk_trace(hipStream_t st, int grid, int grid_dist, const PtScene& sc, const PtPaths& P, const PtQueues& Q, PtCounters* cnt, uint32_t* spill,
                     uint32_t spill_depth, uint32_t* err, int far, int alpha);
bool ptk_trace_has_far(const PtScene& sc);
hipError_t ptk_trace_batch(hipStream_t st, int grid, const PtScene& sc, uint32_t n, const float* o, const float* d, const float* tmax, pt_hit* out,
                           uint8_t* occ, int any_hit, uint32_t* ticket, PtCounters* cnt, uint32_t* spill, uint32_t spill_depth, uint32_t* err, int alpha);
hipError_t ptk_gen(hipStream_t st, int grid, const PtScene& sc, const PtPaths& P, const PtQueues& Q, const uint32_t* pixels, uint32_t n_pix,
                   uint32_t s0, uint32_t n_samples, PtCounters* cnt);
hipError_t ptk_nee_resolve(hipStream_t st, int grid, const PtScene& sc, const PtPaths& P, const PtQueues& Q);
hipError_t ptk_light_renumber(hipStream_t st, PtTri* tris, PtTriInfo* tinfo, const PtLight* lights, uint32_t n);
hipError_t ptk_light_hooks(hipStream_t st, const PtScene& sc, uint32_t light, uint32_t mode, uint32_t n, const float* a, const float* b, float* o3a, float* o3b,
                           float* o1);
hipError_t ptk_light_pdf_from(hipStream_t st, const PtScene& sc, uint32_t light, uint32_t n, const float* ref, const float* wi, float* pdf);
hipError_t ptk_prep(hipStream_t st, const PtQueues& Q, int mode);
hipError_t ptk_shade(hipStream_t st, int grid, const PtScene& sc, const PtPaths& P, const PtQueues& Q, PtCounters* cnt, int local_sort = 0);
int ptk_trace_wide();
hipError_t ptk_film(hipStream_t st, int grid, const PtScene& sc, const PtPaths& P, const uint32_t* pixels, uint32_t n_pix, uint32_t n_samples,
                    float4* own, float4* spill, float* radiance_out, uint32_t s0, uint32_t spp_total);
hipError_t ptk_film_xyzw(hipStream_t st, const float4* own, const float4* spill, float4* xyzw, uint32_t n);
hipError_t ptk_film_add(hipStream_t st, float4* xyzw, const float4* other, uint32_t n);
hipError_t ptk_film_rgb(hipStream_t st, const float4* xyzw, float* rgb, uint32_t n, float scale);
hipError_t ptk_light_grid(hipStream_t st, const PtScene& sc, float* data, uint32_t n_vox, const uint32_t* vox_list = nullptr);
hipError_t ptk_grid_mark(hipStream_t st, int grid, const PtScene& sc, const PtPaths& P, const PtQueues& Q, int32_t* row_of, uint32_t* todo, uint32_t* todo_count);
hipError_t ptk_grid_assign(hipStream_t st, int32_t* row_of, const uint32_t* todo, uint32_t n, uint32_t row0, uint32_t* todo_count);
hipError_t ptk_camera_rays(hipStream_t st, const PtScene& sc, uint32_t n, const int32_t* pixel_xy, const uint32_t* sample_index, float* o, float* d,
                           float* pf);
hipError_t ptk_bsdf_eval(hipStream_t st, const PtScene& sc, uint32_t material, uint32_t n, const float* wo, const float* wi, uint32_t flags, float* f,
                         float* pdf);
hipError_t ptk_bsdf_sample(hipStream_t st, const PtScene& sc, uint32_t material, uint32_t n, const float* wo, const float* u, uint32_t flags, float* f,
                           float* wi, float* pdf, uint32_t* type);
hipError_t ptk_sobol_samples(hipStream_t st, const PtScene& sc, uint32_t n, const int32_t* pixel_xy, const uint32_t* sample_index, const uint32_t* dim,
                             float* out);
hipError_t ptk_ao_tag(hipStream_t st, int grid, const PtPaths& P, uint32_t n_pix, uint32_t n_paths, uint32_t s0);
hipError_t ptk_ao_rays(hipStream_t st, int grid, const PtScene& sc, const PtPaths& P, uint32_t n_paths, float4* ao_o, float4* ao_d, float* ao_w,
                       uint32_t* counter, PtCounters* cnt);
hipError_t ptk_ao_queue(hipStream_t st, const PtQueues& Q, const uint32_t* counter, uint32_t n_s);
hipError_t ptk_iota(hipStream_t st, int grid, uint32_t* out, uint32_t n);
hipError_t ptk_ao_resolve(hipStream_t st, int grid, const PtScene& sc, const PtPaths& P, uint32_t n_paths, const float* ao_w, const uint8_t* occ);
hipError_t ptk_aov(hipStream_t st, int grid, const PtScene& sc, const PtPaths& P, uint32_t n_paths, int32_t target, float scale, PtCounters* cnt);
hipError_t ptk_expand_tiles(hipStream_t st, const int4* tiles, const uint32_t* tile_off, uint32_t n_tiles, int32_t sb_x0, int32_t sb_y0, uint32_t sb_w,
                            uint32_t* pixels, uint32_t* bitmap, uint32_t* err);
hipError_t ptk_wavefront_results(hipStream_t st, int grid, const PtScene& sc, const PtPaths& P, uint32_t n, const uint8_t* kind, pt_hit* out, uint8_t* occ);
int ptk_shade_prof_read(unsigned long long* out16);
size_t ptk_sort_rays_temp_bytes(uint32_t cap);
hipError_t ptk_sort_shadow_rays(hipStream_t st, uint32_t* ids, uint32_t* ids_alt, uint32_t* keys, uint32_t* keys_alt, void* temp, size_t temp_bytes, uint32_t n,
                                uint32_t** sorted);
hipError_t ptk_cont_keys(hipStream_t st, int grid, const PtScene& sc, const PtPaths& P, const uint32_t* list, uint32_t n, uint32_t* keys);
size_t ptk_sort_rays_keep_temp_bytes(uint32_t cap);
hipError_t ptk_sort_rays_keep(hipStream_t st, const uint32_t* ids, uint32_t* ids_out, const uint32_t* keys, uint32_t* keys_out, void* temp, size_t temp_bytes, uint32_t n);
int ptk_trace_dist_blocks_per_cu();
hipError_t ptk_rec_init(hipStream_t st, int grid, const PtScene& sc, const PtPaths& P, const PtRec& R, uint32_t n);
hipError_t ptk_rec_enter(hipStream_t st, int grid, const PtScene& sc, const PtPaths& P, const PtQueues& Q, const PtQueues& Qn, const PtRec& R, PtCounters* cnt,
                         uint32_t lights_per_node);
hipError_t ptk_rec_next(hipStream_t st, int grid, const PtScene& sc, const PtPaths& P, const PtQueues& Q, const PtRec& R);
```

Measured before the change: 1199.

## Convert path pool from structure-of-arrays to per-path array-of-structs records

Replaces the separate per-field path arrays (ray origin, direction, beta, sobol index, pixel, state, hit t/rec, shadow and probe rays, pend A/L) with packed 64/32/8-byte records, accessed through inline accessor methods. The intent is that a thread touching one path reads one or two contiguous cache lines instead of many scattered arrays, especially in traversal where origin and direction are loaded together. The cost is that coalescing changes for kernels that read only one field across a wavefront, so they now fetch strided data. It also adds an asm barrier in the AOV distance path.

```diff
diff --git a/pbrt-r3_amd/csrc/pt_context.cpp b/pbrt-r3_amd/csrc/pt_context.cpp
--- a/pbrt-r3_amd/csrc/pt_context.cpp
+++ b/pbrt-r3_amd/csrc/pt_context.cpp
@@ -210,25 +210,20 @@
         ctx->paths.tex_res = nullptr;
     }
     if (ctx->pool_paths >= n_paths && ctx->d_pool.p) return PT_OK;
-    const size_t per_path = 11 * 16 + 8 + 8 + 6 * 4 + 4;
-    PT_HIP(ctx->d_pool.alloc(n_paths * per_path + 16384));
+    const PtPoolLayout lay = pt_pool_layout(n_paths);
+    if (lay.end > lay.bytes) return ctx->fail(PT_ERR_DEVICE, "internal: path pool carve overflow");
+    PT_HIP(ctx->d_pool.alloc(lay.bytes));
     char* base = ctx->d_pool.as<char>();
-    size_t off = 0;
-    auto carve = [&](size_t elem) { void* p = base + off; off += (n_paths * elem + 255) & ~(size_t)255; return p; };
     PtPaths& P = ctx->paths;
-    P.ray_o = (float4*)carve(16); P.ray_d = (float4*)carve(16);
-    P.sh_o = (float4*)carve(16); P.sh_d = (float4*)carve(16);
-    P.pr_o = (float4*)carve(16); P.pr_d = (float4*)carve(16);
-    P.beta = (float4*)carve(16); P.L = (float4*)carve(16);
-    P.pendA = (float4*)carve(16); P.pendB = (float4*)carve(16); P.pbeta = (float4*)carve(16);
-    P.p_film = (float2*)carve(8);
-    P.sobol_index = (uint64_t*)carve(8);
-    P.pixel = (uint32_t*)carve(4); P.state = (uint32_t*)carve(4);
-    P.hit_t = (float*)carve(4); P.hit_rec = (int32_t*)carve(4);
-    P.nee = (uint32_t*)carve(4);
-    P.probe_rec = (int32_t*)carve(4);
-    P.occluded = (uint8_t*)carve(1);
-    if (off > ctx->d_pool.bytes) return ctx->fail(PT_ERR_DEVICE, "internal: path pool carve overflow");
+    P.ray = (PtRayRec*)(base + lay.ray);
+    P.shadow = (PtSegRec*)(base + lay.shadow); P.probe = (PtSegRec*)(base + lay.probe);
+    P.pend = (PtPendRec*)(base + lay.pend);
+    P.pendB = (float4*)(base + lay.pendB); P.pbeta = (float4*)(base + lay.pbeta);
+    P.p_film = (float2*)(base + lay.p_film);
+    P.hit = (PtHitRec*)(base + lay.hit);
+    P.nee = (uint32_t*)(base + lay.nee);
+    P.probe_rec = (int32_t*)(base + lay.probe_rec);
+    P.occluded = (uint8_t*)(base + lay.occluded);
     PT_HIP(ctx->d_qa.alloc(n_paths * 4));
     PT_HIP(ctx->d_qb.alloc(n_paths * 4));
     PT_HIP(ctx->d_qnee.alloc(n_paths * 4));
@@ -1982,7 +1977,7 @@
     {
         size_t free_b = 0, total_b = 0;
         if (hipMemGetInfo(&free_b, &total_b) == hipSuccess) {
-            size_t per_path = 11 * 16 + 8 + 8 + 6 * 4 + 4 + 6 * 4 + 4 * 4;
+            size_t per_path = PT_POOL_PER_PATH + 6 * 4 + 4 * 4;
             if (sc.textured && !sc.n_instances) per_path += PT_TEX_RES_F4 * 16;
             if (ctx->sort_cont != 0) per_path += 4 * 4;
             if (rec) {
@@ -2099,9 +2094,8 @@
                     ctx->ao_rays_cap = cap;
                     PT_HIP(ptk_iota(ctx->stream, ctx->grid_wide, reinterpret_cast<uint32_t*>(ctx->d_ao.as<char>() + ctx->ao_rays_cap * 36), (uint32_t)cap));
                 }
-                float4* ao_o = ctx->d_ao.as<float4>();
-                float4* ao_d = ao_o + ctx->ao_rays_cap;
-                float* ao_w = reinterpret_cast<float*>(ao_d + ctx->ao_rays_cap);
+                PtSegRec* ao_ray = ctx->d_ao.as<PtSegRec>();
+                float* ao_w = reinterpret_cast<float*>(ao_ray + ctx->ao_rays_cap);
                 uint32_t* ao_ids = reinterpret_cast<uint32_t*>(ao_w + ctx->ao_rays_cap);
                 uint8_t* ao_occ = reinterpret_cast<uint8_t*>(ao_ids + ctx->ao_rays_cap);
                 uint32_t* ao_count = ctx->d_ticket.as<uint32_t>() + 2;
@@ -2114,10 +2108,10 @@
                 PT_HIP(hipEventRecord(a, ctx->stream));
                 PT_HIP(ptk_trace_any(ctx, ctx->stream, ctx->grid_trace, ctx->grid_trace_dist, sc, ctx->paths, Q, cnt, ctx->d_spill.as<uint32_t>(), ctx->spill_depth, err, 0, ctx->scene_alpha ? 1 : 0));
                 ctx->trace_launches++;
-                PT_HIP(ptk_ao_rays_any(ctx, ctx->stream, ctx->grid_wide, sc, ctx->paths, n_paths, ao_o, ao_d, ao_w, ao_count, cnt));
+                PT_HIP(ptk_ao_rays_any(ctx, ctx->stream, ctx->grid_wide, sc, ctx->paths, n_paths, ao_ray, ao_w, ao_count, cnt));
                 {
                     PtPaths AP = ctx->paths;
-                    AP.sh_o = ao_o; AP.sh_d = ao_d; AP.occluded = ao_occ;
+                    AP.shadow = ao_ray; AP.occluded = ao_occ;
                     PtQueues AQ = Q;
                     AQ.shadow = ao_ids;
                     PT_HIP(ptk_ao_queue(ctx->stream, AQ, ao_count, (uint32_t)sc.ao_samples));
@@ -2153,7 +2147,7 @@
                 auto take = [&](size_t bytes) { char* q = rb; rb += (bytes + 255) & ~(size_t)255; return q; };
                 R.diff = (float4*)take(np * 64);
                 R.frames = (float4*)take(np * (size_t)rec_depth * PT_REC_FRAME_F4 * 16);
-                R.sh_o = (float4*)take(ne * 16); R.sh_d = (float4*)take(ne * 16); R.pr_o = (float4*)take(ne * 16); R.pr_d = (float4*)take(ne * 16);
+                R.sh = (PtSegRec*)take(ne * sizeof(PtSegRec)); R.pr = (PtSegRec*)take(ne * sizeof(PtSegRec));
                 R.A = (float4*)take(ne * 16); R.B = (float4*)take(ne * 16);
                 R.panic = err;
                 R.prec = (int32_t*)take(ne * 4); R.flags = (uint32_t*)take(ne * 4);
@@ -2165,7 +2159,7 @@
                 R.s0 = s0; R.n_pix = n_pix;
                 if (5u + 2u * R.n_arrays > 60000u) return ctx->fail(PT_ERR_UNSUPPORTED, "directlighting \"all\": too many lights x maxdepth for the sampler's array dimensions");
                 PtPaths NP = ctx->paths;
-                NP.sh_o = R.sh_o; NP.sh_d = R.sh_d; NP.pr_o = R.pr_o; NP.pr_d = R.pr_d; NP.occluded = R.occ; NP.probe_rec = R.prec;
+                NP.shadow = R.sh; NP.probe = R.pr; NP.occluded = R.occ; NP.probe_rec = R.prec;
                 PtQueues Qn = Q;
                 Qn.counts = ctx->d_counts2.as<uint32_t>(); Qn.shadow = nl_shadow; Qn.probe = nl_probe;
                 PT_HIP(ptk_rec_init_any(ctx, ctx->stream, ctx->grid_wide, sc, ctx->paths, R, n_paths));
@@ -2555,24 +2549,22 @@
     if (!ctx->have_scene) return ctx->fail(PT_ERR_NO_SCENE, "no scene uploaded");
     if (n == 0) return PT_OK;
     (void)hipSetDevice(ctx->device);
-    std::vector<float> o4((size_t)n * 4), d4((size_t)n * 4);
+    std::vector<PtSegRec> seg(n);
+    std::vector<PtRayRec> rays(n);
     std::vector<uint32_t> ids[3];
     for (uint32_t i = 0; i < n; i++) {
         if (kind[i] < 1 || kind[i] > 3) return ctx->fail(PT_ERR_INVALID_ARGUMENT, "ray kind must be 1 (continuation), 2 (shadow) or 3 (probe)");
         ids[kind[i] - 1].push_back(i);
-        for (int k = 0; k < 3; k++) { o4[4 * (size_t)i + k] = o[3 * (size_t)i + k]; d4[4 * (size_t)i + k] = d[3 * (size_t)i + k]; }
-        o4[4 * (size_t)i + 3] = tmax[i];
-        d4[4 * (size_t)i + 3] = 0.0f;
+        seg[i].o = make_float4(o[3 * (size_t)i], o[3 * (size_t)i + 1], o[3 * (size_t)i + 2], tmax[i]);
+        seg[i].d = make_float4(d[3 * (size_t)i], d[3 * (size_t)i + 1], d[3 * (size_t)i + 2], 0.0f);
+        rays[i].o = seg[i].o; rays[i].d = seg[i].d;
     }
     pt_status st;
     if ((st = ensure_pool(ctx, std::max<size_t>(n, 65536))) != PT_OK) return st;
     const PtPaths& P = ctx->paths;
-    float4* const dst_o[3] = {P.ray_o, P.sh_o, P.pr_o};
-    float4* const dst_d[3] = {P.ray_d, P.sh_d, P.pr_d};
-    for (int k = 0; k < 3; k++) {
-        PT_HIP(hipMemcpyAsync(dst_o[k], o4.data(), (size_t)n * 16, hipMemcpyHostToDevice, ctx->stream));
-        PT_HIP(hipMemcpyAsync(dst_d[k], d4.data(), (size_t)n * 16, hipMemcpyHostToDevice, ctx->stream));
-    }
+    PT_HIP(hipMemcpyAsync(P.ray, rays.data(), (size_t)n * sizeof(PtRayRec), hipMemcpyHostToDevice, ctx->stream));
+    PT_HIP(hipMemcpyAsync(P.shadow, seg.data(), (size_t)n * sizeof(PtSegRec), hipMemcpyHostToDevice, ctx->stream));
+    PT_HIP(hipMemcpyAsync(P.probe, seg.data(), (size_t)n * sizeof(PtSegRec), hipMemcpyHostToDevice, ctx->stream));
     PtQueues Q;
     Q.cur = ctx->d_qa.as<uint32_t>(); Q.next = ctx->d_qb.as<uint32_t>();
     Q.nee = ctx->d_qnee.as<uint32_t>(); Q.counts = ctx->d_counts.as<uint32_t>(); Q.sorted = ctx->d_qsorted.as<uint32_t>();
diff --git a/pbrt-r3_amd/csrc/pt_device.h b/pbrt-r3_amd/csrc/pt_device.h
--- a/pbrt-r3_amd/csrc/pt_device.h
+++ b/pbrt-r3_amd/csrc/pt_device.h
@@ -1,4 +1,5 @@
 #pragma once
+#include <stddef.h>
 #include <stdint.h>
 #include "../../include/pbrtgpu.h"
 
@@ -319,37 +320,98 @@
 static_assert(sizeof(PtDeltaLight) == 80 && sizeof(PtEnvLight) % 8 == 0 && sizeof(PtLight) % 16 == 0, "side records of the light buffer");
 static_assert(__builtin_offsetof(PtScene, nodes) == 16, "n_deltas fills the hole in front of PtScene::nodes");
 
+struct alignas(64) PtRayRec {
+    float4 o;
+    float4 d;
+    float4 beta;
+    uint64_t sobol_index;
+    uint32_t pixel;
+    uint32_t state;
+};
+struct alignas(32) PtSegRec {
+    float4 o;
+    float4 d;
+};
+struct alignas(32) PtPendRec {
+    float4 A;
+    float4 L;
+};
+struct alignas(8) PtHitRec {
+    float t;
+    int32_t rec;
+};
+static_assert(sizeof(PtRayRec) == 64 && __builtin_offsetof(PtRayRec, o) == 0 && __builtin_offsetof(PtRayRec, d) == 16 && __builtin_offsetof(PtRayRec, beta) == 32 &&
+              __builtin_offsetof(PtRayRec, sobol_index) == 48 && __builtin_offsetof(PtRayRec, pixel) == 56 && __builtin_offsetof(PtRayRec, state) == 60, "ray record");
+static_assert(sizeof(PtSegRec) == 32 && __builtin_offsetof(PtSegRec, o) == 0 && __builtin_offsetof(PtSegRec, d) == 16, "shadow / probe record");
+static_assert(sizeof(PtPendRec) == 32 && __builtin_offsetof(PtPendRec, A) == 0 && __builtin_offsetof(PtPendRec, L) == 16, "pend record");
+static_assert(sizeof(PtHitRec) == 8 && __builtin_offsetof(PtHitRec, t) == 0 && __builtin_offsetof(PtHitRec, rec) == 4, "hit record");
+
+#if defined(__HIPCC__) || defined(__CUDACC__)
+#define PT_PATHS_FN __host__ __device__ __forceinline__
+#else
+#define PT_PATHS_FN inline
+#endif
 struct PtPaths {
-    float4* ray_o;
-    float4* ray_d;
-    float4* sh_o;
-    float4* sh_d;
-    float4* pr_o;
-    float4* pr_d;
-    float4* beta;
-    float4* L;
-    float4* pendA;
+    PtRayRec* ray;
+    PtSegRec* shadow;
+    PtSegRec* probe;
+    PtPendRec* pend;
+    PtHitRec* hit;
     float4* pendB;
     float4* pbeta;
     float2* p_film;
-    uint64_t* sobol_index;
-    uint32_t* pixel;
-    uint32_t* state;
-    float* hit_t;
-    int32_t* hit_rec;
     uint32_t* nee;
     uint8_t* occluded;
     int32_t* probe_rec;
     uint32_t* hit_inst;
     float4* tex_res;
-};
+    PT_PATHS_FN float4& ray_o(uint32_t p) const { return ray[p].o; }
+    PT_PATHS_FN float4& ray_d(uint32_t p) const { return ray[p].d; }
+    PT_PATHS_FN float4& beta(uint32_t p) const { return ray[p].beta; }
+    PT_PATHS_FN uint64_t& sobol_index(uint32_t p) const { return ray[p].sobol_index; }
+    PT_PATHS_FN uint32_t& pixel(uint32_t p) const { return ray[p].pixel; }
+    PT_PATHS_FN uint32_t& state(uint32_t p) const { return ray[p].state; }
+    PT_PATHS_FN float4& sh_o(uint32_t p) const { return shadow[p].o; }
+    PT_PATHS_FN float4& sh_d(uint32_t p) const { return shadow[p].d; }
+    PT_PATHS_FN float4& pr_o(uint32_t p) const { return probe[p].o; }
+    PT_PATHS_FN float4& pr_d(uint32_t p) const { return probe[p].d; }
+    PT_PATHS_FN float4& pendA(uint32_t p) const { return pend[p].A; }
+    PT_PATHS_FN float4& L(uint32_t p) const { return pend[p].L; }
+    PT_PATHS_FN float& hit_t(uint32_t p) const { return hit[p].t; }
+    PT_PATHS_FN int32_t& hit_rec(uint32_t p) const { return hit[p].rec; }
+};
+
+#define PT_POOL_PER_PATH (sizeof(PtRayRec) + 2 * sizeof(PtSegRec) + sizeof(PtPendRec) + sizeof(PtHitRec) + 2 * 16 + 8 + 2 * 4 + 4)
+#define PT_POOL_SLACK 16384u
+struct PtPoolLayout {
+    size_t ray, shadow, probe, pend, pendB, pbeta, p_film, hit, nee, probe_rec, occluded;
+    size_t end;
+    size_t bytes;
+};
+inline PtPoolLayout pt_pool_layout(size_t n_paths) {
+    PtPoolLayout l{};
+    size_t off = 0;
+    auto carve = [&](size_t elem) { const size_t at = off; off += (n_paths * elem + 255) & ~(size_t)255; return at; };
+    l.ray = carve(sizeof(PtRayRec));
+    l.shadow = carve(sizeof(PtSegRec)); l.probe = carve(sizeof(PtSegRec));
+    l.pend = carve(sizeof(PtPendRec));
+    l.pendB = carve(16); l.pbeta = carve(16);
+    l.p_film = carve(8);
+    l.hit = carve(sizeof(PtHitRec));
+    l.nee = carve(4); l.probe_rec = carve(4);
+    l.occluded = carve(1);
+    l.end = off;
+    l.bytes = n_paths * PT_POOL_PER_PATH + PT_POOL_SLACK;
+    return l;
+}
 #define PT_TEX_RES_F4 9u
 
 #define PT_REC_FRAME_F4 8u
 struct PtRec {
     float4* diff;
     float4* frames;
-    float4 *sh_o, *sh_d, *pr_o, *pr_d, *A, *B;
+    PtSegRec *sh, *pr;
+    float4 *A, *B;
     uint8_t* occ;
     int32_t* prec;
     uint32_t* flags;
diff --git a/pbrt-r3_amd/csrc/pt_kernels.hip b/pbrt-r3_amd/csrc/pt_kernels.hip
--- a/pbrt-r3_amd/csrc/pt_kernels.hip
+++ b/pbrt-r3_amd/csrc/pt_kernels.hip
@@ -1033,6 +1033,12 @@
 #ifndef PT_TRACE_DIST_WAVES
 #define PT_TRACE_DIST_WAVES 4
 #endif
+
+PT_DEV const float4* item_ray(const PtPaths& P, int kind, uint32_t p) {
+    const PtSegRec* base = kind == 1 ? reinterpret_cast<const PtSegRec*>(P.ray) : (kind == 2 ? P.shadow : P.probe);
+    return &base[kind == 1 ? (size_t)p * 2u : (size_t)p].o;
+}
+static_assert(sizeof(PtRayRec) == 2 * sizeof(PtSegRec) && __builtin_offsetof(PtRayRec, d) == __builtin_offsetof(PtSegRec, d), "item_ray: a path record's head is a ray record");
 
 #ifndef PT_LEAF_LANES_MIN
 #define PT_LEAF_LANES_MIN 18
@@ -1133,9 +1139,8 @@
             }
         } else if (pf_stage == 2) {
             if (lane < pf_count) {
-                const float4* so = pf_kind == 1 ? P.ray_o : (pf_kind == 2 ? P.sh_o : P.pr_o);
-                const float4* sd = pf_kind == 1 ? P.ray_d : (pf_kind == 2 ? P.sh_d : P.pr_d);
-                pf_o = so[pf_p]; pf_d = sd[pf_p];
+                const float4* ray = item_ray(P, pf_kind, pf_p);
+                pf_o = ray[0]; pf_d = ray[1];
             }
             pf_stage = 3;
         }
@@ -1143,7 +1148,7 @@
         constexpr bool LATE_RETIRE = DIST;
 #define PT_RETIRE()                                                                                                                                      \
         if (kind != 0 && ray_done(r)) {                                                                                                                  \
-            if (kind == 1) { P.hit_t[p] = r.ray_tmax; P.hit_rec[p] = r.best; if (INST && (!ALPHA || sc.n_instances)) P.hit_inst[p] = r.best_inst; }      \
+            if (kind == 1) { PtHitRec& h = P.hit[p]; h.t = r.ray_tmax; h.rec = r.best; if (INST && (!ALPHA || sc.n_instances)) P.hit_inst[p] = r.best_inst; }      \
             else if (kind == 2) P.occluded[p] = r.best >= 0 ? 1 : 0;                                                                                     \
             else P.probe_rec[p] = r.best;                                                                                                                \
             kind = 0;                                                                                                                                    \
@@ -1352,7 +1357,8 @@
                     if (r.top == PT_INST_EXIT_REF) {
                         (void)stk_pop(c, r.top, r.sp);
                         const float w_tmax = __uint_as_float(stk_pop(c, r.top, r.sp)), w_tmin = __uint_as_float(stk_pop(c, r.top, r.sp));
-                        const float4 ro = (kind == 1 ? P.ray_o : (kind == 2 ? P.sh_o : P.pr_o))[p], rd = (kind == 1 ? P.ray_d : (kind == 2 ? P.sh_d : P.pr_d))[p];
+                        const float4* ray = item_ray(P, kind, p);
+                        const float4 ro = ray[0], rd = ray[1];
                         const bool hit_inside = r.best >= 0 && r.best_inst == r.cur_inst;
                         ray_set_direction_state(r, f4_3(ro), mk3(rd.x, rd.y, rd.z));
                         r.tmin = w_tmin; r.tmax = hit_inside ? r.ray_tmax : w_tmax;
@@ -1484,16 +1490,16 @@
         uint8_t oc = 0;
         if (k == 2u) oc = P.occluded[i];
         else {
-            const int32_t rec = k == 1u ? P.hit_rec[i] : P.probe_rec[i];
+            const int32_t rec = k == 1u ? P.hit_rec(i) : P.probe_rec[i];
             if (rec >= 0) {
                 const uint32_t inst = (k == 1u && sc.n_instances) ? P.hit_inst[i] : 0u;
                 TriVerts tv = load_tri(sc.tris, (uint32_t)rec);
                 h.prim = inst ? (int32_t)sc.instances[inst - 1u].world_prim : (int32_t)tv.prim;
                 if (k == 1u) {
-                    h.t = P.hit_t[i];
+                    h.t = P.hit_t(i);
                     if (!inst && !(tv.flags & (PT_TRI_SPHERE | PT_TRI_INSTANCE))) {
                         RayPre rp;
-                        ray_precompute(rp, f4_3(P.ray_o[i]), f4_3(P.ray_d[i]));
+                        ray_precompute(rp, f4_3(P.ray_o(i)), f4_3(P.ray_d(i)));
                         TriHit th;
                         tri_test(rp, tv.p0, tv.p1, tv.p2, tv.flags, PT_INF, th);
                         h.b0 = th.b0; h.b1 = th.b1;
@@ -1546,14 +1552,14 @@
         (void)sm.get_1d(sc);
         V3 o, d;
         generate_camera_ray(sc, p_film, u_lens, &o, &d);
-        P.ray_o[i] = make_float4(o.x, o.y, o.z, PT_INF);
-        P.ray_d[i] = make_float4(d.x, d.y, d.z, 0.0f);
-        P.beta[i] = make_float4(1.0f, 1.0f, 1.0f, 1.0f);
-        P.L[i] = make_float4(0.0f, 0.0f, 0.0f, 0.0f);
+        P.ray_o(i) = make_float4(o.x, o.y, o.z, PT_INF);
+        P.ray_d(i) = make_float4(d.x, d.y, d.z, 0.0f);
+        P.beta(i) = make_float4(1.0f, 1.0f, 1.0f, 1.0f);
+        P.L(i) = make_float4(0.0f, 0.0f, 0.0f, 0.0f);
         P.p_film[i] = make_float2(p_film.x, p_film.y);
-        P.sobol_index[i] = sm.index;
-        P.pixel[i] = pk;
-        P.state[i] = sm.dim | (PT_ST_CAMERA << 24);
+        P.sobol_index(i) = sm.index;
+        P.pixel(i) = pk;
+        P.state(i) = sm.dim | (PT_ST_CAMERA << 24);
         P.nee[i] = 0;
         Q.cur[i] = i;
     }
@@ -2020,12 +2026,12 @@
     const uint32_t n = Q.counts[PT_Q_NEE];
     for (uint32_t i = blockIdx.x * blockDim.x + threadIdx.x; i < n; i += gridDim.x * blockDim.x) {
         const uint32_t p = Q.nee[i];
-        const float4 A = P.pendA[p];
+        const float4 A = P.pendA(p);
         if (__float_as_uint(A.w) == 0u) {
             if (P.occluded[p] == 0) {
-                float4 L = P.L[p];
+                float4 L = P.L(p);
                 L.x += A.x; L.y += A.y; L.z += A.z;
-                P.L[p] = L;
+                P.L(p) = L;
             }
             continue;
         }
@@ -2038,22 +2044,22 @@
         }
         V3 ldn = ld / A.w;
         float4 pb = P.pbeta[p];
-        float4 L = P.L[p];
+        float4 L = P.L(p);
         V3 add = mk3(pb.x, pb.y, pb.z) * ldn;
         L.x += add.x; L.y += add.y; L.z += add.z;
-        P.L[p] = L;
+        P.L(p) = L;
     }
 }
 PT_KERNEL void __launch_bounds__(PT_BLOCK) k_nee_resolve_env(PtScene sc, PtPaths P, PtQueues Q) {
     const uint32_t n = Q.counts[PT_Q_NEE];
     for (uint32_t i = blockIdx.x * blockDim.x + threadIdx.x; i < n; i += gridDim.x * blockDim.x) {
         const uint32_t p = Q.nee[i];
-        const float4 A = P.pendA[p];
+        const float4 A = P.pendA(p);
         if (__float_as_uint(A.w) == 0u) {
             if (P.occluded[p] == 0) {
-                float4 L = P.L[p];
+                float4 L = P.L(p);
                 L.x += A.x; L.y += A.y; L.z += A.z;
-                P.L[p] = L;
+                P.L(p) = L;
             }
             continue;
         }
@@ -2068,15 +2074,15 @@
         }
         V3 ldn = ld / A.w;
         float4 pb = P.pbeta[p];
-        float4 L = P.L[p];
+        float4 L = P.L(p);
         V3 add = mk3(pb.x, pb.y, pb.z) * ldn;
         L.x += add.x; L.y += add.y; L.z += add.z;
-        P.L[p] = L;
+        P.L(p) = L;
     }
 }
 
 PT_DEV uint32_t path_sort_bin(const PtScene& sc, const PtPaths& P, uint32_t p) {
-    int32_t rec = P.hit_rec[p];
+    int32_t rec = P.hit_rec(p);
     if (rec < 0) return 0xffffffffu;
     uint32_t m1 = sc.tris[rec].flags >> PT_TRI_MATERIAL_SHIFT;
     return m1 == 0 ? (sc.n_instances ? PT_SORT_GENERAL0 : 0u) : sc.materials[m1 - 1].sort_bin;
@@ -2521,13 +2527,13 @@
         uint32_t wr = 0, o_nee = 0, o_state = 0;
         float4 o_ray_o = make_float4(0.0f, 0.0f, 0.0f, 0.0f), o_ray_d = o_ray_o, o_beta = o_ray_o;
         auto commit = [&]() {
-            if (wr & 64u) P.pendA[p] = s_stage[4][threadIdx.x];
-            if (wr & 4u) { P.sh_o[p] = s_stage[0][threadIdx.x]; P.sh_d[p] = s_stage[1][threadIdx.x]; }
-            if (wr & 8u) { P.pr_o[p] = s_stage[2][threadIdx.x]; P.pr_d[p] = s_stage[3][threadIdx.x]; }
-            if (wr & 16u) { P.pendA[p] = s_stage[4][threadIdx.x]; P.pendB[p] = s_stage[5][threadIdx.x]; P.pbeta[p] = s_stage[6][threadIdx.x]; P.nee[p] = o_nee; }
-            if (wr & 1u) P.ray_o[p] = o_ray_o;
-            if (wr & 2u) { P.ray_d[p] = o_ray_d; P.beta[p] = o_beta; }
-            if (wr & 32u) P.state[p] = o_state;
+            if (wr & 64u) P.pendA(p) = s_stage[4][threadIdx.x];
+            if (wr & 4u) { P.sh_o(p) = s_stage[0][threadIdx.x]; P.sh_d(p) = s_stage[1][threadIdx.x]; }
+            if (wr & 8u) { P.pr_o(p) = s_stage[2][threadIdx.x]; P.pr_d(p) = s_stage[3][threadIdx.x]; }
+            if (wr & 16u) { P.pendA(p) = s_stage[4][threadIdx.x]; P.pendB[p] = s_stage[5][threadIdx.x]; P.pbeta[p] = s_stage[6][threadIdx.x]; P.nee[p] = o_nee; }
+            if (wr & 1u) P.ray_o(p) = o_ray_o;
+            if (wr & 2u) { P.ray_d(p) = o_ray_d; P.beta(p) = o_beta; }
+            if (wr & 32u) P.state(p) = o_state;
             wr = 0;
         };
 #ifndef PT_DEFER_WIDE
@@ -2548,10 +2554,10 @@
         if (active) {
             p = had_pf ? pf_p_now : list[item];
             PT_SHP_SYNC(13);
-            const float4 ro4 = P.ray_o[p], rd4 = P.ray_d[p], beta4 = P.beta[p];
+            const float4 ro4 = P.ray_o(p), rd4 = P.ray_d(p), beta4 = P.beta(p);
             V3 ro = f4_3(ro4), rd = f4_3(rd4);
-            int32_t rec = had_pf ? pf_rec_now : P.hit_rec[p];
-            uint32_t st = had_pf ? pf_st_now : P.state[p];
+            int32_t rec = had_pf ? pf_rec_now : P.hit_rec(p);
+            uint32_t st = had_pf ? pf_st_now : P.state(p);
             uint32_t dim = st & 0xffffu, bounces = (st >> 16) & 0xffu, flags = st >> 24;
             V3 beta = f4_3(beta4);
             float eta_scale = beta4.w;
@@ -2564,8 +2570,8 @@
             SamplerPre sm;
             sm.s.index = 0; sm.s.dim = dim; sm.s.px = 0; sm.s.py = 0; sm.dim0 = dim; sm.have = false;
             if (rec >= 0 && (int32_t)bounces < sc.max_depth) {
-                sm.s.index = had_pf ? pf_idx_now : P.sobol_index[p];
-                const uint32_t pk = had_pf ? pf_pk_now : P.pixel[p];
+                sm.s.index = had_pf ? pf_idx_now : P.sobol_index(p);
+                const uint32_t pk = had_pf ? pf_pk_now : P.pixel(p);
                 sm.s.px = (int32_t)(pk & 0xffffu) + sc.film.sample_bounds[0];
                 sm.s.py = (int32_t)(pk >> 16) + sc.film.sample_bounds[1];
                 PT_SHP_SYNC(15);
@@ -2579,27 +2585,27 @@
             else found = rec >= 0 && make_surf_any_rec<SPH>(sc, ro, rd, (uint32_t)rec, rec_a, rec_b, rec_c, s, &thit);
             PT_SHP(0);
             if (pf_lane) {
-                pf_rec = P.hit_rec[pf_p];
-                pf_st = P.state[pf_p]; pf_idx = P.sobol_index[pf_p]; pf_pk = P.pixel[pf_p];
+                pf_rec = P.hit_rec(pf_p);
+                pf_st = P.state(pf_p); pf_idx = P.sobol_index(pf_p); pf_pk = P.pixel(pf_p);
             }
             if constexpr (ENV) {
                 if (rec < 0 && (bounces == 0 || (flags & PT_ST_SPECULAR))) {
-                    float4 L = P.L[p];
+                    float4 L = P.L(p);
                     for (uint32_t k = 0; k < sc.n_envs; k++) {
                         const V3 add = beta * env_le(sc, scene_envs(sc)[k], rd);
                         L.x += add.x; L.y += add.y; L.z += add.z;
                     }
-                    P.L[p] = L;
+                    P.L(p) = L;
                 }
             }
             if (found && (bounces == 0 || (flags & PT_ST_SPECULAR))) {
                 int32_t li = s.light;
                 if (li >= 0) {
                     V3 le = light_L(sc.lights[li], s.n, -rd);
-                    float4 L = P.L[p];
+                    float4 L = P.L(p);
                     V3 add = beta * le;
                     L.x += add.x; L.y += add.y; L.z += add.z;
-                    P.L[p] = L;
+                    P.L(p) = L;
                 }
             }
             if (found && (int32_t)bounces < sc.max_depth) {
@@ -2615,9 +2621,9 @@
                         const bool has_diff = (flags & PT_ST_CAMERA) != 0;
                         if (has_diff) {
                             Sampler sl;
-                            sl.index = P.sobol_index[p];
+                            sl.index = P.sobol_index(p);
                             sl.dim = 2;
-                            uint32_t pk2 = P.pixel[p];
+                            uint32_t pk2 = P.pixel(p);
                             sl.px = (int32_t)(pk2 & 0xffffu) + sc.film.sample_bounds[0];
                             sl.py = (int32_t)(pk2 >> 16) + sc.film.sample_bounds[1];
                             V2 u_lens = mk2(0.0f, 0.0f);
@@ -2919,11 +2925,11 @@
     __shared__ float s_texval[3 * PT_TEX_PROG_MAX][PT_BLOCK];
     for (uint32_t i = begin + blockIdx.x * blockDim.x + threadIdx.x; i < end; i += gridDim.x * blockDim.x) {
         const uint32_t p = list[i];
-        const int32_t rec = P.hit_rec[p];
-        const uint32_t st = P.state[p];
+        const int32_t rec = P.hit_rec(p);
+        const uint32_t st = P.state(p);
         const uint32_t bounces = (st >> 16) & 0xffu, flags = st >> 24;
         if (rec < 0 || (int32_t)bounces >= sc.max_depth) continue;
-        const float4 ro4 = P.ray_o[p], rd4 = P.ray_d[p];
+        const float4 ro4 = P.ray_o(p), rd4 = P.ray_d(p);
         const V3 ro = f4_3(ro4), rd = f4_3(rd4);
         const float4* q = reinterpret_cast<const float4*>(sc.tris) + (size_t)(uint32_t)rec * 3;
         const float4 rec_a = q[0], rec_b = q[1], rec_c = q[2];
@@ -2937,9 +2943,9 @@
         const bool has_diff = (flags & PT_ST_CAMERA) != 0;
         if (has_diff) {
             Sampler sl;
-            sl.index = P.sobol_index[p];
+            sl.index = P.sobol_index(p);
             sl.dim = 2;
-            const uint32_t pk2 = P.pixel[p];
+            const uint32_t pk2 = P.pixel(p);
             sl.px = (int32_t)(pk2 & 0xffffu) + sc.film.sample_bounds[0];
             sl.py = (int32_t)(pk2 >> 16) + sc.film.sample_bounds[1];
             V2 u_lens = mk2(0.0f, 0.0f);
@@ -2978,7 +2984,7 @@
 PT_KERNEL void __launch_bounds__(PT_BLOCK) k_cont_keys(PtScene sc, PtPaths P, const uint32_t* list, uint32_t n, uint32_t* keys) {
     for (uint32_t i = blockIdx.x * blockDim.x + threadIdx.x; i < n; i += gridDim.x * blockDim.x) {
         const uint32_t p = list[i];
-        const float4 o = P.ray_o[p], d = P.ray_d[p];
+        const float4 o = P.ray_o(p), d = P.ray_d(p);
         keys[i] = ray_sort_key(sc, mk3(o.x, o.y, o.z), mk3(d.x, d.y, d.z));
     }
 }
@@ -3066,7 +3072,7 @@
         float4 acc = inside ? own[fidx] : make_float4(0.0f, 0.0f, 0.0f, 0.0f);
         for (uint32_t k = 0; k < n_samples; k++) {
             size_t path = (size_t)k * n_pix + j;
-            float4 L4 = P.L[path];
+            float4 L4 = P.L(path);
             V3 l = validate_radiance(mk3(L4.x, L4.y, L4.z));
             if (radiance_out) {
                 float* ro = radiance_out + ((size_t)j * spp_total + (s0 + k)) * 3;
@@ -3219,9 +3225,9 @@
     const uint32_t n = Q.counts[PT_Q_CUR];
     for (uint32_t i = blockIdx.x * blockDim.x + threadIdx.x; i < n; i += gridDim.x * blockDim.x) {
         const uint32_t p = Q.cur[i];
-        const int32_t rec = P.hit_rec[p];
+        const int32_t rec = P.hit_rec(p);
         if (rec < 0) continue;
-        const V3 ro = f4_3(P.ray_o[p]), rd = f4_3(P.ray_d[p]);
+        const V3 ro = f4_3(P.ray_o(p)), rd = f4_3(P.ray_d(p));
         Surf s;
         float thit;
         bool found;
@@ -3453,8 +3459,8 @@
                 V3 origin = offset_ray_origin(s.p, s.p_error, s.n, lp - s.p);
                 V3 target = offset_ray_origin(lp, lperr, ln, origin - lp);
                 V3 sd = target - origin;
-                R.sh_o[e] = make_float4(origin.x, origin.y, origin.z, 1.0f - PT_SHADOW_EPS);
-                R.sh_d[e] = make_float4(sd.x, sd.y, sd.z, 0.0f);
+                R.sh[e].o = make_float4(origin.x, origin.y, origin.z, 1.0f - PT_SHADOW_EPS);
+                R.sh[e].d = make_float4(sd.x, sd.y, sd.z, 0.0f);
                 if (light_is_delta<ENV>(lt)) A = f * li / lpdf;
                 else {
                     float weight = power_heuristic(lpdf, spdf);
@@ -3483,8 +3489,8 @@
                         const float weight = power_heuristic(spdf2, lp2);
                         const V3 le = env_le(sc, en, wi2);
                         B = f * le * 1.0f * (weight / spdf2);
-                        R.pr_o[e] = make_float4(po.x, po.y, po.z, PT_INF);
-                        R.pr_d[e] = make_float4(wi2.x, wi2.y, wi2.z, 0.0f);
+                        R.pr[e].o = make_float4(po.x, po.y, po.z, PT_INF);
+                        R.pr[e].d = make_float4(wi2.x, wi2.y, wi2.z, 0.0f);
                         nee |= PT_NEE_PROBE;
                     }
                 }
@@ -3496,8 +3502,8 @@
                     float weight = power_heuristic(spdf2, lp2);
                     V3 le = light_L(lt, ls.n, -wi2);
                     B = f * le * 1.0f * (weight / spdf2);
-                    R.pr_o[e] = make_float4(po.x, po.y, po.z, PT_INF);
-                    R.pr_d[e] = make_float4(wi2.x, wi2.y, wi2.z, 0.0f);
+                    R.pr[e].o = make_float4(po.x, po.y, po.z, PT_INF);
+                    R.pr[e].d = make_float4(wi2.x, wi2.y, wi2.z, 0.0f);
                     nee |= PT_NEE_PROBE;
                 }
             }
@@ -3511,21 +3517,21 @@
 PT_KERNEL void __launch_bounds__(PT_BLOCK) k_rec_init(PtScene sc, PtPaths P, PtRec R, uint32_t n) {
     for (uint32_t p = blockIdx.x * blockDim.x + threadIdx.x; p < n; p += gridDim.x * blockDim.x) {
         Sampler sl;
-        sl.index = P.sobol_index[p];
+        sl.index = P.sobol_index(p);
         sl.dim = 2;
-        const uint32_t pk = P.pixel[p];
+        const uint32_t pk = P.pixel(p);
         sl.px = (int32_t)(pk & 0xffffu) + sc.film.sample_bounds[0];
         sl.py = (int32_t)(pk >> 16) + sc.film.sample_bounds[1];
         V2 u_lens = mk2(0.0f, 0.0f);
         if (sc.cam.lens_radius > 0.0f) u_lens = sl.get_2d(sc);
         const float2 pf = P.p_film[p];
         RayDiffs rdf;
-        camera_differentials(sc, mk2(pf.x, pf.y), u_lens, f4_3(P.ray_o[p]), f4_3(P.ray_d[p]), rdf);
+        camera_differentials(sc, mk2(pf.x, pf.y), u_lens, f4_3(P.ray_o(p)), f4_3(P.ray_d(p)), rdf);
         R.diff[p] = make_float4(rdf.rx_o.x, rdf.rx_o.y, rdf.rx_o.z, 0.0f);
         R.diff[(size_t)R.n_paths + p] = make_float4(rdf.ry_o.x, rdf.ry_o.y, rdf.ry_o.z, 0.0f);
         R.diff[2 * (size_t)R.n_paths + p] = make_float4(rdf.rx_d.x, rdf.rx_d.y, rdf.rx_d.z, 0.0f);
         R.diff[3 * (size_t)R.n_paths + p] = make_float4(rdf.ry_d.x, rdf.ry_d.y, rdf.ry_d.z, 0.0f);
-        P.state[p] = (5u + 2u * R.n_arrays) | (0u << 16) | (PT_ST_DIFF << 24);
+        P.state(p) = (5u + 2u * R.n_arrays) | (0u << 16) | (PT_ST_DIFF << 24);
         P.nee[p] = 0;
     }
 }
@@ -3547,10 +3553,10 @@
         uint32_t ns = 0, np = 0, e_first = 0;
         if (i < n) {
         const uint32_t p = Q.cur[i];
-        const V3 ro = f4_3(P.ray_o[p]), rd = f4_3(P.ray_d[p]);
-        const int32_t rec = P.hit_rec[p];
+        const V3 ro = f4_3(P.ray_o(p)), rd = f4_3(P.ray_d(p));
+        const int32_t rec = P.hit_rec(p);
         const uint32_t inst = sc.n_instances ? P.hit_inst[p] : 0u;
-        uint32_t st = P.state[p];
+        uint32_t st = P.state(p);
         uint32_t dim = st & 0xffffu, depth = (st >> 16) & 0xffu, flags = (st >> 24) & 3u;
         const bool has_diff = (flags & PT_ST_DIFF) != 0;
         RayDiffs rdf;
@@ -3564,7 +3570,7 @@
             if (whitted) outcome = PT_REC_OUT_RETURN0;
             else {
                 const V3 no = offset_ray_origin(nd.s.p, nd.s.p_error, nd.s.n, rd);
-                P.ray_o[p] = make_float4(no.x, no.y, no.z, PT_INF);
+                P.ray_o(p) = make_float4(no.x, no.y, no.z, PT_INF);
                 flags &= ~PT_ST_DIFF;
                 outcome = PT_REC_OUT_RETRACE;
             }
@@ -3572,9 +3578,9 @@
         if (outcome == PT_REC_OUT_FRAME) {
             n_vert++;
             Sampler sm;
-            sm.index = P.sobol_index[p];
+            sm.index = P.sobol_index(p);
             sm.dim = dim;
-            const uint32_t pk = P.pixel[p];
+            const uint32_t pk = P.pixel(p);
             sm.px = (int32_t)(pk & 0xffffu) + sc.film.sample_bounds[0];
             sm.py = (int32_t)(pk >> 16) + sc.film.sample_bounds[1];
             V3 l = mk3(0.0f, 0.0f, 0.0f);
@@ -3596,8 +3602,8 @@
                             V3 origin = offset_ray_origin(nd.s.p, nd.s.p_error, nd.s.n, lp - nd.s.p);
                             V3 target = offset_ray_origin(lp, lperr, ln, origin - lp);
                             V3 sd = target - origin;
-                            R.sh_o[e0 + j] = make_float4(origin.x, origin.y, origin.z, 1.0f - PT_SHADOW_EPS);
-                            R.sh_d[e0 + j] = make_float4(sd.x, sd.y, sd.z, 0.0f);
+                            R.sh[e0 + j].o = make_float4(origin.x, origin.y, origin.z, 1.0f - PT_SHADOW_EPS);
+                            R.sh[e0 + j].d = make_float4(sd.x, sd.y, sd.z, 0.0f);
                             A = f * li * (abs_dot(wi, nd.n_before) / lpdf);
                             nee |= PT_NEE_SHADOW;
                         }
@@ -3660,7 +3666,7 @@
                 *rec_frame(R, depth, 6, p) = make_float4(le.x, le.y, le.z, 0.0f);
             }
         }
-        P.state[p] = (dim & 0xffffu) | (depth << 16) | ((flags | (outcome << 2)) << 24);
+        P.state(p) = (dim & 0xffffu) | (depth << 16) | ((flags | (outcome << 2)) << 24);
         if (outcome == PT_REC_OUT_FRAME) {
             e_first = p * R.epp;
             for (uint32_t j = 0; j < R.epp; j++) { const uint32_t fl = R.flags[e_first + j]; ns += (fl & PT_NEE_SHADOW) ? 1u : 0u; np += (fl & PT_NEE_PROBE) ? 1u : 0u; }
@@ -3687,7 +3693,7 @@
                 const uint32_t e = e_first + j, fl = R.flags[e];
                 if (fl & PT_NEE_SHADOW) {
                     Qn.shadow[os] = e;
-                    if (Qn.shadow_key) { const float4 o4 = R.sh_o[e], d4 = R.sh_d[e]; Qn.shadow_key[os] = ray_sort_key(sc, mk3(o4.x, o4.y, o4.z), mk3(d4.x, d4.y, d4.z)); }
+                    if (Qn.shadow_key) { const float4 o4 = R.sh[e].o, d4 = R.sh[e].d; Qn.shadow_key[os] = ray_sort_key(sc, mk3(o4.x, o4.y, o4.z), mk3(d4.x, d4.y, d4.z)); }
                     os++;
                 }
                 if (fl & PT_NEE_PROBE) Qn.probe[op++] = e;
@@ -3736,8 +3742,8 @@
     float wo_ns = dot(wo, ns);
     if (!(pdf > 0.0f && !is_black(f) && wi_ns != 0.0f)) return false;
     const V3 no = offset_ray_origin(s.p, s.p_error, s.n, wi);
-    P.ray_o[p] = make_float4(no.x, no.y, no.z, PT_INF);
-    P.ray_d[p] = make_float4(wi.x, wi.y, wi.z, 0.0f);
+    P.ray_o(p) = make_float4(no.x, no.y, no.z, PT_INF);
+    P.ray_d(p) = make_float4(wi.x, wi.y, wi.z, 0.0f);
     *child_flags = 0;
     if (has_diff) {
         const V3 rx_o = s.p + nd.th.dpdx, ry_o = s.p + nd.th.dpdy;
@@ -3810,15 +3816,15 @@
         uint32_t p = 0;
         if (i < n) {
             p = Q.cur[i];
-            uint32_t st = P.state[p];
+            uint32_t st = P.state(p);
             uint32_t dim = st & 0xffffu, depth = (st >> 16) & 0xffu, flags = (st >> 24) & 3u;
             const uint32_t outcome = (st >> 26) & 3u;
-            if (outcome == PT_REC_OUT_RETRACE) cont = true;
+            if (outcome == PT_REC_OUT_RETRACE) { cont = true; st &= ~(3u << 26); }
             else {
                 Sampler sm;
-                sm.index = P.sobol_index[p];
+                sm.index = P.sobol_index(p);
                 sm.dim = dim;
-                const uint32_t pk = P.pixel[p];
+                const uint32_t pk = P.pixel(p);
                 sm.px = (int32_t)(pk & 0xffffu) + sc.film.sample_bounds[0];
                 sm.py = (int32_t)(pk >> 16) + sc.film.sample_bounds[1];
                 V3 v = mk3(0.0f, 0.0f, 0.0f);
@@ -3871,7 +3877,7 @@
                 }
                 for (;;) {
                     if (returning) {
-                        if (d < 0) { P.L[p] = make_float4(v.x, v.y, v.z, 0.0f); break; }
+                        if (d < 0) { P.L(p) = make_float4(v.x, v.y, v.z, 0.0f); break; }
                         const float4 fr2 = *rec_frame(R, (uint32_t)d, 2, p);
                         const uint32_t ph = __float_as_uint(fr2.w);
                         const float4 pf = *rec_frame(R, (uint32_t)d, 7, p);
@@ -3915,9 +3921,9 @@
                 }
                 dim = sm.dim;
                 if (sc.sobol.kind == PT_SAMPLER_HALTON && dim > sc.sobol.h_n_dims) atomicOr(R.panic, 4u);
-                P.state[p] = (dim & 0xffffu) | (depth << 16) | (flags << 24);
+                st = (dim & 0xffffu) | (depth << 16) | (flags << 24);
             }
-            if (outcome == PT_REC_OUT_RETRACE) P.state[p] = st & ~(3u << 26);
+            P.state(p) = st;
         }
         s_e[n_batch][threadIdx.x] = p;
         want |= (cont ? 1u : 0u) << n_batch;
@@ -3978,17 +3984,19 @@
         const uint32_t p = base + lane;
         bool found = false;
         if (p < n_paths) {
-            const int32_t rec = P.hit_rec[p];
+            const int32_t rec = P.hit_rec(p);
             if (rec >= 0) {
-                const V3 ro = f4_3(P.ray_o[p]), rd = f4_3(P.ray_d[p]);
-                Sampler sl;
-                sl.index = P.sobol_index[p];
-                sl.dim = 2;
-                const uint32_t pk = P.pixel[p];
-                sl.px = (int32_t)(pk & 0xffffu) + sc.film.sample_bounds[0];
-                sl.py = (int32_t)(pk >> 16) + sc.film.sample_bounds[1];
+                const V3 ro = f4_3(P.ray_o(p)), rd = f4_3(P.ray_d(p));
                 V2 u_lens = mk2(0.0f, 0.0f);
-                if (sc.cam.lens_radius > 0.0f) u_lens = sl.get_2d(sc);
+                if (sc.cam.lens_radius > 0.0f) {
+                    Sampler sl;
+                    sl.index = P.sobol_index(p);
+                    sl.dim = 2;
+                    const uint32_t pk = P.pixel(p);
+                    sl.px = (int32_t)(pk & 0xffffu) + sc.film.sample_bounds[0];
+                    sl.py = (int32_t)(pk >> 16) + sc.film.sample_bounds[1];
+                    u_lens = sl.get_2d(sc);
+                }
                 const float2 pf = P.p_film[p];
                 RayDiffs rdf;
                 camera_differentials(sc, mk2(pf.x, pf.y), u_lens, ro, rd, rdf);
@@ -4018,7 +4026,13 @@
                     }
                     V3 l = mk3(0.0f, 0.0f, 0.0f);
                     switch (target) {
-                        case PT_AOV_DISTANCE: { const float dist = P.hit_t[p] / length(rd); l = aov_clamp(mk3(dist, dist, dist), scale); break; }
+                                                case PT_AOV_DISTANCE: {
+                            uint32_t p_again = p;
+                            asm volatile("" : "+v"(p_again));
+                            const float dist = P.hit_t(p_again) / length(rd);
+                            l = aov_clamp(mk3(dist, dist, dist), scale);
+                            break;
+                        }
                         case PT_AOV_DEPTH: { const float dist = length(sf.p - ro); l = aov_clamp(mk3(dist, dist, dist), scale); break; }
                         case PT_AOV_N: l = aov_v2c(sf.n, scale); break;
                         case PT_AOV_NS: l = aov_v2c(sf.sh_n, scale); break;
@@ -4035,7 +4049,7 @@
                         case PT_AOV_DPDVS: l = aov_v2c(sf.sh_dpdv, scale); break;
                         default: break;
                     }
-                    P.L[p] = make_float4(l.x, l.y, l.z, 0.0f);
+                    P.L(p) = make_float4(l.x, l.y, l.z, 0.0f);
                 }
             }
         }
@@ -4125,7 +4139,7 @@
     return PT_LAUNCH_CHECK();
 }
 template <bool SPH, bool INST>
-PT_DEV void ao_rays_body(const PtScene& sc, const PtPaths& P, uint32_t n_paths, float4* ao_o, float4* ao_d, float* ao_w, uint32_t* counter,
+PT_DEV void ao_rays_body(const PtScene& sc, const PtPaths& P, uint32_t n_paths, PtSegRec* ao_ray, float* ao_w, uint32_t* counter,
                          PtCounters* cnt) {
     const uint32_t lane = threadIdx.x & 63;
     const uint32_t n_s = (uint32_t)sc.ao_samples;
@@ -4135,9 +4149,9 @@
         Surf s;
         V3 rd = mk3(0.0f, 0.0f, 1.0f);
         if (p < n_paths) {
-            const V3 ro = f4_3(P.ray_o[p]);
-            rd = f4_3(P.ray_d[p]);
-            const int32_t rec = P.hit_rec[p];
+            const V3 ro = f4_3(P.ray_o(p));
+            rd = f4_3(P.ray_d(p));
+            const int32_t rec = P.hit_rec(p);
             float thit;
             if constexpr (INST) found = rec >= 0 && make_surf_inst<SPH>(sc, ro, rd, (uint32_t)rec, P.hit_inst[p], s, &thit);
             else found = rec >= 0 && make_surf_any<SPH>(sc, ro, rd, (uint32_t)rec, s, &thit);
@@ -4155,7 +4169,7 @@
         const V3 n = face_forward(s.n, -rd);
         const V3 ss = normalize(s.dpdu);
         const V3 tt = cross(s.n, ss);
-        const uint32_t pk = P.pixel[p];
+        const uint32_t pk = P.pixel(p);
         const int32_t px = (int32_t)(pk & 0xffffu) + sc.film.sample_bounds[0], py = (int32_t)(pk >> 16) + sc.film.sample_bounds[1];
         const uint32_t cam_sample = (uint32_t)P.probe_rec[p];
         for (uint32_t k = 0; k < n_s; k++) {
@@ -4174,23 +4188,23 @@
             wi = mk3(wi.x * ss.x + wi.y * tt.x + wi.z * n.x, wi.x * ss.y + wi.y * tt.y + wi.z * n.y, wi.x * ss.z + wi.y * tt.z + wi.z * n.z);
             const V3 o = offset_ray_origin(s.p, s.p_error, s.n, wi);
             const size_t r = r0 + k;
-            ao_o[r] = make_float4(o.x, o.y, o.z, PT_INF);
-            ao_d[r] = make_float4(wi.x, wi.y, wi.z, 0.0f);
+            ao_ray[r].o = make_float4(o.x, o.y, o.z, PT_INF);
+            ao_ray[r].d = make_float4(wi.x, wi.y, wi.z, 0.0f);
             ao_w[r] = dot(wi, n) / (pdf * (float)n_s);
         }
     }
 }
-PT_KERNEL void __launch_bounds__(PT_BLOCK) k_ao_rays(PtScene sc, PtPaths P, uint32_t n_paths, float4* ao_o, float4* ao_d, float* ao_w,
+PT_KERNEL void __launch_bounds__(PT_BLOCK) k_ao_rays(PtScene sc, PtPaths P, uint32_t n_paths, PtSegRec* ao_ray, float* ao_w,
                                                                 uint32_t* counter, PtCounters* cnt) {
-    ao_rays_body<false, false>(sc, P, n_paths, ao_o, ao_d, ao_w, counter, cnt);
-}
-PT_KERNEL void __launch_bounds__(PT_BLOCK) k_ao_rays_sph(PtScene sc, PtPaths P, uint32_t n_paths, float4* ao_o, float4* ao_d, float* ao_w,
+    ao_rays_body<false, false>(sc, P, n_paths, ao_ray, ao_w, counter, cnt);
+}
+PT_KERNEL void __launch_bounds__(PT_BLOCK) k_ao_rays_sph(PtScene sc, PtPaths P, uint32_t n_paths, PtSegRec* ao_ray, float* ao_w,
                                                                     uint32_t* counter, PtCounters* cnt) {
-    ao_rays_body<true, false>(sc, P, n_paths, ao_o, ao_d, ao_w, counter, cnt);
-}
-PT_KERNEL void __launch_bounds__(PT_BLOCK) k_ao_rays_inst(PtScene sc, PtPaths P, uint32_t n_paths, float4* ao_o, float4* ao_d, float* ao_w,
+    ao_rays_body<true, false>(sc, P, n_paths, ao_ray, ao_w, counter, cnt);
+}
+PT_KERNEL void __launch_bounds__(PT_BLOCK) k_ao_rays_inst(PtScene sc, PtPaths P, uint32_t n_paths, PtSegRec* ao_ray, float* ao_w,
                                                                      uint32_t* counter, PtCounters* cnt) {
-    ao_rays_body<true, true>(sc, P, n_paths, ao_o, ao_d, ao_w, counter, cnt);
+    ao_rays_body<true, true>(sc, P, n_paths, ao_ray, ao_w, counter, cnt);
 }
 PT_KERNEL void __launch_bounds__(PT_BLOCK) k_ao_tag(PtPaths P, uint32_t n_pix, uint32_t n_paths, uint32_t s0) {
     for (uint32_t i = blockIdx.x * blockDim.x + threadIdx.x; i < n_paths; i += gridDim.x * blockDim.x) P.probe_rec[i] = (int32_t)(s0 + i / n_pix);
@@ -4205,7 +4219,7 @@
             for (uint32_t k = 0; k < n_s; k++)
                 if (!occ[r0 + k]) l += ao_w[r0 + k];
         }
-        P.L[p] = make_float4(l, l, l, 0.0f);
+        P.L(p) = make_float4(l, l, l, 0.0f);
         P.nee[p] = 0;
     }
 }
@@ -4213,11 +4227,11 @@
     hipLaunchKernelGGL(k_ao_tag, dim3(grid), dim3(PT_BLOCK), 0, st, P, n_pix, n_paths, s0);
     return PT_LAUNCH_CHECK();
 }
-hipError_t ptk_ao_rays(hipStream_t st, int grid, const PtScene& sc, const PtPaths& P, uint32_t n_paths, float4* ao_o, float4* ao_d, float* ao_w,
+hipError_t ptk_ao_rays(hipStream_t st, int grid, const PtScene& sc, const PtPaths& P, uint32_t n_paths, PtSegRec* ao_ray, float* ao_w,
                        uint32_t* counter, PtCounters* cnt) {
-    if (sc.n_instances) hipLaunchKernelGGL(k_ao_rays_inst, dim3(grid), dim3(PT_BLOCK), 0, st, sc, P, n_paths, ao_o, ao_d, ao_w, counter, cnt);
-    else if (sc.n_spheres) hipLaunchKernelGGL(k_ao_rays_sph, dim3(grid), dim3(PT_BLOCK), 0, st, sc, P, n_paths, ao_o, ao_d, ao_w, counter, cnt);
-    else hipLaunchKernelGGL(k_ao_rays, dim3(grid), dim3(PT_BLOCK), 0, st, sc, P, n_paths, ao_o, ao_d, ao_w, counter, cnt);
+    if (sc.n_instances) hipLaunchKernelGGL(k_ao_rays_inst, dim3(grid), dim3(PT_BLOCK), 0, st, sc, P, n_paths, ao_ray, ao_w, counter, cnt);
+    else if (sc.n_spheres) hipLaunchKernelGGL(k_ao_rays_sph, dim3(grid), dim3(PT_BLOCK), 0, st, sc, P, n_paths, ao_ray, ao_w, counter, cnt);
+    else hipLaunchKernelGGL(k_ao_rays, dim3(grid), dim3(PT_BLOCK), 0, st, sc, P, n_paths, ao_ray, ao_w, counter, cnt);
     return PT_LAUNCH_CHECK();
 }
 PT_KERNEL void k_ao_queue(PtQueues Q, const uint32_t* counter, uint32_t n_s) {
diff --git a/pbrt-r3_amd/csrc/pt_kernels_decl.inc b/pbrt-r3_amd/csrc/pt_kernels_decl.inc
--- a/pbrt-r3_amd/csrc/pt_kernels_decl.inc
+++ b/pbrt-r3_amd/csrc/pt_kernels_decl.inc
@@ -30,7 +30,7 @@
 hipError_t ptk_sobol_samples(hipStream_t st, const PtScene& sc, uint32_t n, const int32_t* pixel_xy, const uint32_t* sample_index, const uint32_t* dim,
                              float* out);
 hipError_t ptk_ao_tag(hipStream_t st, int grid, const PtPaths& P, uint32_t n_pix, uint32_t n_paths, uint32_t s0);
-hipError_t ptk_ao_rays(hipStream_t st, int grid, const PtScene& sc, const PtPaths& P, uint32_t n_paths, float4* ao_o, float4* ao_d, float* ao_w,
+hipError_t ptk_ao_rays(hipStream_t st, int grid, const PtScene& sc, const PtPaths& P, uint32_t n_paths, PtSegRec* ao_ray, float* ao_w,
                        uint32_t* counter, PtCounters* cnt);
 hipError_t ptk_ao_queue(hipStream_t st, const PtQueues& Q, const uint32_t* counter, uint32_t n_s);
 hipError_t ptk_iota(hipStream_t st, int grid, uint32_t* out, uint32_t n);
```

New measurement: 1202 (median of 6 runs). No clear change (+0.3%).
